# alanqrwang/keymorph

Hardware: AMD Instinct MI355X
Metric: volume-pairs/sec (fwd+bwd) at 256^3, 512 kp, TPS (higher is better)
Workload: dtype f32

## Files before the change

### include/keymorph_hip.h

```cpp
#ifndef KEYMORPH_HIP_H
#define KEYMORPH_HIP_H
#include <stddef.h>
#include <stdint.h>
#ifdef __cplusplus
extern "C" {
#endif

#define KMH_EINVAL (-22)
#define KMH_ABI_VERSION 1
int kmh_abi_version(void);

int kmh_grid_sample3d_fwd(const float* x, const float* grid, float* out, int N, int C, int D, int H,
                          int W, int Do, int Ho, int Wo, int mode, void* stream);
int kmh_grid_sample3d_bwd_grid(const float* x, const float* grid, const float* gout, float* dgrid,
                               int N, int C, int D, int H, int W, int Do, int Ho, int Wo, void* stream);
int kmh_grid_sample3d_bwd_input(const float* grid, const float* gout, float* dx, int N, int C, int D,
                                int H, int W, int Do, int Ho, int Wo, void* stream);

size_t kmh_reduce_ws_bytes(void);
int kmh_mse_fwd(const float* a, const float* b, long long n, float* out, void* ws, void* stream);
int kmh_mse_bwd(const float* a, const float* b, const float* gscale, long long n, float* da, void* stream);
int kmh_warp_mse_fwd(const float* x, const float* grid, const float* fixed, float* out, float* out_loss,
                     int N, int C, int D, int H, int W, int Do, int Ho, int Wo, void* ws, void* stream);
int kmh_warp_mse_fwd_grad(const float* x, const float* grid, const float* fixed, float* out, float* out_loss,
// ... 124 lines not shown
                               const float* wscale, void* stream);
size_t kmh_conv3d_up2_dgrad_pack_bytes(int Cout, int Cl, int terms);
int kmh_conv3d_up2_dgrad_pack_weight(const float* w, void* packed, int Cout, int Ctot, int cofs, int Cl, int terms,
                                     const float* wscale, void* stream);
size_t kmh_conv3d_up2_dgrad_stats_ws_bytes(int N, int Dl, int Hl, int Wl, int Cl);
int kmh_conv3d_up2_dgrad(const float* dz, const void* packed, float* ds, int N, int Dl, int Hl, int Wl, int Cl, int Cout,
                         int terms, const float* dscale, const float* wscale, void* stats_ws, double* stats_out,
                         int in_blocked ,
                         void* stream);
int kmh_up2_boxsum(const float* dz, float* G, int N, int Dl, int Hl, int Wl, int Cout, int in_blocked ,
                   void* stream);
size_t kmh_up2_wgrad_gemm_ws_bytes(int N, int V, int Cl, int J);
int kmh_up2_wgrad_gemm(const float* A, const float* B, float* C, int N, int V, int Cl, int J, int terms,
                       const float* ascale, const float* bscale, const float* a_scale, const float* a_shift, void* ws,
                       void* stream);
int kmh_up2_wgrad_fold_ok(int Cl, int Cout, int terms);
size_t kmh_up2_wgrad_fold_ws_bytes(int N, int Dl, int Hl, int Wl, int Cl, int Cout);
int kmh_up2_wgrad_fold(const float* xl, const float* dz, float* C, int N, int Dl, int Hl, int Wl, int Cl, int Cout, int terms,
                       const float* ascale, const float* dscale, const float* a_scale, const float* a_shift, int dz_blocked,
                       void* ws, void* stream);
int kmh_conv3d_up2_fwd(const float* xl, const float* scale, const float* shift, int Ctot, int cofs, const void* packed,
                       float* y, int N, int Dl, int Hl, int Wl, int Cl, int Cout, int terms, const float* ascale,
                       const float* wscale, void* stream);
size_t kmh_conv3d_wgrad_bf_ws_bytes(int N, int D, int H, int W, int Cin, int Cout, int terms);
int kmh_conv3d_wgrad_bf_blocked_ok(int N, int D, int H, int W, int Cin, int Cout, int terms);
int kmh_conv3d_wgrad_bf(const float* x, const float* scale, const float* shift, const float* dz,
                        const float* dzmask, float* dw, int N, int D, int H, int W, int Cin, int Cout, int relu_in,
                        int accumulate, int terms, int append_ones, const float* xscale, const float* dscale, int dz_blocked, const float* w_fold, double* bhat,
                        void* ws, void* stream);
int kmh_conv3d_wgrad_bf_sparse_ok(int N, int D, int H, int W, int Cin, int Cout, int terms);
int kmh_conv3d_wgrad_bf_sparse(const float* x, const float* scale, const float* shift, const float* dzp,
                               const unsigned char* winners, float* dw, int N, int D, int H, int W, int Cin, int Cout,
                               int relu_in, int accumulate, int terms, const float* xscale, const float* dscale,
                               const float* w_fold, double* bhat, void* ws, void* stream);
size_t kmh_conv3d_first_layer_fwd_ws_bytes(int N, int D, int H, int W, int Cout);
int kmh_conv3d_first_layer_fwd(const float* x, const float* scale, const float* shift, const float* w, float* y, int N,
                               int D, int H, int W, int Cout, void* ws, double* stats_out, void* stream);
size_t kmh_conv3d_first_layer_wgrad_ws_bytes(int N, int D, int H, int W, int Cout);
int kmh_conv3d_first_layer_wgrad(const float* x, const float* dz, const float* dzmask, const float* c123, double* rs, int N,
                                 int D, int H, int W, int Cout, void* ws, void* stream);
int kmh_conv3d_first_layer_fold(const void* rs, int rs_f64, const float* w, const float* scale_n, const float* shift_n, int Cout,
                                float* dw, double* ab_n, int accumulate, void* stream);
size_t kmh_conv3d_wgrad_ws_bytes(int N, int D, int H, int W, int Cin, int Cout);
int kmh_conv3d_wgrad(const float* x, const float* scale, const float* shift, const float* dz,
                     const float* dzmask, float* dw, int N, int D, int H, int W, int Cin, int Cout, int relu_in,
                     int accumulate, void* ws, void* stream);

size_t kmh_channel_stats_ws_bytes(int N, int C);
int kmh_channel_stats(const float* a, const float* b, int mode, int N, long long V, int C, double* out, void* ws,
                      const int* only_if, void* stream);
int kmh_gn_fwd_coeffs(const double* stats, const float* gamma, const float* beta, int N, int C, int G, double count,
                      float eps, float* scale, float* shift, float* mean_rstd, float* ascale, void* stream);
int kmh_absmax_scale(const float* x, long long n, float min_abs, float* out2, void* stream);
int kmh_gn_bwd_coeffs(const double* ab, const float* gamma, const float* mean_rstd, int N, int C, int G,
                      double count, float* c123, float* dgamma, float* dbeta, const int* only_if, void* stream);
int kmh_gn_bwd_coeffs_fold(const double* dstats, const double* bhat, const float* gamma, const float* beta,
                           const float* mean_rstd, int N, int C, int G, double count, float* c123, float* dgamma,
                           float* dbeta, int* fallback, void* stream);
int kmh_in_bwd_stats(const float* du, const float* z, const float* scale, const float* shift, int N, long long V, int C,
                     double* out, void* ws, void* stream);
int kmh_in_bwd_apply(const float* du, const float* z, const float* scale, const float* shift, const float* c123, int N,
                     long long V, int C, float* dz, float* dz_scale2, void* stream);
int kmh_in_bwd_apply_pool(const unsigned char* argmax, const float* du, const float* z, const float* scale,
                          const float* shift, const float* c123, int N, int D, int H, int W, int C, float* dz,
                          float* dz_scale2, void* stream);

int kmh_gn_bwd_apply(const float* dxn, const float* x, const float* c123, int N, long long V, int C,
                     int relu_mask, int accumulate, float* dx, float* dx_scale2, int out_blocked, void* stream);
int kmh_relu_mask(const float* dy, const float* y, long long n, float* dz, void* stream);
int kmh_norm_apply(const float* x, const float* scale, const float* shift, int N, long long V, int C, int relu,
                   float* y, void* stream);

int kmh_maxpool3d_fwd(const float* x, float* y, unsigned char* argmax, int N, int D, int H, int W, int C, void* stream);
int kmh_maxpool3d_bwd(const float* x, const unsigned char* argmax, const float* dy, const float* add, int add_cstride,
                      float* dx, int N, int D, int H, int W, int C, int out_blocked, void* stream);
size_t kmh_maxpool3d_bwd_split_bytes(int N, int D, int H, int W, int C);
int kmh_maxpool3d_bwd_split(const unsigned char* argmax, const float* dy, const float* dy_scale2, float* dxs, int N, int D,
                            int H, int W, int C, void* stream);
int kmh_maxpool3d_bwd_lazy(const unsigned char* argmax, const float* dy, const float* dxn, const float* x, const float* c123,
                           float* dx, int N, int D, int H, int W, int C, float* dx_scale2, void* stream);
int kmh_upcat_fwd(const float* skip, const float* low, float* out, int N, int D, int H, int W, int Cs, int Dl,
                  int Hl, int Wl, int Cl, void* stream);
int kmh_upcat_bwd(const float* dout, float* dskip, float* dlow, int N, int D, int H, int W, int Cs, int Dl, int Hl,
                  int Wl, int Cl, int accumulate_skip, void* stream);
int kmh_layout_convert(const float* in, float* out, int N, long long V, int C, int to_ncdhw, void* stream);

int kmh_pointwise_pack(const float* w, float* wt, int Cout, int Cin, void* stream);
int kmh_pointwise_fwd(const float* x, const float* wt, const float* bias, float* y, int N, long long V, int Cin,
                      int Cout, void* stream);
int kmh_pointwise_dgrad(const float* dy, const float* w, float* dx, int N, long long V, int Cin, int Cout,
                        void* stream);
size_t kmh_pointwise_wgrad_ws_bytes(int N, long long V, int Cin, int Cout);
int kmh_pointwise_wgrad(const float* dy, const float* x, float* dw, float* dbias, int N, long long V, int Cin,
                        int Cout, int accumulate, void* ws, void* stream);

size_t kmh_headcom_fwd_ws_bytes(int N, long long V, int Cout);
size_t kmh_headcom_bwd_ws_bytes(int N, long long V, int Cin, int Cout);
int kmh_headcom_fwd(const float* feat, const float* w, const float* bias, float* pts, float* sums, float* sq, int N, int D,
                    int H, int W, int Cin, int Cout, void* ws, void* stream);
int kmh_headcom_bwd(const float* dpts, const float* dpower, const float* feat, const float* w, const float* bias,
                    const float* sums, float* dfeat, float* dw, float* dbias, int N, int D, int H, int W, int Cin,
                    int Cout, int mask_dfeat, void* ws, void* stream);
size_t kmh_headcom_fwd_bf_ws_bytes(int N, long long V, int Cout, int terms);
size_t kmh_headcom_bwd_bf_ws_bytes(int N, long long V, int Cin, int Cout, int terms);
size_t kmh_headcom_mask_words(int N, int D, int H, int W, int Cout);
int kmh_headcom_fwd_bf(const float* feat, const float* w, const float* bias, float* pts, float* sums, float* sq,
// ... 60 lines not shown
```

### keymorph_amd/_handoff.py

```python
KEYS = ("stats", "grad_scale", "layout", "lazy_gn", "up_sources", "packed")
_ATTR = "_kmh_handoff"


def attach(t, key: str, payload) -> None:
    assert key in KEYS and payload is not None, key
    if not hasattr(t, _ATTR):
        setattr(t, _ATTR, {})
    getattr(t, _ATTR)[key] = (payload, t._version)


def peek(t, key: str):
    assert key in KEYS, key
    tag = getattr(t, _ATTR, {}).get(key)
    return tag[0] if (tag is not None and tag[1] == t._version) else None


def expect(t, key: str, present: bool, what: str, remedy: str) -> None:
    if (peek(t, key) is not None) != present:
        raise RuntimeError("keymorph_amd: %s: the tensor that arrived carries %s '%s' hand-off where %s was expected (a hook, "
                           "retain_grad, an in-place op or a second consumer replaced or changed it?) -- set %s=1"
                           % (what, "a" if not present else "no valid", key, "one" if present else "none", remedy))
```

### keymorph_amd/_lib.py

```python
from __future__ import annotations

import ctypes as C
import os

from .build import LIBPATH

_f = C.c_void_p
_i = C.c_int
_ll = C.c_longlong
_sz = C.c_size_t

PROTOS = {
    "kmh_abi_version": (_i, []),
    "kmh_grid_sample3d_fwd": (_i, [_f, _f, _f, _i, _i, _i, _i, _i, _i, _i, _i, _i, _f]),
    "kmh_grid_sample3d_bwd_grid": (_i, [_f, _f, _f, _f, _i, _i, _i, _i, _i, _i, _i, _i, _f]),
    "kmh_grid_sample3d_bwd_input": (_i, [_f, _f, _f, _i, _i, _i, _i, _i, _i, _i, _i, _f]),
    "kmh_reduce_ws_bytes": (_sz, []),
    "kmh_mse_fwd": (_i, [_f, _f, _ll, _f, _f, _f]),
    "kmh_mse_bwd": (_i, [_f, _f, _f, _ll, _f, _f]),
    "kmh_warp_mse_fwd": (_i, [_f, _f, _f, _f, _f, _i, _i, _i, _i, _i, _i, _i, _i, _f, _f]),
    "kmh_warp_mse_fwd_grad": (_i, [_f, _f, _f, _f, _f, _f, _i, _i, _i, _i, _i, _i, _i, _i, _f, _f]),
    "kmh_scale_unless_one": (_i, [_f, _ll, _f, _f]),
    "kmh_dice_sums": (_i, [_f, _f, _i, _ll, _f, _f, _f]),
    "kmh_rows_axpby": (_i, [_f, _f, _f, _f, _i, _ll, _f, _f]),
# ... 37 lines not shown
    "kmh_mi_final": (_i, [_f, _f, _i, _ll, _i, _f, _f, _f]),
    "kmh_mi_bwd": (_i, [_f, _f, _f, _f, _f, _i, _ll, _i, _f, _f, _f]),
    "kmh_mi_range": (_i, [_f, _f, _i, _ll, _i, _i, C.c_float, C.c_float, _i, C.c_float, C.c_float, _f, _f, _f]),
    "kmh_mi_hist_ranges": (_i, [_f, _f, _f, _i, _ll, _i, _f, _f]),
    "kmh_warp_mi_ws_bytes": (_sz, [_i, _i, _i, _i, _i]),
    "kmh_warp_mi_hist": (_i, [_f, _f, _f, _f, _i, _i, _i, _i, _i, _f, _f]),
    "kmh_warp_mi_bwd": (_i, [_f, _f, _f, _f, _f, _f, _i, _i, _i, _i, _i, _f, _f, _f]),
    "kmh_affine_build_matrix": (_i, [_f, _f, _f, _f, _f, _i, _f]),
    "kmh_affine_points_bwd": (_i, [_f, _f, _f, _f, _f, _i, _i, _f]),
    "kmh_com3d_fwd": (_i, [_f, _f, _f, _i, _i, _i, _i, _i, _f, _f]),
    "kmh_com3d_bwd": (_i, [_f, _f, _f, _f, _i, _i, _i, _i, _i, _f]),
    "kmh_conv3d_pack_weight": (_i, [_f, _f, _i, _i, _i, _f]),
    "kmh_conv3d_fwd": (_i, [_f, _f, _f, _f, _f, _f, _f, _i, _i, _i, _i, _i, _i, _i, _i, _f]),
    "kmh_conv3d_pack_bf_bytes": (_sz, [_i, _i, _i, _i]),
    "kmh_conv3d_pack_weight_bf": (_i, [_f, _f, _i, _i, _i, _i, _f, _f]),
    "kmh_conv3d_fwd_bf": (_i, [_f, _f, _f, _f, _f, _f, _f, _i, _i, _i, _i, _i, _i, _i, _i, _i, _i, _f, _f, _f, _f, _i, _f, _f]),
    "kmh_conv3d_fwd_bf_set_dispatch": (_i, [_i]),
    "kmh_conv3d_fwd_bf_variant": (_i, [_i, _i, _i, _i, _i, _i, _i, _i, _i]),
    "kmh_conv3d_fwd_bf_pool_ok": (_i, [_i, _i, _i, _i, _i, _i, _i]),
    "kmh_conv3d_fwd_bf_split_ok": (_i, [_i, _i, _i, _i, _i, _i, _i]),
    "kmh_conv3d_fwd_bf_sparse_ok": (_i, [_i, _i, _i, _i, _i, _i, _i]),
    "kmh_conv3d_fwd_bf_sparse": (_i, [_f, _f, _f, _f, _f, _i, _i, _i, _i, _i, _i, _i, _i, _f, _f, _f, _f, _f]),
    "kmh_conv3d_fwd_bf_pool": (_i, [_f, _f, _f, _f, _f, _f, _i, _i, _i, _i, _i, _i, _i, _i, _f, _f, _f, _f, _i, _f]),
    "kmh_conv3d_up2_dgrad_pack_bytes": (_sz, [_i, _i, _i]),
    "kmh_conv3d_up2_dgrad_pack_weight": (_i, [_f, _f, _i, _i, _i, _i, _i, _f, _f]),
    "kmh_conv3d_up2_dgrad_stats_ws_bytes": (_sz, [_i, _i, _i, _i, _i]),
    "kmh_conv3d_up2_dgrad": (_i, [_f, _f, _f, _i, _i, _i, _i, _i, _i, _i, _f, _f, _f, _f, _i, _f]),
    "kmh_up2_boxsum": (_i, [_f, _f, _i, _i, _i, _i, _i, _i, _f]),
    "kmh_up2_wgrad_gemm_ws_bytes": (_sz, [_i, _i, _i, _i]),
    "kmh_up2_wgrad_gemm": (_i, [_f, _f, _f, _i, _i, _i, _i, _i, _f, _f, _f, _f, _f, _f]),
    "kmh_up2_wgrad_fold_ok": (_i, [_i, _i, _i]),
    "kmh_up2_wgrad_fold_ws_bytes": (_sz, [_i, _i, _i, _i, _i, _i]),
    "kmh_up2_wgrad_fold": (_i, [_f, _f, _f, _i, _i, _i, _i, _i, _i, _i, _f, _f, _f, _f, _i, _f, _f]),
    "kmh_conv3d_up2_pack_bytes": (_sz, [_i, _i, _i]),
    "kmh_conv3d_up2_pack_weight": (_i, [_f, _f, _i, _i, _i, _i, _i, _f, _f]),
    "kmh_conv3d_up2_fwd": (_i, [_f, _f, _f, _i, _i, _f, _f, _i, _i, _i, _i, _i, _i, _i, _f, _f, _f]),
    "kmh_conv3d_fwd_bf_stats_ws_bytes": (_sz, [_i, _i, _i, _i, _i, _i]),
    "kmh_conv3d_first_layer_fwd_ws_bytes": (_sz, [_i, _i, _i, _i, _i]),
    "kmh_conv3d_first_layer_fwd": (_i, [_f, _f, _f, _f, _f, _i, _i, _i, _i, _i, _f, _f, _f]),
    "kmh_conv3d_wgrad_bf_ws_bytes": (_sz, [_i, _i, _i, _i, _i, _i, _i]),
    "kmh_conv3d_wgrad_bf": (_i, [_f, _f, _f, _f, _f, _f, _i, _i, _i, _i, _i, _i, _i, _i, _i, _i, _f, _f, _i, _f, _f, _f, _f]),
    "kmh_conv3d_wgrad_bf_blocked_ok": (_i, [_i, _i, _i, _i, _i, _i, _i]),
    "kmh_conv3d_wgrad_bf_sparse_ok": (_i, [_i, _i, _i, _i, _i, _i, _i]),
    "kmh_conv3d_wgrad_bf_sparse": (_i, [_f, _f, _f, _f, _f, _f, _i, _i, _i, _i, _i, _i, _i, _i, _i, _f, _f, _f, _f, _f, _f]),
    "kmh_conv3d_first_layer_wgrad_ws_bytes": (_sz, [_i, _i, _i, _i, _i]),
    "kmh_conv3d_first_layer_wgrad": (_i, [_f, _f, _f, _f, _f, _i, _i, _i, _i, _i, _f, _f]),
    "kmh_conv3d_first_layer_fold": (_i, [_f, _i, _f, _f, _f, _i, _f, _f, _i, _f]),
    "kmh_conv3d_wgrad_ws_bytes": (_sz, [_i, _i, _i, _i, _i, _i]),
    "kmh_conv3d_wgrad": (_i, [_f, _f, _f, _f, _f, _f, _i, _i, _i, _i, _i, _i, _i, _i, _f, _f]),
    "kmh_channel_stats_ws_bytes": (_sz, [_i, _i]),
    "kmh_channel_stats": (_i, [_f, _f, _i, _i, _ll, _i, _f, _f, _f, _f]),
    "kmh_gn_fwd_coeffs": (_i, [_f, _f, _f, _i, _i, _i, C.c_double, C.c_float, _f, _f, _f, _f, _f]),
    "kmh_absmax_scale": (_i, [_f, _ll, C.c_float, _f, _f]),
    "kmh_gn_bwd_coeffs": (_i, [_f, _f, _f, _i, _i, _i, C.c_double, _f, _f, _f, _f, _f]),
    "kmh_gn_bwd_coeffs_fold": (_i, [_f, _f, _f, _f, _f, _i, _i, _i, C.c_double, _f, _f, _f, _f, _f]),
    "kmh_gn_bwd_apply": (_i, [_f, _f, _f, _i, _ll, _i, _i, _i, _f, _f, _i, _f]),
    "kmh_in_bwd_stats": (_i, [_f, _f, _f, _f, _i, _ll, _i, _f, _f, _f]),
    "kmh_in_bwd_apply": (_i, [_f, _f, _f, _f, _f, _i, _ll, _i, _f, _f, _f]),
    "kmh_in_bwd_apply_pool": (_i, [_f, _f, _f, _f, _f, _f, _i, _i, _i, _i, _i, _f, _f, _f]),
    "kmh_relu_mask": (_i, [_f, _f, _ll, _f, _f]),
    "kmh_norm_apply": (_i, [_f, _f, _f, _i, _ll, _i, _i, _f, _f]),
    "kmh_maxpool3d_fwd": (_i, [_f, _f, _f, _i, _i, _i, _i, _i, _f]),
    "kmh_maxpool3d_bwd": (_i, [_f, _f, _f, _f, _i, _f, _i, _i, _i, _i, _i, _i, _f]),
    "kmh_maxpool3d_bwd_split_bytes": (_sz, [_i, _i, _i, _i, _i]),
    "kmh_maxpool3d_bwd_split": (_i, [_f, _f, _f, _f, _i, _i, _i, _i, _i, _f]),
    "kmh_maxpool3d_bwd_lazy": (_i, [_f, _f, _f, _f, _f, _f, _i, _i, _i, _i, _i, _f, _f]),
    "kmh_upcat_fwd": (_i, [_f, _f, _f, _i, _i, _i, _i, _i, _i, _i, _i, _i, _f]),
    "kmh_upcat_bwd": (_i, [_f, _f, _f, _i, _i, _i, _i, _i, _i, _i, _i, _i, _i, _f]),
    "kmh_layout_convert": (_i, [_f, _f, _i, _ll, _i, _i, _f]),
    "kmh_pointwise_pack": (_i, [_f, _f, _i, _i, _f]),
    "kmh_pointwise_fwd": (_i, [_f, _f, _f, _f, _i, _ll, _i, _i, _f]),
    "kmh_pointwise_dgrad": (_i, [_f, _f, _f, _i, _ll, _i, _i, _f]),
    "kmh_pointwise_wgrad_ws_bytes": (_sz, [_i, _ll, _i, _i]),
    "kmh_pointwise_wgrad": (_i, [_f, _f, _f, _f, _i, _ll, _i, _i, _i, _f, _f]),
    "kmh_headcom_fwd_ws_bytes": (_sz, [_i, _ll, _i]),
    "kmh_headcom_bwd_ws_bytes": (_sz, [_i, _ll, _i, _i]),
    "kmh_headcom_fwd_bf_ws_bytes": (_sz, [_i, _ll, _i, _i]),
    "kmh_headcom_bwd_bf_ws_bytes": (_sz, [_i, _ll, _i, _i, _i]),
    "kmh_headcom_mask_words": (_sz, [_i, _i, _i, _i, _i]),
    "kmh_headcom_fwd_bf": (_i, [_f, _f, _f, _f, _f, _f, _f, _i, _i, _i, _i, _i, _i, _i, _f, _f, _f]),
    "kmh_headcom_bwd_bf": (_i, [_f, _f, _f, _f, _f, _f, _f, _f, _f, _i, _i, _i, _i, _i, _i, _i, _i, _f, _f, _f, _f, _f]),
    "kmh_headcom_fwd": (_i, [_f, _f, _f, _f, _f, _f, _i, _i, _i, _i, _i, _i, _f, _f]),
    "kmh_headcom_bwd": (_i, [_f, _f, _f, _f, _f, _f, _f, _f, _f, _i, _i, _i, _i, _i, _i, _i, _f, _f]),
    "kmh_adam_step": (_i, [_f, _f, _f, _f, _ll, C.c_float, C.c_float, C.c_float, C.c_float, _i, C.c_float, _f]),
    "kmh_resize_trilinear3d_fwd": (_i, [_f, _f, _i, _i, _i, _i, _i, _i, _i, _i, _f, _f, _f, _i, _f]),
    "kmh_resize_trilinear3d_bwd": (_i, [_f, _f, _i, _i, _i, _i, _i, _i, _i, _i, _f, _f, _f, _f, _f, _f, _i, _f]),
    "kmh_components3d_ws_bytes": (_sz, [_i, _i, _i, _i]),
    "kmh_components3d": (_i, [_f, _f, _i, _i, _i, _i, _f, _f, _f]),
    "kmh_clean_mask3d": (_i, [_f, _f, _i, _i, _i, _i, C.c_double, _f, _f, _f]),
    "kmh_conv3d_thin_ok": (_i, [_i, _i]),
    "kmh_conv3d_thin_wgrad_ok": (_i, [_i, _i]),
    "kmh_conv3d_thin_fwd": (_i, [_f, _f, _f, _f, _i, _i, _i, _i, _i, _i, _i, _f]),
    "kmh_conv3d_thin_dgrad": (_i, [_f, _f, _f, _f, _i, _i, _i, _i, _i, _i, _f]),
    "kmh_conv3d_thin_wgrad_ws_bytes": (_sz, [_i, _i, _i, _i, _i, _i]),
    "kmh_conv3d_thin_wgrad": (_i, [_f, _f, _f, _f, _f, _i, _i, _i, _i, _i, _i, _f, _f]),
    "kmh_field_identity": (_i, [_f, _i, _i, _i, _i, _f]),
    "kmh_field_compose": (_i, [_f, _f, _f, _i, _i, _i, _i, _i, _i, _i, _f]),
    "kmh_field_invert_ws_bytes": (_sz, [_i, _i, _i, _i]),
    "kmh_field_invert": (_i, [_f, _f, _f, _f, _f, _f, _f, _i, _i, _i, _i, C.c_float, _i, _f, _f]),
    "kmh_field_to_displacement": (_i, [_f, _f, _i, _i, _i, _i, _f]),
    "kmh_field_from_displacement": (_i, [_f, _f, _i, _i, _i, _i, _f]),
    "kmh_bspline_grid_fwd": (_i, [_f, _f, _f, _i, _i, _i, _i, _i, _i, _i, _f]),
    "kmh_bspline_grid_ws_bytes": (_sz, [_i, _i, _i, _i, _i, _i, _i]),
    "kmh_bspline_grid_bwd": (_i, [_f, _f, _i, _i, _i, _i, _i, _i, _i, _f, _f]),
    "kmh_bspline_bending_ws_bytes": (_sz, [_i]),
    "kmh_bspline_bending_fwd": (_i, [_f, _f, _i, _i, _i, _i, _f, _f]),
# ... 105 lines not shown
```

### keymorph_amd/backbone_ops.py

```python
from __future__ import annotations

import os
from typing import Optional, Tuple

import torch

from . import _lib
from ._handoff import attach, expect, peek
from ._lib import check
from .ops import _p, _prep, _stream, workspace

Tensor = torch.Tensor
EPS = 1e-5

CONV_MODE = os.environ.get("KEYMORPH_HIP_CONV", "f16x3")
_TERMS = {"f16x3": 2, "bf16x6": 3}
_HEAD_TERMS = {"f16x3": 2, "bf16x6": 3}
BF_ROWS_PER_WAVE = int(os.environ.get("KEYMORPH_HIP_BF_ROWS", "4"))


def set_conv_mode(mode: str):
    global CONV_MODE
    assert mode in ("f32", "f16x3", "bf16x6"), mode
    CONV_MODE = mode


_SWITCHES = {
    "KEYMORPH_NO_EPILOGUE_STATS": "a separate statistics pass per layer instead of the convolution epilogue's",
    "KEYMORPH_NO_UPCONV": "materialise upsample+concat instead of the fused decoder operator, forward",
    "KEYMORPH_NO_UPCONV_BWD": "materialise upsample+concat instead of the fused decoder operator, backward",
    "KEYMORPH_NO_UPCONV_WGRAD": "the fused decoder operator rebuilds the upsampled half for the 27-tap weight gradient",
    "KEYMORPH_NO_UP2_FOLD": "the upsampled channels' weight gradient by the box-sum tensor + matrix product route",
    "KEYMORPH_NO_STATS_FOLD": "GroupNorm's backward statistics by a pass over the tensors",
    "KEYMORPH_NO_BLOCKED_GRADS": "every gradient in (N,D,H,W,C)",
    "KEYMORPH_NO_BLOCKED_UPCAT": "only the fused decoder operator's gradient in (N,D,H,W,C)",
    "KEYMORPH_NO_SPLIT_POOLGRAD": "the 256^3-level pooled gradient scattered as fp32 instead of pre-split records",
    "KEYMORPH_NO_SPARSE_POOLGRAD": "the 256^3-level pooled gradient scattered into pre-split records instead of handed over with its winners",
    "KEYMORPH_NO_CONV_POOL": "separate pooling pass instead of the conv epilogue's",
    "KEYMORPH_NO_LAZY_FIRST": "GroupNorm backward of the first block as its own pass",
    "KEYMORPH_NO_LAZY_SKIP": "GroupNorm's backward of a decoder skip applied in the decoder",
    "KEYMORPH_NO_LAZY_IN": "ConvNet block by block: separate norm / ReLU / pooling passes",
    "KEYMORPH_RANGE_AUDIT": "debug (ON = audit): per-sample dynamic range of every gradient operand, RANGE_AUDIT_LOG",
}


def _off(name: str) -> bool:
    if name not in _SWITCHES:
        raise KeyError(name)
    return bool(os.environ.get(name))


import contextlib
import functools
import threading

_AMP_DEFAULT = os.environ.get("KEYMORPH_AMP", "0") not in ("", "0")
_amp_tls = threading.local()


def amp_enabled() -> bool:
    return bool(getattr(_amp_tls, "on", _AMP_DEFAULT))


@contextlib.contextmanager
def amp_scope(on: bool):
    prev = amp_enabled()
    _amp_tls.on = bool(on)
    try:
        yield
    finally:
        _amp_tls.on = prev


def set_amp(on: bool) -> bool:
    prev = amp_enabled()
    _amp_tls.on = bool(on)
    return prev


def _t(terms: int) -> int:
    return 1 if (terms == 2 and amp_enabled()) else terms


def _binds_amp(cls):
    fwd, bwd = cls.forward, cls.backward

    @staticmethod
    @functools.wraps(fwd)
    def forward(ctx, *a, **k):
        ctx._kmh_amp = amp_enabled()
        return fwd(ctx, *a, **k)

    @staticmethod
    @functools.wraps(bwd)
    def backward(ctx, *g):
        with amp_scope(ctx._kmh_amp):
            return bwd(ctx, *g)

    cls.forward, cls.backward = forward, backward
    return cls


FIRST_BLOCK_DGRAD = os.environ.get("KEYMORPH_FIRST_BLOCK_DGRAD", "")


def set_first_block_dgrad(mode: str) -> str:
    global FIRST_BLOCK_DGRAD
    assert mode in ("", "bf16x6"), mode
    prev, FIRST_BLOCK_DGRAD = FIRST_BLOCK_DGRAD, mode
    return prev


def first_block_dgrad_terms() -> int:
    return 3 if (FIRST_BLOCK_DGRAD == "bf16x6" and CONV_MODE == "f16x3") else 0


def _f32(shape, dev):
    return torch.empty(shape, dtype=torch.float32, device=dev)


def channel_stats(a: Tensor, b: Optional[Tensor], N: int, V: int, C: int, only_if: Optional[Tensor] = None) -> Tensor:
    lib = _lib.load()
    out = torch.empty((N, C, 2), dtype=torch.float64, device=a.device)
    ws = workspace(int(lib.kmh_channel_stats_ws_bytes(N, C)), a.device, "stats")
    check(lib.kmh_channel_stats(_p(a), _p(b), 0 if b is None else 1, N, V, C, _p(out), _p(ws), _p(only_if), _stream()),
          "kmh_channel_stats")
    return out


def _needs_range_scales() -> bool:
    return _TERMS.get(CONV_MODE, 0) == 2


_CONSTS = {}


def _const(device, *values) -> Tensor:
    key = (str(device), values)
    t = _CONSTS.get(key)
    if t is None:
        t = _CONSTS[key] = torch.tensor(values, dtype=torch.float32, device=device)
    return t


def absmax_scale(x: Tensor, min_abs: float = 0.0) -> Tensor:
    lib = _lib.load()
    out = _f32((2,), x.device)
    check(lib.kmh_absmax_scale(_p(x), x.numel(), float(min_abs), _p(out), _stream()), "kmh_absmax_scale")
    return out


def conv_emits_stats() -> bool:
    return CONV_MODE != "f32" and not _off("KEYMORPH_NO_EPILOGUE_STATS")


def _tag_stats(t: Tensor, stats: Optional[Tensor]) -> None:
    if stats is not None:
        attach(t, "stats", stats)


def _peek_stats(t: Tensor) -> Optional[Tensor]:
    return peek(t, "stats")


STATS_STATS = {"carried": 0, "measured": 0}


def input_stats(x: Tensor, N: int, V: int, C: int) -> Tensor:
    s = _peek_stats(x)
    if s is not None and tuple(s.shape) == (N, C, 2):
        STATS_STATS["carried"] += 1
        return s
    STATS_STATS["measured"] += 1
    return channel_stats(x, None, N, V, C)


def _tag_grad_scale(t: Optional[Tensor], scale2: Optional[Tensor], loosen: float = 1.0) -> None:
    if t is None or scale2 is None:
        return
    if loosen != 1.0:
        scale2 = torch.stack([scale2[0] * (1.0 / loosen), scale2[1] * loosen])
    attach(t, "grad_scale", scale2)


def _sum_bound(a: Optional[Tensor], b: Optional[Tensor]) -> Optional[Tensor]:
    if a is None or b is None:
        return None
    return torch.stack([torch.minimum(a[0], b[0]) * 0.5, torch.maximum(a[1], b[1]) * 2.0])


GRAD_SCALE_STATS = {"carried": 0, "measured": 0}
RANGE_AUDIT_LOG = []


def range_audit(t: Tensor) -> dict:
    with torch.no_grad():
        a = t.detach().abs().reshape(t.shape[0], -1).float()
        m_n = a.amax(dim=1).double()
        M = float(m_n.max())
        if M == 0.0:
            return {"max": 0.0, "per_sample_log2_below_max": [0.0] * t.shape[0], "worst_relative_precision": 2.0 ** -22,
                    "flushed_fraction": 0.0}
        S = 2.0 ** (14 - int(torch.floor(torch.log2(torch.tensor(M))).item()))
        nz = a > 0
        flushed = float(((a * S < 2.0 ** -25) & nz).sum()) / max(1.0, float(nz.sum()))
        below = [float(torch.log2(torch.tensor(M) / m)) if float(m) > 0 else float("inf") for m in m_n]
        prec = max(max(2.0 ** -22, 2.0 ** (b - 39)) for b in below if b != float("inf"))
        return {"max": M, "per_sample_log2_below_max": below, "worst_relative_precision": prec,
                "flushed_fraction": flushed}


def grad_scale(dy: Tensor) -> Tensor:
    if _off("KEYMORPH_RANGE_AUDIT") and not _blocked_kind(dy):
        RANGE_AUDIT_LOG.append(dict(range_audit(dy), shape=tuple(dy.shape)))
    s = peek(dy, "grad_scale")
    if s is not None:
        GRAD_SCALE_STATS["carried"] += 1
        return s
    GRAD_SCALE_STATS["measured"] += 1
    return absmax_scale(dy)


def norm_coeffs(stats: Tensor, gamma: Optional[Tensor], beta: Optional[Tensor], N: int, C: int, G: int, V: int,
                want_ascale: bool = False):
    lib = _lib.load()
    dev = stats.device
    scale, shift, mr = _f32((N, C), dev), _f32((N, C), dev), _f32((N, G, 2), dev)
    ascale = _f32((2,), dev) if (want_ascale and _needs_range_scales()) else None
    check(lib.kmh_gn_fwd_coeffs(_p(stats), _p(gamma), _p(beta), N, C, G, float(V), EPS, _p(scale), _p(shift),
                                _p(mr), _p(ascale), _stream()), "kmh_gn_fwd_coeffs")
    return (scale, shift, mr, ascale) if want_ascale else (scale, shift, mr)


def pack_weight(w: Tensor, transposed: bool, wscale: Optional[Tensor] = None, terms: int = 0) -> Tensor:
    lib = _lib.load()
    Cout, Cin = w.shape[:2]
    if CONV_MODE != "f32":
        terms = terms or _TERMS[CONV_MODE]
        out = torch.empty(int(lib.kmh_conv3d_pack_bf_bytes(Cout, Cin, int(transposed), terms)), dtype=torch.uint8,
                          device=w.device)
        wscale = (wscale if wscale is not None else absmax_scale(w)) if terms == 2 else None
        attach(out, "packed", (terms, wscale))
        check(lib.kmh_conv3d_pack_weight_bf(_p(w), _p(out), Cout, Cin, int(transposed), terms, _p(wscale), _stream()),
              "kmh_conv3d_pack_weight_bf")
        return out
    out = _f32((27, Cout, Cin) if transposed else (27, Cin, Cout), w.device)
    check(lib.kmh_conv3d_pack_weight(_p(w), _p(out), Cout, Cin, int(transposed), _stream()), "kmh_conv3d_pack_weight")
    return out


def _packed(pk: Tensor):
    return peek(pk, "packed") or (0, None)


def _conv_meta(N, D, H, W, Cin, Cout, taps=27) -> None:
    if _lib.profiler.enabled:
        _lib.profiler.meta = {"flops": 2.0 * taps * Cin * Cout * N * D * H * W, "shape": (N, D, H, W, Cin, Cout)}


def conv3_raw(x, scale, shift, packed, bias, N, D, H, W, Cin, Cout, relu_in, relu_out, mask=None,
              ascale=None, stats_out: Optional[Tensor] = None, in_blocked: bool = False,
              addend: Optional[Tensor] = None, winners: Optional[Tensor] = None) -> Tensor:
    lib = _lib.load()
    y = _f32((N, D, H, W, Cout), x.device)
    _conv_meta(N, D, H, W, Cin, Cout)
    terms, wscale = _packed(packed)
    if int(in_blocked) == 3:
        assert terms == 2 and winners is not None and scale is None and shift is None and mask is None and addend is None \
            and not relu_in and ascale is not None and not amp_enabled(), "pooled + winners: a gradient operand of the f16x3 mode"
        assert x.shape == winners.shape == (N, D // 2, H // 2, W // 2, Cin) and winners.dtype == torch.uint8
        sws = None
        if stats_out is not None:
            sws = workspace(int(lib.kmh_conv3d_fwd_bf_stats_ws_bytes(N, D, H, W, Cout, BF_ROWS_PER_WAVE)), x.device, "convstats")
        check(lib.kmh_conv3d_fwd_bf_sparse(_p(x), _p(winners), _p(packed), _p(bias), _p(y), N, D, H, W, Cin, Cout, int(relu_out), 2,
                                           _p(ascale), _p(wscale), _p(sws), _p(stats_out), _stream()), "kmh_conv3d_fwd_bf_sparse")
        return y
    assert winners is None
    if terms:
        if terms == 2 and ascale is None:
            assert scale is None, "a normalised input needs the range scale of the NORMALISED tensor (norm_coeffs)"
            ascale = absmax_scale(x)
        sws = None
        if stats_out is not None:
            sws = workspace(int(lib.kmh_conv3d_fwd_bf_stats_ws_bytes(N, D, H, W, Cout, BF_ROWS_PER_WAVE)), x.device,
                            "convstats")
        check(lib.kmh_conv3d_fwd_bf(_p(x), _p(scale), _p(shift), _p(mask), _p(packed), _p(bias), _p(y), N, D, H, W,
                                    Cin, Cout, int(relu_in), int(relu_out), _t(terms), BF_ROWS_PER_WAVE,
                                    _p(ascale if terms == 2 else None), _p(wscale), _p(sws), _p(stats_out),
                                    int(in_blocked), _p(addend), _stream()), "kmh_conv3d_fwd_bf")
        return y
    assert stats_out is None and addend is None, "only the split-operand kernels emit output statistics / take an addend"
    assert not in_blocked, "the channel-blocked input layout belongs to the split-operand kernels"
    check(lib.kmh_conv3d_fwd(_p(x), _p(scale), _p(shift), _p(mask), _p(packed), _p(bias), _p(y), N, D, H, W, Cin,
                             Cout, int(relu_in), int(relu_out), _stream()), "kmh_conv3d_fwd")
# ... 262 lines not shown
            if dy_sparse:
                sd_in = sd_in if sd_in is not None else absmax_scale(dy)
                full = dy.detach()
                SPLIT_STATS["handoffs"] += 1
                SPARSE_STATS["handoffs"] += 1
            elif dy_split:
                sd_in = sd_in if sd_in is not None else absmax_scale(dy)
                full = torch.empty((N, Cout // 8, D * H * W + 1, 8), dtype=torch.float32, device=dy.device)
                check(lib.kmh_maxpool3d_bwd_split(_p(ctx.pool_arg), _p(dy), _p(sd_in), _p(full), N, D, H, W, Cout, _stream()),
                      "kmh_maxpool3d_bwd_split")
                SPLIT_STATS["handoffs"] += 1
            else:
                full = torch.empty((N, D, H, W, Cout), dtype=torch.float32, device=dy.device)
                if odd:
                    full.zero_()
                check(lib.kmh_maxpool3d_bwd(None, _p(ctx.pool_arg), _p(dy), None, 0, _p(full), N, D, H, W, Cout,
                                            int(dy_blocked), _stream()), "kmh_maxpool3d_bwd")
            _tag_grad_scale(full, sd_in)
            dy = full
            if dy_blocked:
                attach(dy, "layout", 3 if dy_sparse else (2 if dy_split else 1))
                BLOCKED_STATS["handoffs"] += 1
        kind = 3 if dy_sparse else (2 if dy_split else int(dy_blocked))
        if _blocked_kind(dy) != kind:
            raise RuntimeError("keymorph_amd: gradient layout kind %d where %d was expected (1 = fp32 channel-blocked, 2 = pre-split"
                               " records, 3 = pooled + winners); a hook or an in-place op between two operators changed the tensor" % (_blocked_kind(dy), kind))
        ymask = None if dy_premasked else y
        first = Cin == 1 and not ctx.needs_input_grad[0] and (Cout <= 16 or CONV_MODE != "f32")
        dscale = (grad_scale(dy) if (_needs_range_scales() and not (first and Cout <= 16)) else None)
        if first:
            lazy_c123, ymask = lazy_tag if dy_lazy else (None, ymask)
            dw, dgamma, dbeta = first_layer_grads(x, scale, shift, mr, gamma, weight, dy, ymask, N, D, H, W, Cout, G,
                                                  dscale=dscale, lazy_c123=lazy_c123)
            return (None, dgamma, dbeta, dw) + (None,) * 9
        assert not dy_lazy, "only the first layer's correlation kernel applies a pending GroupNorm backward"
        need_affine = ctx.needs_input_grad[1] or ctx.needs_input_grad[2]
        need_dxn = ctx.needs_input_grad[0] or need_affine
        fold = need_dxn and ctx.needs_input_grad[3] and conv_emits_stats() and not _off("KEYMORPH_NO_STATS_FOLD")
        bhat = torch.zeros((N, Cin), dtype=torch.float64, device=x.device) if fold else None
        dw = (conv3_wgrad(x, scale, shift, dy, N, D, H, W, Cin, Cout, False, dzmask=ymask, xscale=ctx.ascale,
                          dscale=dscale, dz_blocked=kind, fold=(weight, bhat) if fold else None,
                          winners=ctx.pool_arg if dy_sparse else None)
              if ctx.needs_input_grad[3] else None)
        dx = dgamma = dbeta = None
        if need_dxn:
            dstats = torch.empty((N, Cin, 2), dtype=torch.float64, device=x.device) if fold else None
            if ctx.dgrad_terms:
                FIRST_BLOCK_STATS["exact_dgrads"] += 1
            dxn = conv3_raw(dy, None, None,
                            pack_weight(weight, True, None if ctx.dgrad_terms else getattr(ctx, "wscale", None), terms=ctx.dgrad_terms),
                            None, N, D, H, W, Cout, Cin, False, False,
                            mask=ymask, ascale=dscale, in_blocked=kind, stats_out=dstats,
                            winners=ctx.pool_arg if dy_sparse else None)
            sc2 = torch.zeros(2, dtype=torch.float32, device=x.device) if (_needs_range_scales() and ctx.needs_input_grad[0]) else None
            c123, dgamma, dbeta = _gn_bwd_coeffs(lambda flag: channel_stats(dxn, x, N, V, Cin, only_if=flag), gamma, mr,
                                                 N, Cin, G, V, fold=(dstats, bhat, beta) if fold else None)
            if ctx.needs_input_grad[0] and dx_lazy:
                assert x_from_relu and not dx_blocked
                dx = dxn
                attach(dx, "lazy_gn", (c123, x))
                LAZY_STATS["handoffs"] += 1
            elif ctx.needs_input_grad[0]:
                dx = _gn_bwd_apply(dxn, x, c123, N, V, Cin, sc2, from_relu=x_from_relu,
                                   out=torch.empty_like(dxn) if dx_blocked else None, blocked=dx_blocked)
        return (dx, dgamma, dbeta, dw) + (None,) * 9


def _up2_forward(skip, low, scale, shift, ascale, weight, N, D, H, W, Cs, Cl, Cout, ystats):
    lib = _lib.load()
    terms = _TERMS[CONV_MODE]
    dev = skip.device
    pk_s = pack_weight(weight[:, :Cs].contiguous(), False)
    wsu = None
    if terms == 2:
        wsu = absmax_scale(weight[:, Cs:].contiguous()) * _const(dev, 0.125, 8.0)
    pku = torch.empty(int(lib.kmh_conv3d_up2_pack_bytes(Cout, Cl, terms)), dtype=torch.uint8, device=dev)
    check(lib.kmh_conv3d_up2_pack_weight(_p(weight), _p(pku), Cout, Cs + Cl, Cs, Cl, terms, _p(wsu), _stream()),
          "kmh_conv3d_up2_pack_weight")
    part = _f32((N, D, H, W, Cout), dev)
    _conv_meta(N, D, H, W, Cl, Cout, taps=8)
    check(lib.kmh_conv3d_up2_fwd(_p(low), _p(scale), _p(shift), Cs + Cl, Cs, _p(pku), _p(part), N, D // 2, H // 2,
                                 W // 2, Cl, Cout, _t(terms), _p(ascale if terms == 2 else None), _p(wsu), _stream()),
          "kmh_conv3d_up2_fwd")
    y = conv3_raw(skip, scale[:, :Cs].contiguous(), shift[:, :Cs].contiguous(), pk_s, None, N, D, H, W, Cs, Cout,
                  False, True, ascale=ascale, stats_out=ystats, addend=part)
    UPCONV_STATS["calls"] += 1
    return y


def upcat_conv_ok(skip, low, Cout) -> bool:
    return (CONV_MODE in _TERMS and conv_emits_stats() and Cout > 16 and Cout % 4 == 0 and skip.shape[-1] % 8 == 0
            and low.shape[-1] % 8 == 0 and all(a == 2 * b for a, b in zip(skip.shape[1:4], low.shape[1:4]))
            and not _off("KEYMORPH_NO_UPCONV") and not _off("KEYMORPH_NO_UPCONV_BWD"))


@_binds_amp
class _UpCatConvGCR(torch.autograd.Function):

    @staticmethod
    def forward(ctx, skip, low, gamma, beta, weight, num_groups, dy_premasked, dskip_lazy=False, dy_blocked=False):
        ctx.dskip_lazy = bool(dskip_lazy)
        ctx.dy_blocked = bool(dy_blocked)
        assert not dy_blocked or dy_premasked, "a channel-blocked gradient comes from a SingleConv, i.e. already masked"
        skip, low, gamma, beta, weight = _prep(skip), _prep(low), _prep(gamma), _prep(beta), _prep(weight)
        N, D, H, W, Cs = skip.shape
        Cl, Cout = low.shape[-1], weight.shape[0]
        V = D * H * W
# ... 23 lines not shown
            check(lib.kmh_relu_mask(_p(dy), _p(y), dy.numel(), _p(dzm), _stream()), "kmh_relu_mask")
            dy = dzm
        dscale = grad_scale(dy) if _needs_range_scales() else None
        bhat_s = torch.zeros((N, Cs), dtype=torch.float64, device=dy.device)
        dw_s = conv3_wgrad(skip, scale[:, :Cs].contiguous(), shift[:, :Cs].contiguous(), dy, N, D, H, W, Cs, Cout, False,
                           xscale=ctx.ascale, dscale=dscale, dz_blocked=blk, fold=(weight[:, :Cs].contiguous(), bhat_s))
        if Cout % 4 == 0 and not _off("KEYMORPH_NO_UPCONV_WGRAD"):
            Vl = V // 8
            sc_l, sh_l = scale[:, Cs:].contiguous(), shift[:, Cs:].contiguous()
            terms = _TERMS[CONV_MODE]
            dwn = _f32((N, Cl, 27, Cout), dy.device)
            if _lib.profiler.enabled:
                _lib.profiler.meta = {"flops": 2.0 * 27 * Cl * Cout * N * Vl, "shape": (N, Vl, Cl, 27 * Cout)}
            if up2_wgrad_fold_ok(Cl, Cout, terms):
                UP2_STATS["fold"] += 1
                gws = workspace(int(lib.kmh_up2_wgrad_fold_ws_bytes(N, D // 2, H // 2, W // 2, Cl, Cout)), dy.device, "wgrad")
                check(lib.kmh_up2_wgrad_fold(_p(low), _p(dy), _p(dwn), N, D // 2, H // 2, W // 2, Cl, Cout, _t(terms), _p(ctx.ascale),
                                             _p(dscale), _p(sc_l), _p(sh_l), int(blk), _p(gws), _stream()), "kmh_up2_wgrad_fold")
            else:
                UP2_STATS["boxsum"] += 1
                boxes = _f32((N, Vl, 27 * Cout), dy.device)
                check(lib.kmh_up2_boxsum(_p(dy), _p(boxes), N, D // 2, H // 2, W // 2, Cout, int(blk), _stream()), "kmh_up2_boxsum")
                gws = workspace(int(lib.kmh_up2_wgrad_gemm_ws_bytes(N, Vl, Cl, 27 * Cout)), dy.device, "wgrad")
                bsc = (dscale * _const(dy.device, 0.125, 8.0)) if terms == 2 else None
                check(lib.kmh_up2_wgrad_gemm(_p(low), _p(boxes), _p(dwn), N, Vl, Cl, 27 * Cout, _t(terms),
                                             _p(ctx.ascale if terms == 2 else None), _p(bsc), _p(sc_l), _p(sh_l), _p(gws),
                                             _stream()), "kmh_up2_wgrad_gemm")
                del boxes
            dw_l = dwn.sum(0).permute(2, 0, 1).reshape(Cout, Cl, 3, 3, 3)
            wl = weight[:, Cs:].reshape(Cout, Cl, 27).permute(1, 2, 0)
            bhat_l = (dwn.double() * wl.double().unsqueeze(0)).sum(dim=(2, 3))
        else:
            xu = _f32((N, D, H, W, Cl), dy.device)
            check(lib.kmh_upcat_fwd(_p(skip), _p(low), _p(xu), N, D, H, W, 0, D // 2, H // 2, W // 2, Cl, _stream()),
                  "kmh_upcat_fwd")
            bhat_l = torch.zeros((N, Cl), dtype=torch.float64, device=dy.device)
            dw_l = conv3_wgrad(xu, scale[:, Cs:].contiguous(), shift[:, Cs:].contiguous(), dy, N, D, H, W, Cl, Cout,
                               False, xscale=ctx.ascale, dscale=dscale, dz_blocked=blk,
                               fold=(weight[:, Cs:].contiguous(), bhat_l))
            del xu
        dw = torch.cat([dw_s, dw_l], dim=1)
        bhat = torch.cat([bhat_s, bhat_l], dim=1)
        dst_s = torch.empty((N, Cs, 2), dtype=torch.float64, device=dy.device)
        dxn_s = conv3_raw(dy, None, None, pack_weight(weight[:, :Cs].contiguous(), True), None, N, D, H, W, Cout, Cs,
                          False, False, ascale=dscale, stats_out=dst_s, in_blocked=blk)
        dst_l = torch.empty((N, Cl, 2), dtype=torch.float64, device=dy.device)
        dsum_l = conv3_up2_dgrad(dy, weight, Cs, Cl, dscale, stats_out=dst_l, dz_blocked=blk)
        dstats = torch.cat([dst_s, dst_l], dim=1)
        ab = lambda flag: torch.cat([channel_stats(dxn_s, skip, N, V, Cs, only_if=flag),
                                     channel_stats(dsum_l, low, N, V // 8, Cl, only_if=flag)], dim=1)
        c123, dgamma, dbeta = _gn_bwd_coeffs(ab, gamma, mr, N, C, G, V, fold=(dstats, bhat, beta))
        c_s = c123[:, :Cs].contiguous()
        c_l = (c123[:, Cs:] * _const(dy.device, 1.0, 8.0, 8.0)).contiguous()
        sc_s = torch.zeros(2, dtype=torch.float32, device=dy.device) if _needs_range_scales() else None
        sc_l = torch.zeros(2, dtype=torch.float32, device=dy.device) if _needs_range_scales() else None
        dskip = dlow = None
        if ctx.needs_input_grad[0] and ctx.dskip_lazy:
            dskip = dxn_s
            attach(dskip, "lazy_gn", (c_s, skip))
            LAZY_STATS["handoffs"] += 1
        elif ctx.needs_input_grad[0]:
            dskip = _gn_bwd_apply(dxn_s, skip, c_s, N, V, Cs, sc_s)
        if ctx.needs_input_grad[1]:
            dlow = _gn_bwd_apply(dsum_l, low, c_l, N, V // 8, Cl, sc_l)
        return (dskip, dlow, dgamma, dbeta, dw) + (None,) * 4


def upcat_blocked_ok(skip, low, Cout) -> bool:
    N, D, H, W, Cs = skip.shape
    return (torch.is_grad_enabled() and Cout % 8 == 0 and not _off("KEYMORPH_NO_UPCONV_WGRAD")
            and not _off("KEYMORPH_NO_BLOCKED_UPCAT") and grad_blocked_ok(N, D, H, W, Cs, Cout))


def upcat_conv_gcr(skip, low, gamma, beta, weight, num_groups: int, dy_premasked: bool = False,
                   dskip_lazy: bool = False, dy_blocked: bool = False) -> Tensor:
    if dskip_lazy:
        node = skip.grad_fn
        if node is not None and type(node).__name__ == "_PoolForkBackward":
            node._kmh_expect_lazy = True
        else:
            dskip_lazy = False
    y, ystats = _UpCatConvGCR.apply(skip, low, gamma, beta, weight, num_groups, dy_premasked, dskip_lazy, dy_blocked)
    _tag_stats(y, ystats)
    return y


def single_conv_gcr(x, gamma, beta, weight, num_groups: int, x_from_relu: bool = True,
                    dy_premasked: bool = False, dy_blocked: bool = False, dx_blocked: bool = False,
                    pool: bool = False, dy_lazy: bool = False, dx_lazy: bool = False, dgrad_terms: int = 0) -> Tensor:
    y, ystats = _SingleConvGCR.apply(x, gamma, beta, weight, num_groups, x_from_relu, dy_premasked, dy_blocked,
                                     dx_blocked, pool, dy_lazy, dx_lazy, dgrad_terms)
    _tag_stats(y, ystats)
    return y


POOL_STATS = {"fused": 0}
FIRST_BLOCK_STATS = {"exact_dgrads": 0}
LAZY_STATS = {"handoffs": 0}


def lazy_skip_ok(skip) -> bool:
    return (torch.is_grad_enabled() and skip.shape[1] % 2 == 0 and skip.shape[2] % 2 == 0 and skip.shape[3] % 2 == 0
            and skip.shape[4] % 4 == 0 and not _off("KEYMORPH_NO_LAZY_SKIP"))


def lazy_first_layer_ok(x, cout1: int) -> bool:
    return (x.shape[-1] == 1 and cout1 <= 16 and not x.requires_grad and torch.is_grad_enabled()
            and not _off("KEYMORPH_NO_LAZY_FIRST"))
# ... 31 lines not shown
    if add is not None:
        acs = add.stride(3)
        dense_voxels = add.stride() == (D * H * W * acs, H * W * acs, W * acs, acs, 1)
        if odd or add.dtype != torch.float32 or not dense_voxels:
            add, acs = add.contiguous().float().clone(), C
    if add is not None and acs == C and odd:
        dx = add
    else:
        dx = (torch.zeros if odd else torch.empty)((N, D, H, W, C), dtype=torch.float32, device=arg.device)
    dy_c = _prep(dy)
    check(lib.kmh_maxpool3d_bwd(None, _p(arg), _p(dy_c), _p(add), acs, _p(dx), N, D, H, W, C, int(out_blocked),
                                _stream()), "kmh_maxpool3d_bwd")
    if out_blocked:
        attach(dx, "layout", 1)
        BLOCKED_STATS["handoffs"] += 1
    sd = peek(dy, "grad_scale")
    _tag_grad_scale(dx, sd if add_tag is _NO_ADD else _sum_bound(sd, add_tag))
    return dx


class _MaxPool2(torch.autograd.Function):
    @staticmethod
    def forward(ctx, x, blocked_grad):
        ctx.blocked_grad = bool(blocked_grad)
        return _maxpool_fwd(ctx, x)[1]

    @staticmethod
    def backward(ctx, dy):
        return _maxpool_bwd(ctx, dy, None, ctx.blocked_grad), None


def maxpool2(x: Tensor, blocked_grad: bool = False) -> Tensor:
    return _MaxPool2.apply(x, blocked_grad)


class _PoolFork(torch.autograd.Function):

    @staticmethod
    def forward(ctx, x):
        x, y = _maxpool_fwd(ctx, x)
        ctx.set_materialize_grads(False)
        return y, x.view_as(x)

    @staticmethod
    def backward(ctx, dy, dskip):
        if dskip is not None and getattr(ctx, "_kmh_expect_lazy", False):
            expect(dskip, "lazy_gn", True, "pool_fork's skip gradient with its GroupNorm backward pending", "KEYMORPH_NO_LAZY_SKIP")
        lazy = peek(dskip, "lazy_gn") if dskip is not None else None
        if lazy is not None:
            lib = _lib.load()
            c123, x = lazy
            N, D, H, W, C = ctx.xshape
            dxn = _prep(dskip)
            sc2 = torch.zeros(2, dtype=torch.float32, device=dxn.device) if _needs_range_scales() else None
            if dy is None:
                return _gn_bwd_apply(dxn, x, c123, N, D * H * W, C, sc2)
            (arg,) = ctx.saved_tensors
            dx = torch.empty((N, D, H, W, C), dtype=torch.float32, device=dxn.device)
            check(lib.kmh_maxpool3d_bwd_lazy(_p(arg), _p(_prep(dy)), _p(dxn), _p(x), _p(c123), _p(dx), N, D, H, W, C, _p(sc2),
                                             _stream()), "kmh_maxpool3d_bwd_lazy")
            _tag_grad_scale(dx, sc2)
            return dx
        if dy is None:
            return dskip
        return _maxpool_bwd(ctx, dy, dskip)


def pool_fork(x: Tensor):
    y, skip = _PoolFork.apply(x)
    _tag_stats(skip, _peek_stats(x))
    return y, skip


class _UpCat(torch.autograd.Function):
    @staticmethod
    def forward(ctx, skip, low, lazy_skip_grad):
        lib = _lib.load()
        skip, low = _prep(skip), _prep(low)
        N, D, H, W, Cs = skip.shape
        _, Dl, Hl, Wl, Cl = low.shape
        out = _f32((N, D, H, W, Cs + Cl), skip.device)
        check(lib.kmh_upcat_fwd(_p(skip), _p(low), _p(out), N, D, H, W, Cs, Dl, Hl, Wl, Cl, _stream()), "kmh_upcat_fwd")
        ctx.dims = (N, D, H, W, Cs, Dl, Hl, Wl, Cl)
        ctx.lazy = bool(lazy_skip_grad)
        return out

    @staticmethod
    def backward(ctx, dout):
        lib = _lib.load()
        N, D, H, W, Cs, Dl, Hl, Wl, Cl = ctx.dims
        dout = _prep(dout)
        dskip = None if ctx.lazy else _f32((N, D, H, W, Cs), dout.device)
        dlow = _f32((N, Dl, Hl, Wl, Cl), dout.device)
        check(lib.kmh_upcat_bwd(_p(dout), _p(dskip), _p(dlow), N, D, H, W, Cs, Dl, Hl, Wl, Cl, 0, _stream()),
              "kmh_upcat_bwd")
        if ctx.lazy:
            dskip = dout[..., :Cs]
        sd = peek(dout, "grad_scale")
        _tag_grad_scale(dskip, sd)
        if (D, H, W) == (2 * Dl, 2 * Hl, 2 * Wl):
            _tag_grad_scale(dlow, sd, loosen=8.0)
        return dskip, dlow, None


def upcat(skip: Tensor, low: Tensor, lazy_skip_grad: bool = False) -> Tensor:
    out = _UpCat.apply(skip, low, lazy_skip_grad)
    ss, sl = _peek_stats(skip), _peek_stats(low)
# ... 156 lines not shown
        dw = conv3_wgrad(x, None, None, dz, N, D, H, W, Cin, Cout, False, dzmask=dzmask)
        dzm = dz
        if dzmask is not None:
            dzm = torch.empty_like(dz)
            check(lib.kmh_relu_mask(_p(dz), _p(dzmask), dz.numel(), _p(dzm), _stream()), "kmh_relu_mask")
        db = channel_stats(dzm, None, N, V, Cout)[:, :, 0].sum(0).float()
        dx = None
        if ctx.needs_input_grad[0]:
            dx = conv3_raw(dz, None, None, pack_weight(weight, True), None, N, D, H, W, Cout, Cin, False, False,
                           mask=dzmask)
        return (dx, dw, db, dgamma, dbeta) + (None,) * 5


def conv_block(x, weight, bias, gamma=None, beta=None, groups: int = 0) -> Tensor:
    return _ConvBlock.apply(x, weight, bias, gamma, beta, groups)


def conv_block_batchnorm(x, weight, bias, bn: "torch.nn.modules.batchnorm._BatchNorm", training: bool) -> Tensor:
    assert abs(bn.eps - EPS) < 1e-12, "the norm kernels use eps = 1e-5 (what every norm layer of the reference uses)"
    use_batch = training or not bn.track_running_stats or bn.running_mean is None
    if not use_batch:
        return _ConvBlock.apply(x, weight, bias, bn.weight, bn.bias, 0, 2, bn.running_mean, bn.running_var, bn.eps)
    y, stats = _ConvBlock.apply(x, weight, bias, bn.weight, bn.bias, 0, 1, None, None, bn.eps)
    if training and bn.track_running_stats and bn.running_mean is not None:
        with torch.no_grad():
            n = float(x.shape[0] * x.shape[1] * x.shape[2] * x.shape[3])
            mean = stats[0, :, 0] / n
            var = (stats[0, :, 1] / n - mean * mean).clamp_min(0.0)
            bn.num_batches_tracked += 1
            mom = bn.momentum if bn.momentum is not None else 1.0 / float(bn.num_batches_tracked)
            bn.running_mean.mul_(1 - mom).add_(mean.to(bn.running_mean.dtype), alpha=mom)
            bn.running_var.mul_(1 - mom).add_((var * (n / max(n - 1.0, 1.0))).to(bn.running_var.dtype), alpha=mom)
    return y


LAZY_IN_STATS = {"units": 0}


def convnet_lazy_ok(x: Tensor, norm_type: str) -> bool:
    return (norm_type == "instance" and conv_emits_stats() and not _off("KEYMORPH_NO_LAZY_IN")
            and not (x.requires_grad and torch.is_grad_enabled())
            and all(int(d) % 16 == 0 for d in x.shape[1:4]))


def _in_bwd(g, u, zprev, scale, shift, mr, arg=None, in_place=False):
    lib = _lib.load()
    N, Dp, Hp, Wp, C = zprev.shape
    ab = torch.empty((N, C, 2), dtype=torch.float64, device=g.device)
    ws = workspace(int(lib.kmh_channel_stats_ws_bytes(N, C)), g.device, "stats")
    check(lib.kmh_in_bwd_stats(_p(g), _p(u), _p(scale), _p(shift), N, u.shape[1] * u.shape[2] * u.shape[3], C, _p(ab), _p(ws),
                               _stream()), "kmh_in_bwd_stats")
    c123, _, _ = _gn_bwd_coeffs(ab, None, mr, N, C, C, Dp * Hp * Wp)
    out = g if in_place else torch.empty_like(zprev)
    sc2 = torch.zeros(2, dtype=torch.float32, device=g.device) if _needs_range_scales() else None
    if arg is not None:
        check(lib.kmh_in_bwd_apply_pool(_p(arg), _p(g), _p(zprev), _p(scale), _p(shift), _p(c123), N, Dp, Hp, Wp, C, _p(out),
                                        _p(sc2), _stream()), "kmh_in_bwd_apply_pool")
    else:
        check(lib.kmh_in_bwd_apply(_p(g), _p(zprev), _p(scale), _p(shift), _p(c123), N, Dp * Hp * Wp, C, _p(out), _p(sc2),
                                   _stream()), "kmh_in_bwd_apply")
    _tag_grad_scale(out, sc2)
    return out


@_binds_amp
class _ConvINUnit(torch.autograd.Function):

    @staticmethod
    def forward(ctx, zprev, st, weight, bias, pool, first):
        lib = _lib.load()
        zprev, weight, bias = _prep(zprev), _prep(weight), _prep(bias)
        N, Dp, Hp, Wp, Cin = zprev.shape
        Cout = weight.shape[0]
        ctx.first, ctx.pool = bool(first), bool(pool)
        scale = shift = mr = ascale = arg = None
        u = zprev
        if not first:
            scale, shift, mr, ascale = norm_coeffs(st, None, None, N, Cin, Cin, Dp * Hp * Wp, want_ascale=True)
            if pool:
                u = _f32((N, Dp // 2, Hp // 2, Wp // 2, Cin), zprev.device)
                arg = torch.empty(u.shape, dtype=torch.uint8, device=zprev.device)
                check(lib.kmh_maxpool3d_fwd(_p(zprev), _p(u), _p(arg), N, Dp, Hp, Wp, Cin, _stream()), "kmh_maxpool3d_fwd")
        D, H, W = u.shape[1:4]
        pk = pack_weight(weight, False)
        ctx.wscale = _packed(pk)[1]
        zst = torch.empty((N, Cout, 2), dtype=torch.float64, device=zprev.device)
        z = conv3_raw(u, scale, shift, pk, bias, N, D, H, W, Cin, Cout, not first, False, ascale=ascale, stats_out=zst)
        ctx.ascale = ascale
        ctx.dims = (N, Dp, Hp, Wp, D, H, W, Cin, Cout)
        saved = [zprev, weight] + ([] if first else [scale, shift, mr]) + ([u, arg] if (pool and not first) else [])
        ctx.save_for_backward(*saved)
        ctx.mark_non_differentiable(zst)
        LAZY_IN_STATS["units"] += 1
        return z, zst

    @staticmethod
    def backward(ctx, dz, _dst):
        N, Dp, Hp, Wp, D, H, W, Cin, Cout = ctx.dims
        saved = ctx.saved_tensors
        zprev, weight = saved[0], saved[1]
        dscale = peek(dz, "grad_scale")
        dz = _prep(dz)
        if _needs_range_scales() and dscale is None:
            dscale = absmax_scale(dz)
        db = torch.zeros(Cout, dtype=torch.float32, device=dz.device)
        if ctx.first:
            xs = absmax_scale(zprev) if _needs_range_scales() else None
# ... 50 lines not shown
    N, D, H, W, Cin = feat.shape
    Cout = w.shape[0]
    pts, sums = _f32((N, Cout, 3), feat.device), _f32((N, Cout, 4), feat.device)
    hsc = hmask = None
    if CONV_MODE != "f32" and Cin % 4 == 0:
        terms = _HEAD_TERMS[CONV_MODE]
        ws = workspace(int(lib.kmh_headcom_fwd_bf_ws_bytes(N, D * H * W, Cout, terms)), feat.device, "head")
        if scales and terms == 2:
            hsc = _f32((4,), feat.device)
        nmask = int(lib.kmh_headcom_mask_words(N, D, H, W, Cout)) if mask else 0
        if nmask:
            hmask = torch.empty(nmask, dtype=torch.int32, device=feat.device)
        check(lib.kmh_headcom_fwd_bf(_p(feat), _p(w), _p(b), _p(pts), _p(sums), _p(sq), _p(hsc), N, D, H, W, Cin, Cout,
                                     _t(terms), _p(hmask), _p(ws), _stream()), "kmh_headcom_fwd_bf")
    else:
        ws = workspace(int(lib.kmh_headcom_fwd_ws_bytes(N, D * H * W, Cout)), feat.device, "head")
        check(lib.kmh_headcom_fwd(_p(feat), _p(w), _p(b), _p(pts), _p(sums), _p(sq), N, D, H, W, Cin, Cout, _p(ws),
                                  _stream()), "kmh_headcom_fwd")
    return pts, sums, hsc, hmask


@_binds_amp
class _HeadCoM(torch.autograd.Function):

    @staticmethod
    def forward(ctx, feat, w, b, feat_from_relu=False):
        ctx.set_materialize_grads(False)
        ctx.mask_dfeat = int(bool(feat_from_relu))
        feat, w = _prep(feat), _prep(w)
        b = None if b is None else _prep(b)
        pts, sums, ctx.hsc, ctx.hmask = _headcom_fwd(feat, w, b, scales=True, mask=HEAD_MASK and any(ctx.needs_input_grad[:3]))
        if CONV_MODE != "f32" and feat.shape[-1] % 4 == 0:
            HEAD_STATS["mask" if ctx.hmask is not None else "recompute"] += 1
        ctx.save_for_backward(feat, w, sums) if b is None else ctx.save_for_backward(feat, w, sums, b)
        return pts, sums[:, :, 0].contiguous()

    @staticmethod
    def backward(ctx, dpts, dpower):
        lib = _lib.load()
        saved = ctx.saved_tensors
        feat, w, sums = saved[:3]
        b = saved[3] if len(saved) > 3 else None
        N, D, H, W, Cin = feat.shape
        Cout = w.shape[0]
        dpts = torch.zeros((N, Cout, 3), dtype=torch.float32, device=feat.device) if dpts is None else _prep(dpts)
        dpower = None if dpower is None else _prep(dpower)
        dfeat = torch.empty_like(feat) if ctx.needs_input_grad[0] else None
        need_w = ctx.needs_input_grad[1] or (b is not None and ctx.needs_input_grad[2])
        dw = torch.empty_like(w) if need_w else None
        db = _f32((Cout,), feat.device) if (need_w and b is not None) else None
        if CONV_MODE != "f32" and Cin % 4 == 0:
            terms = _HEAD_TERMS[CONV_MODE]
            ws = workspace(int(lib.kmh_headcom_bwd_bf_ws_bytes(N, D * H * W, Cin, Cout, terms)), feat.device, "head")
            dsc = (torch.zeros(2, dtype=torch.float32, device=feat.device)
                   if (terms == 2 and dfeat is not None) else None)
            check(lib.kmh_headcom_bwd_bf(_p(dpts), _p(dpower), _p(feat), _p(w), _p(b), _p(sums), _p(dfeat), _p(dw), _p(db), N, D, H,
                                         W, Cin, Cout, _t(terms), ctx.mask_dfeat, _p(ctx.hsc), _p(dsc), _p(ctx.hmask), _p(ws), _stream()),
                  "kmh_headcom_bwd_bf")
            _tag_grad_scale(dfeat, dsc)
        else:
            ws = workspace(int(lib.kmh_headcom_bwd_ws_bytes(N, D * H * W, Cin, Cout)), feat.device, "head")
            check(lib.kmh_headcom_bwd(_p(dpts), _p(dpower), _p(feat), _p(w), _p(b), _p(sums), _p(dfeat), _p(dw), _p(db), N, D, H,
                                      W, Cin, Cout, ctx.mask_dfeat, _p(ws), _stream()), "kmh_headcom_bwd")
        return dfeat, dw, db, None


HEAD_FUSED_MAX_CIN = 64


def head_moments(feat: Tensor, w: Tensor, b: Optional[Tensor]):
    with torch.no_grad():
        feat, w = _prep(feat), _prep(w)
        b = None if b is None else _prep(b)
        sq = _f32((feat.shape[0], w.shape[0]), feat.device)
        pts, sums, _, _ = _headcom_fwd(feat, w, b, sq=sq)
        return pts, sums[:, :, 0].contiguous(), sq


def head_com(feat: Tensor, w: Tensor, b: Optional[Tensor], feat_from_relu: bool = False) -> Tensor:
    return _HeadCoM.apply(feat, w, b, feat_from_relu)[0]


def head_com_power(feat: Tensor, w: Tensor, b: Optional[Tensor], feat_from_relu: bool = False):
    return _HeadCoM.apply(feat, w, b, feat_from_relu)
```

### keymorph_amd/csrc/absmax.h

```cpp
#pragma once
#include "common.h"

namespace kmh_absmax {
__device__ __forceinline__ void publish(float m, unsigned* acc) {
  m = wave_max(m);
  if ((threadIdx.x & 63) == 0) {
    const unsigned bits = __float_as_uint(m);
    if (bits > __hip_atomic_load(acc, __ATOMIC_RELAXED, __HIP_MEMORY_SCOPE_AGENT)) atomicMax(acc, bits);
  }
}
__global__ __launch_bounds__(256) static void partial_kernel(const float* __restrict__ x, long long n,
                                                             unsigned* __restrict__ acc) {
  float m = 0.f;
  long long head = (long long)(((16 - (reinterpret_cast<unsigned long long>(x) & 15)) & 15) >> 2);
  if (head > n) head = n;
  const float* xb = x + head;
  const long long nb = n - head, n4 = nb >> 2;
  for (long long i = (long long)blockIdx.x * 256 + threadIdx.x; i < n4; i += (long long)gridDim.x * 256) {
    const float4 v = reinterpret_cast<const float4*>(xb)[i];
    m = fmaxf(fmaxf(m, fmaxf(fabsf(v.x), fabsf(v.y))), fmaxf(fabsf(v.z), fabsf(v.w)));
  }
  if (blockIdx.x == 0) {
    for (long long i = threadIdx.x; i < head; i += 256) m = fmaxf(m, fabsf(x[i]));
    for (long long i = (n4 << 2) + threadIdx.x; i < nb; i += 256) m = fmaxf(m, fabsf(xb[i]));
  }
  publish(m, acc);
}
__global__ static void final_kernel(float* __restrict__ out2, float min_abs) {
  const float m = fmaxf(__uint_as_float(reinterpret_cast<unsigned*>(out2)[0]), min_abs);
  range_scale(m, out2);
}
static inline int launch(const float* x, long long n, float min_abs, float* out2, hipStream_t s) {
  hipError_t e = hipMemsetAsync(out2, 0, 2 * sizeof(float), s);
  if (e != hipSuccess) return (int)e;
  long long nb = (n / 4 + 256) / 256;
  if (nb > 2048) nb = 2048;
  partial_kernel<<<(int)nb, 256, 0, s>>>(x, n, reinterpret_cast<unsigned*>(out2));
  final_kernel<<<1, 1, 0, s>>>(out2, min_abs);
  return (int)hipGetLastError();
}
}
```

### keymorph_amd/csrc/headcom.hip

```cpp
#include <type_traits>
#include "common.h"
#include "absmax.h"

namespace {

typedef float f32x16 __attribute__((ext_vector_type(16)));
constexpr int HTPB = 256;
constexpr int VT = 128;
constexpr int LD = 65;
constexpr int GC = 128;

struct Dims { int D, H, W; };

__device__ __forceinline__ void stage_feat(const float* __restrict__ feat, long long v0, long long V, int Cin,
                                           Dims d, float* sX, float4* sC, int tid) {
  for (int e = tid; e < VT * 64; e += HTPB) {
    const int c = e & 63, v = e >> 6;
    float val = 0.f;
    if (c < Cin && v0 + v < V) val = feat[(v0 + v) * Cin + c];
    sX[v * LD + c] = val;
  }
  if (tid < VT) {
    const long long v = v0 + tid;
    float4 c = make_float4(0.f, 0.f, 0.f, 0.f);
// ... 689 lines not shown
      }
#pragma unroll
      for (int s2 = 0; s2 < 2; ++s2) {
        bf16x8 a[TERMS];
        split8<TERMS>(dh + 8 * s2, a);
#pragma unroll
        for (int ct = 0; ct < 2; ++ct) {
          if (32 * ct < Cin) {
            bf16x8 b[TERMS];
#pragma unroll
            for (int t = 0; t < TERMS; ++t)
              b[t] = *reinterpret_cast<const bf16x8*>(sFT + t * (64 * 128) + swz(32 * ct + li, 4 * vb + 2 * s2 + lh));
            dw[ct] = mfma_split<TERMS>(a, b, dw[ct]);
          }
        }
      }
    }
    n = n_next;
    v0 = v_next;
    step(n_next, v_next);
    if (tile + 1 < t_end) {
      commit(tile + 1, v0);
      if (tile + 2 < t_end) feat_fetch<WVT, NT_>(pre, feat + (long long)n_next * V * Cin, v_next, V, Cin, tid);
    }
    __syncthreads();
  }
  float* ow = pw + (long long)slab * Cout * Cin;
#pragma unroll
  for (int ct = 0; ct < 2; ++ct) {
    const int c = 32 * ct + li;
#pragma unroll
    for (int r = 0; r < 16; ++r) {
      const int k = grp * (32 * NWV) + 32 * wv + (r & 3) + 8 * (r >> 2) + 4 * lh;
      if (k < Cout && c < Cin) ow[(long long)k * Cin + c] = dw[ct][r] * desc_w;
    }
  }
  db += __shfl_xor(db, 32, 64);
  if (ROWS) db /= sDh;
  if (lh == 0 && co < Cout) pb[(long long)slab * Cout + co] = db;
}

constexpr int BF_TPB = 512;
constexpr int WBLK = 64;
template <int TERMS>
__global__ __launch_bounds__(BF_TPB, 2) void headcom_bwd_feat_bf_kernel(const float* __restrict__ feat,
                                                                        const __bf16* __restrict__ wkp,
                                                                        const __bf16* __restrict__ wt,
                                                                        const float* __restrict__ bias,
                                                                        const float* __restrict__ g,
                                                                        float* __restrict__ dfeat, long long V,
                                                                        int Cin, int Cout, int CoutP, Dims d,
                                                                        const float* __restrict__ hs, int mask_dfeat,
                                                                        unsigned* __restrict__ amax ,
                                                                        const int* __restrict__ gate, int want) {
  if (gate && *gate != want) return;
  extern __shared__ __attribute__((aligned(16))) unsigned char hsm[];
  constexpr int IMG = TERMS * 64 * 128;
  constexpr int BUF = 2 * IMG + WBLK * 32;
  constexpr int NLD = (2 * IMG / 16 + BF_TPB - 1) / BF_TPB;
  const int tid = threadIdx.x, lane = tid & 63, wv = tid >> 6, li = lane & 31, lh = lane >> 5;
  const int n = blockIdx.y;
  const long long v = (long long)blockIdx.x * 256 + 32 * wv + li;
  const bool vok = v < V;
  const int nks = (Cin + 15) >> 4;
  const float* fn = feat + (long long)n * V * Cin;
  const float sFs = hs[0], desc = hs[1] * hs[3], sDh = hs[4], desc_f = hs[5] * hs[3];
  float cz = 0.f, cy = 0.f, cx = 0.f;
  if (vok) {
    const int x = (int)(v % d.W), y = (int)((v / d.W) % d.H), z = (int)(v / ((long long)d.W * d.H));
    cz = d.D > 1 ? (float)z / (float)(d.D - 1) : 0.f;
    cy = d.H > 1 ? (float)y / (float)(d.H - 1) : 0.f;
    cx = d.W > 1 ? (float)x / (float)(d.W - 1) : 0.f;
  }
  bf16x8 fb[4][TERMS];
#pragma unroll
  for (int s = 0; s < 4; ++s) {
    float x8[8] = {0.f, 0.f, 0.f, 0.f, 0.f, 0.f, 0.f, 0.f};
    const int c0 = 16 * s + 4 * lh;
    if (vok && c0 < Cin) {
      const float4 p = *reinterpret_cast<const float4*>(fn + v * Cin + c0);
      x8[0] = p.x; x8[1] = p.y; x8[2] = p.z; x8[3] = p.w;
    }
    if (vok && c0 + 8 < Cin) {
      const float4 p = *reinterpret_cast<const float4*>(fn + v * Cin + c0 + 8);
      x8[4] = p.x; x8[5] = p.y; x8[6] = p.z; x8[7] = p.w;
    }
#pragma unroll
    for (int j = 0; j < 8; ++j) x8[j] *= sFs;
    split8<TERMS>(x8, fb[s]);
  }
  f32x16 acc2[2];
#pragma unroll
  for (int mt = 0; mt < 2; ++mt)
#pragma unroll
    for (int r = 0; r < 16; ++r) acc2[mt][r] = 0.f;

  const int nblk = CoutP / WBLK;
  uint4 pre[NLD];
  auto fetch = [&](int blk) {
#pragma unroll
    for (int k = 0; k < NLD; ++k) {
      const int i = tid + k * BF_TPB;
      pre[k] = make_uint4(0u, 0u, 0u, 0u);
      if (i < 2 * IMG / 16) {
        const int chunk = i & 7, row = (i >> 3) & 63, t = (i >> 9) % TERMS, img = i / (TERMS * 512);
        const __bf16* src = img == 0 ? wkp + ((long long)t * CoutP + blk * WBLK + row) * 64 + chunk * 8
// ... 43 lines not shown
          bf16x8 a[TERMS];
#pragma unroll
          for (int t = 0; t < TERMS; ++t)
            a[t] = *reinterpret_cast<const bf16x8*>(sWk + t * (64 * 128) + swz(32 * m + li, 2 * s + lh));
          acc = mfma_split<TERMS>(a, fb[s], acc);
        }
      }
      float dh[16];
#pragma unroll
      for (int r = 0; r < 16; ++r) {
        const float4 gq = *reinterpret_cast<const float4*>(sG + (32 * m + (r & 3) + 8 * (r >> 2) + 4 * lh) * 8);
        const float gd = fmaf(gq.w, cx, fmaf(gq.z, cy, fmaf(gq.y, cz, gq.x)));
        dh[r] = acc[r] > 0.f ? gd : 0.f;
      }
#pragma unroll
      for (int s2 = 0; s2 < 2; ++s2) {
        bf16x8 b[TERMS];
        split8<TERMS>(dh + 8 * s2, b);
#pragma unroll
        for (int mt = 0; mt < 2; ++mt) {
          if (32 * mt < Cin) {
            bf16x8 a[TERMS];
#pragma unroll
            for (int t = 0; t < TERMS; ++t)
              a[t] = *reinterpret_cast<const bf16x8*>(sWt + t * (64 * 128) + swz(32 * mt + li, 4 * m + 2 * s2 + lh));
            acc2[mt] = mfma_split<TERMS>(a, b, acc2[mt]);
          }
        }
      }
    }
    if (blk + 1 < nblk) commit(blk + 1, hsm + ((blk + 1) & 1) * BUF);
    __syncthreads();
  }
  float mxo = 0.f;
  if (vok) {
    float* o = dfeat + ((long long)n * V + v) * Cin;
#pragma unroll
    for (int mt = 0; mt < 2; ++mt)
#pragma unroll
      for (int q = 0; q < 4; ++q) {
        const int c = 32 * mt + 8 * q + 4 * lh;
        if (c < Cin) {
          float4 r = make_float4(acc2[mt][4 * q] * desc_f, acc2[mt][4 * q + 1] * desc_f, acc2[mt][4 * q + 2] * desc_f,
                                 acc2[mt][4 * q + 3] * desc_f);
          if (mask_dfeat) {
            const float4 f = *reinterpret_cast<const float4*>(fn + v * Cin + c);
            r.x = f.x > 0.f ? r.x : 0.f; r.y = f.y > 0.f ? r.y : 0.f; r.z = f.z > 0.f ? r.z : 0.f; r.w = f.w > 0.f ? r.w : 0.f;
          }
          *reinterpret_cast<float4*>(o + c) = r;
          mxo = fmaxf(fmaxf(mxo, fmaxf(fabsf(r.x), fabsf(r.y))), fmaxf(fabsf(r.z), fabsf(r.w)));
        }
      }
  }
  if (amax) kmh_absmax::publish(mxo, amax);
}

template <int TERMS, int NWV, bool WIDE, bool AMP = false>
__global__ __launch_bounds__(64 * NWV, 2) void headcom_bwd_w_mask_kernel(
    const float* __restrict__ feat, const unsigned* __restrict__ mask, const float* __restrict__ g,
    float* __restrict__ pw , float* __restrict__ pb , int N, long long V,
    int Cin, int Cout, int CoutP, Dims d, int tiles_per_slab, int ngroups, const float* __restrict__ hs,
    const int* __restrict__ gate, int want) {
  if (gate && *gate != want) return;
  extern __shared__ __attribute__((aligned(16))) unsigned char hsm[];
  constexpr int WBUF = TERMS * 64 * 128;
  const int tid = threadIdx.x, lane = tid & 63, wv = tid >> 6, li = lane & 31, lh = lane >> 5;
  const int item = xcd_remap(blockIdx.x, gridDim.x);
  const int grp = item % ngroups, slab = item / ngroups;
  constexpr int NT_ = 64 * NWV;
  const int co = grp * (32 * NWV) + 32 * wv + li;
  const float sFs = hs[0], sDh = hs[4], desc_w = hs[5] * hs[1];
  f32x16 dw[2];
#pragma unroll
  for (int ct = 0; ct < 2; ++ct)
#pragma unroll
    for (int r = 0; r < 16; ++r) dw[ct][r] = 0.f;
  kmh_f2 db2 = {0.f, 0.f};
  const long long tiles_per_n = V / WVT, ntiles = tiles_per_n * N;
  long long t_beg = (long long)slab * tiles_per_slab, t_end = t_beg + tiles_per_slab;
  if (t_end > ntiles) t_end = ntiles;
  FeatRegs<WVT, NT_> pre;
  int n = t_beg < t_end ? (int)(t_beg / tiles_per_n) : 0;
  long long v0 = (t_beg - (long long)n * tiles_per_n) * WVT;
  const unsigned* mrow = mask + co;
  auto commit = [&](long long tile, long long vfirst) {
    unsigned char* b = hsm + (int)((tile - t_beg) & 1) * WBUF;
    feat_commit<TERMS, WVT, NT_, true, false>(pre, vfirst, V, d, nullptr, b, nullptr, tid, sFs, false);
  };
  auto mfetch = [&](int nn, long long vv, unsigned out[2]) {
    const long long nb = ((long long)nn * V + vv) >> 5;
    out[0] = mrow[nb * CoutP];
    out[1] = mrow[(nb + 1) * CoutP];
  };
  auto step = [&](int& nn, long long& vv) { vv += WVT; if (vv >= V) { vv = 0; ++nn; } };
  int n_next = n;
  long long v_next = v0;
  step(n_next, v_next);
  unsigned mcur[2] = {0u, 0u}, mnext[2] = {0u, 0u};
  if (t_beg < t_end) {
    feat_fetch<WVT, NT_>(pre, feat + (long long)n * V * Cin, v0, V, Cin, tid);
    mfetch(n, v0, mcur);
    commit(t_beg, v0);
    if (t_beg + 1 < t_end) {
      feat_fetch<WVT, NT_>(pre, feat + (long long)n_next * V * Cin, v_next, V, Cin, tid);
      mfetch(n_next, v_next, mnext);
    }
  }
// ... 20 lines not shown
        unsigned m;
        asm("v_bfe_i32 %0, %1, %2, 1" : "=v"(m) : "v"(w), "n"(pos));
        dh[r] = __uint_as_float(__float_as_uint(fmaf(gxs, (float)pos, G)) & m);
      }
#pragma unroll
      for (int j = 0; j < 8; ++j) db2 += kmh_f2{dh[2 * j], dh[2 * j + 1]};
#pragma unroll
      for (int s2 = 0; s2 < 2; ++s2) {
        bf16x8 a[TERMS];
        split8<TERMS>(dh + 8 * s2, a);
#pragma unroll
        for (int ct = 0; ct < (WIDE ? 2 : 1); ++ct) {
          bf16x8 b[TERMS];
#pragma unroll
          for (int t = 0; t < TERMS; ++t)
            b[t] = *reinterpret_cast<const bf16x8*>(sFT + t * (64 * 128) + swz(32 * ct + li, 4 * vb + 2 * s2 + lh));
          dw[ct] = mfma_split<TERMS, AMP>(a, b, dw[ct]);
        }
      }
    }
    n = n_next;
    v0 = v_next;
    step(n_next, v_next);
    mcur[0] = mnext[0]; mcur[1] = mnext[1];
    if (tile + 1 < t_end) {
      commit(tile + 1, v0);
      if (tile + 2 < t_end) {
        feat_fetch<WVT, NT_>(pre, feat + (long long)n_next * V * Cin, v_next, V, Cin, tid);
        mfetch(n_next, v_next, mnext);
      }
    }
    __syncthreads();
  }
  float* ow = pw + (long long)slab * Cout * Cin;
#pragma unroll
  for (int ct = 0; ct < 2; ++ct) {
    const int c = 32 * ct + li;
#pragma unroll
    for (int r = 0; r < 16; ++r) {
      const int k = grp * (32 * NWV) + 32 * wv + (r & 3) + 8 * (r >> 2) + 4 * lh;
      if (k < Cout && c < Cin) ow[(long long)k * Cin + c] = dw[ct][r] * desc_w;
    }
  }
  float db = db2.x + db2.y;
  db += __shfl_xor(db, 32, 64);
  db /= sDh;
  if (lh == 0 && co < Cout) pb[(long long)slab * Cout + co] = db;
}

template <int TERMS, bool WIDE, bool AMP = false>
__global__ __launch_bounds__(BF_TPB, 2) void headcom_bwd_feat_mask_kernel(
    const float* __restrict__ feat, const __bf16* __restrict__ wt, const unsigned* __restrict__ mask,
    const float* __restrict__ g, float* __restrict__ dfeat, long long V, int Cin, int Cout, int CoutP, Dims d,
    const float* __restrict__ hs, int mask_dfeat, unsigned* __restrict__ amax, const int* __restrict__ gate, int want) {
  if (gate && *gate != want) return;
  extern __shared__ __attribute__((aligned(16))) unsigned char hsm[];
  constexpr int IMG = TERMS * 64 * 128;
  constexpr int BUF = IMG + 8 * WBLK * 16;
  constexpr int NLD = (IMG / 16 + BF_TPB - 1) / BF_TPB;
  const int tid = threadIdx.x, lane = tid & 63, li = lane & 31, lh = lane >> 5;
  const int wv = __builtin_amdgcn_readfirstlane(tid >> 6);
  const int n = blockIdx.y;
  const long long vw = (long long)blockIdx.x * 256 + 32 * wv;
  const bool wok = vw < V;
  const long long v = vw + li;
  const float* fn = feat + (long long)n * V * Cin;
  const float sDh = hs[4], desc_f = hs[5] * hs[3];
  float cz = 0.f, cy = 0.f, cx = 0.f;
  if (wok) {
    const unsigned u = (unsigned)vw, row = u / (unsigned)d.W, x0 = u - row * (unsigned)d.W;
    const unsigned z = row / (unsigned)d.H, y = row - z * (unsigned)d.H;
    cz = d.D > 1 ? (float)z / (float)(d.D - 1) : 0.f;
    cy = d.H > 1 ? (float)y / (float)(d.H - 1) : 0.f;
    cx = d.W > 1 ? (float)(x0 + li) / (float)(d.W - 1) : 0.f;
  }
  const unsigned* mrow = mask + ((((long long)n * V + (wok ? vw : 0)) >> 5) * CoutP) + lane;
  f32x16 acc2[2];
#pragma unroll
  for (int mt = 0; mt < 2; ++mt)
#pragma unroll
    for (int r = 0; r < 16; ++r) acc2[mt][r] = 0.f;
  const int nblk = CoutP / WBLK;
  uint4 pre[NLD];
  unsigned mpre;
  auto fetch = [&](int blk) {
#pragma unroll
    for (int k = 0; k < NLD; ++k) {
      const int i = tid + k * BF_TPB;
      pre[k] = make_uint4(0u, 0u, 0u, 0u);
      if (i < IMG / 16) {
        const int chunk = i & 7, row = (i >> 3) & 63, t = i >> 9;
        pre[k] = *reinterpret_cast<const uint4*>(wt + ((long long)t * 64 + row) * CoutP + blk * WBLK + chunk * 8);
      }
    }
    mpre = mrow[blk * WBLK];
  };
  auto commit = [&](int blk, unsigned char* buf) {
#pragma unroll
    for (int k = 0; k < NLD; ++k) {
      const int i = tid + k * BF_TPB;
      if (i < IMG / 16) {
        const int chunk = i & 7, row = (i >> 3) & 63, t = i >> 9;
        *reinterpret_cast<uint4*>(buf + t * (64 * 128) + swz(row, chunk)) = pre[k];
      }
    }
    const int k = blk * WBLK + lane;
    float4 gq = make_float4(0.f, 0.f, 0.f, 0.f);
// ... 17 lines not shown
#pragma unroll
      for (int hb = 0; hb < 2; ++hb) {
        kmh_f4 ab[8];
#pragma unroll
        for (int r = 0; r < 8; ++r) ab[r] = sAB4[32 * m + (r & 3) + 8 * ((8 * hb + r) >> 2) + 4 * lh];
        __builtin_amdgcn_sched_barrier(0);
#pragma unroll
        for (int r = 0; r < 8; ++r) {
          asm volatile("" : "+v"(ab[r]));
          unsigned mk;
          float gd;
          asm("v_bfe_i32 %0, %1, %2, 1" : "=v"(mk) : "v"(ab[r].z), "v"(li));
          asm("v_fma_f32 %0, %1, %2, %3" : "=v"(gd) : "v"(ab[r].y), "v"(cx), "v"(ab[r].x));
          dh[8 * hb + r] = __uint_as_float(__float_as_uint(gd) & mk);
        }
      }
#pragma unroll
      for (int s2 = 0; s2 < 2; ++s2) {
        bf16x8 b[TERMS];
        split8<TERMS>(dh + 8 * s2, b);
#pragma unroll
        for (int mt = 0; mt < (WIDE ? 2 : 1); ++mt) {
          bf16x8 a[TERMS];
#pragma unroll
          for (int t = 0; t < TERMS; ++t)
            a[t] = *reinterpret_cast<const bf16x8*>(sWt + t * (64 * 128) + swz(32 * mt + li, 4 * m + 2 * s2 + lh));
          acc2[mt] = mfma_split<TERMS, AMP>(a, b, acc2[mt]);
        }
      }
    }
    if (blk + 1 < nblk) commit(blk + 1, hsm + ((blk + 1) & 1) * BUF);
    __syncthreads();
  }
  float mxo = 0.f;
  if (wok) {
    float* o = dfeat + ((long long)n * V + v) * Cin;
#pragma unroll
    for (int mt = 0; mt < 2; ++mt)
#pragma unroll
      for (int q = 0; q < 4; ++q) {
        const int c = 32 * mt + 8 * q + 4 * lh;
        if (c < Cin) {
          float4 r = make_float4(acc2[mt][4 * q] * desc_f, acc2[mt][4 * q + 1] * desc_f, acc2[mt][4 * q + 2] * desc_f,
                                 acc2[mt][4 * q + 3] * desc_f);
          if (mask_dfeat) {
            const float4 f = *reinterpret_cast<const float4*>(fn + v * Cin + c);
            r.x = f.x > 0.f ? r.x : 0.f; r.y = f.y > 0.f ? r.y : 0.f; r.z = f.z > 0.f ? r.z : 0.f; r.w = f.w > 0.f ? r.w : 0.f;
          }
          *reinterpret_cast<float4*>(o + c) = r;
          mxo = fmaxf(fmaxf(mxo, fmaxf(fabsf(r.x), fabsf(r.y))), fmaxf(fabsf(r.z), fabsf(r.w)));
        }
      }
  }
  if (amax) kmh_absmax::publish(mxo, amax);
}


static int fwd_slabs(long long V, int* tps) {
  const long long ntiles = (V + VT - 1) / VT;
  long long t = (ntiles + 255) / 256;
  if (t < 1) t = 1;
  *tps = (int)t;
  return (int)((ntiles + t - 1) / t);
}
static int bwdw_slabs(int N, long long V, int* tps) {
  const long long ntiles = ((V + VT - 1) / VT) * N;
  long long t = (ntiles + 255) / 256;
  if (t < 1) t = 1;
  *tps = (int)t;
  return (int)((ntiles + t - 1) / t);
}

}

KMH_API size_t kmh_headcom_fwd_ws_bytes(int N, long long V, int Cout) {
  int tps;
  return (size_t)N * Cout * fwd_slabs(V, &tps) * 5 * sizeof(double);
}
KMH_API size_t kmh_headcom_bwd_ws_bytes(int N, long long V, int Cin, int Cout) {
  int tps;
  const int ns = bwdw_slabs(N, V, &tps);
  return (size_t)N * Cout * 4 * sizeof(float) + (size_t)ns * 4 * ((size_t)Cout * Cin + Cout) * sizeof(float) + 256;
}

KMH_API int kmh_headcom_fwd(const float* feat, const float* w, const float* bias, float* pts, float* sums, float* sq,
                            int N, int D, int H, int W, int Cin, int Cout, void* ws, void* stream) {
  if (Cin > 64) return -22;
  hipStream_t s = (hipStream_t)stream;
  const long long V = (long long)D * H * W;
  int tps;
  const int ns = fwd_slabs(V, &tps);
  Dims d{D, H, W};
  headcom_fwd_kernel<<<dim3(ns, ceil_div(Cout, GC), N), HTPB, 0, s>>>(feat, w, bias, (double*)ws, V, Cin, Cout, d, tps,
                                                                     ns);
  headcom_final_kernel<<<ceil_div(N * Cout, 64), 64, 0, s>>>((const double*)ws, ns, N * Cout, pts, sums, sq);
  return KMH_LAUNCH_CHECK();
}

KMH_API int kmh_headcom_bwd(const float* dpts, const float* dpower, const float* feat, const float* w, const float* bias,
                            const float* sums, float* dfeat, float* dw, float* dbias, int N, int D, int H, int W,
                            int Cin, int Cout, int mask_dfeat, void* ws, void* stream) {
  if (Cin > 64) return -22;
  hipStream_t s = (hipStream_t)stream;
  const long long V = (long long)D * H * W;
  Dims d{D, H, W};
  float* g = (float*)ws;
  int tps;
// ... 115 lines not shown
  const HeadBfPlan p = head_bf_plan(N, V, Cout, TERMS);
  double* partial = (double*)ws;
  void* img = (char*)ws + align256((size_t)N * Cout * p.nslab_f * 5 * sizeof(double));
  float* hs = (float*)((char*)img + align256(p.img_bytes));
  int rc = head_scales<TERMS>(feat, (long long)N * V * Cin, w, (long long)Cout * Cin, hs, s);
  if (rc) return rc;
  rc = head_pack<TERMS>(w, Cout, Cin, p, img, hs, s);
  if (rc) return rc;
  Dims d{D, H, W};
  const size_t lds = 2 * ((size_t)TERMS * FVT * 128 + FVT * sizeof(float4));
  const bool rows = head_rows_ok(D, H, W);
  if (mask && !rows) return -22;
  auto kern = p.nwv == 16 ? (rows ? (amp ? headcom_fwd_bf_kernel<TERMS, true, 16, true> : headcom_fwd_bf_kernel<TERMS, true, 16>)
                                  : headcom_fwd_bf_kernel<TERMS, false, 16>)
                          : (rows ? (amp ? headcom_fwd_bf_kernel<TERMS, true, 4, true> : headcom_fwd_bf_kernel<TERMS, true, 4>)
                                  : headcom_fwd_bf_kernel<TERMS, false, 4>);
  hipError_t e = hipFuncSetAttribute((const void*)kern, hipFuncAttributeMaxDynamicSharedMemorySize, (int)lds);
  if (e != hipSuccess) return (int)e;
  kern<<<dim3(p.nslab_f * p.ngroups, N), 64 * p.nwv, lds, s>>>(feat, (const __bf16*)img, bias, partial, V, Cin, Cout, p.CoutP, d,
                                                         p.tps_f, p.nslab_f, p.ngroups, hs, sq != nullptr, mask);
  headcom_final_kernel<<<ceil_div(N * Cout, 64), 64, 0, s>>>(partial, p.nslab_f, N * Cout, pts, sums, sq);
  if (scales_out) head_scales_copy_kernel<<<1, 64, 0, s>>>(hs, scales_out);
  return KMH_LAUNCH_CHECK();
}

template <int TERMS>
static int head_bwd_bf(const float* dpts, const float* dpower, const float* feat, const float* w, const float* bias, const float* sums,
                       float* dfeat, float* dw, float* dbias, int N, int D, int H, int W, int Cin, int Cout,
                       int mask_dfeat, const float* scales_in, float* dfeat_scale2, const unsigned* mask, void* ws,
                       hipStream_t s, bool amp) {
  const long long V = (long long)D * H * W;
  if (mask && !head_rows_ok(D, H, W)) return -22;
  const HeadBfPlan p = head_bf_plan(N, V, Cout, TERMS);
  char* base = (char*)ws;
  float* g = (float*)base;
  base += align256((size_t)N * Cout * 4 * sizeof(float));
  void* img = base;
  base += align256(p.img_bytes);
  float* pw = (float*)base;
  float* pb = pw + (size_t)p.nslab_w * Cout * Cin;
  float* hs = (float*)((char*)pb + align256((size_t)p.nslab_w * Cout * sizeof(float)));
  const HeadBfPlan p3 = head_bf_plan(N, V, Cout, 3);
  void* img3 = (char*)hs + 256;
  float* hs3 = (float*)((char*)img3 + align256(p3.img_bytes));
  int* gate = TERMS == 2 ? (int*)((char*)hs3 + 128) : nullptr;
  int rc = head_scales<TERMS>(feat, (long long)N * V * Cin, w, (long long)Cout * Cin, hs, s, scales_in);
  if (rc) return rc;
  rc = head_pack<TERMS>(w, Cout, Cin, p, img, hs, s);
  if (rc) return rc;
  Dims d{D, H, W};
  headcom_coef_kernel<<<ceil_div(N * Cout, 64), 64, 0, s>>>(dpts, dpower, sums, N * Cout, g);
  if (TERMS == 2) head_dh_scale_kernel<<<1, 256, 0, s>>>(g, N * Cout, hs + 4, gate);

  auto launch = [&](auto tag, const HeadBfPlan& pl, const void* img_, const float* hs_, int want, bool amp) -> int {
    constexpr int T = decltype(tag)::value;
    const __bf16* wk = (const __bf16*)img_;
    const __bf16* wkp = wk + (size_t)T * pl.CoutP * 64;
    const __bf16* wt = wkp + (size_t)T * pl.CoutP * 64;
    if (dfeat && mask) {
      const size_t lds = 2 * ((size_t)T * 64 * 128 + 8 * WBLK * 16);
      auto kern = Cin > 32 ? (amp ? headcom_bwd_feat_mask_kernel<T, true, true> : headcom_bwd_feat_mask_kernel<T, true>)
                           : (amp ? headcom_bwd_feat_mask_kernel<T, false, true> : headcom_bwd_feat_mask_kernel<T, false>);
      hipError_t e = hipFuncSetAttribute((const void*)kern, hipFuncAttributeMaxDynamicSharedMemorySize, (int)lds);
      if (e != hipSuccess) return (int)e;
      kern<<<dim3(ceil_div(V, 256), N), BF_TPB, lds, s>>>(
          feat, wt, mask, g, dfeat, V, Cin, Cout, pl.CoutP, d, hs_, mask_dfeat, reinterpret_cast<unsigned*>(dfeat_scale2),
          gate, want);
    } else if (dfeat) {
      const size_t lds = 2 * ((size_t)2 * T * 64 * 128 + WBLK * 32);
      hipError_t e = hipFuncSetAttribute((const void*)headcom_bwd_feat_bf_kernel<T>,
                                         hipFuncAttributeMaxDynamicSharedMemorySize, (int)lds);
      if (e != hipSuccess) return (int)e;
      headcom_bwd_feat_bf_kernel<T><<<dim3(ceil_div(V, 256), N), BF_TPB, lds, s>>>(
          feat, wkp, wt, bias, g, dfeat, V, Cin, Cout, pl.CoutP, d, hs_, mask_dfeat,
          reinterpret_cast<unsigned*>(dfeat_scale2), gate, want);
    }
    if (dw && mask) {
      const size_t lds = 2 * ((size_t)T * 64 * 128);
      auto kern = pl.nwv_w == 8 ? (Cin > 32 ? (amp ? headcom_bwd_w_mask_kernel<T, 8, true, true> : headcom_bwd_w_mask_kernel<T, 8, true>)
                                            : (amp ? headcom_bwd_w_mask_kernel<T, 8, false, true> : headcom_bwd_w_mask_kernel<T, 8, false>))
                                : (Cin > 32 ? (amp ? headcom_bwd_w_mask_kernel<T, 4, true, true> : headcom_bwd_w_mask_kernel<T, 4, true>)
                                            : (amp ? headcom_bwd_w_mask_kernel<T, 4, false, true> : headcom_bwd_w_mask_kernel<T, 4, false>));
      hipError_t e = hipFuncSetAttribute((const void*)kern, hipFuncAttributeMaxDynamicSharedMemorySize, (int)lds);
      if (e != hipSuccess) return (int)e;
      kern<<<dim3(pl.nslab_w * pl.ngroups_w), 64 * pl.nwv_w, lds, s>>>(feat, mask, g, pw, pb, N, V, Cin, Cout, pl.CoutP, d,
                                                                      pl.tps_w, pl.ngroups_w, hs_, gate, want);
    } else if (dw) {
      const size_t lds = 2 * ((size_t)2 * T * WVT * 128 + WVT * sizeof(float4));
      const bool rows = W % 32 == 0 && V % WVT == 0 && V < (1ll << 31);
      auto kern = pl.nwv_w == 8 ? (rows ? headcom_bwd_w_bf_kernel<T, true, 8> : headcom_bwd_w_bf_kernel<T, false, 8>)
                                : (rows ? headcom_bwd_w_bf_kernel<T, true, 4> : headcom_bwd_w_bf_kernel<T, false, 4>);
      hipError_t e = hipFuncSetAttribute((const void*)kern, hipFuncAttributeMaxDynamicSharedMemorySize, (int)lds);
      if (e != hipSuccess) return (int)e;
      kern<<<dim3(pl.nslab_w * pl.ngroups_w), 64 * pl.nwv_w, lds, s>>>(feat, wk, bias, g, pw, pb, N, V, Cin, Cout, pl.CoutP,
                                                                      d, pl.tps_w, pl.ngroups_w, hs_, gate, want);
    }
    return KMH_LAUNCH_CHECK();
  };
  rc = launch(std::integral_constant<int, TERMS>{}, p, img, hs, 0, amp);
  if (rc) return rc;
  if (TERMS == 2) {
    head_scales_one_kernel<<<1, 64, 0, s>>>(hs3);
    rc = head_pack<3>(w, Cout, Cin, p3, img3, hs3, s);
    if (rc) return rc;
    rc = launch(std::integral_constant<int, 3>{}, p3, img3, hs3, 1, false);
    if (rc) return rc;
  }
  if (dfeat && dfeat_scale2) kmh_absmax::final_kernel<<<1, 1, 0, s>>>(dfeat_scale2, 0.f);
  if (dw) {
    int nb = ceil_div((long long)Cout * Cin, 64);
    if (nb > 2048) nb = 2048;
    headcom_reduce_kernel<<<nb, 256, 0, s>>>(pw, p.nslab_w, (long long)Cout * Cin, dw);
    if (dbias) headcom_reduce_kernel<<<ceil_div(Cout, 64), 256, 0, s>>>(pb, p.nslab_w, Cout, dbias);
  }
  return KMH_LAUNCH_CHECK();
}
}

KMH_API size_t kmh_headcom_fwd_bf_ws_bytes(int N, long long V, int Cout, int terms) {
  const HeadBfPlan p = head_bf_plan(N, V, Cout, terms);
  return align256((size_t)N * Cout * p.nslab_f * 5 * sizeof(double)) + align256(p.img_bytes) + 256;
}
KMH_API size_t kmh_headcom_bwd_bf_ws_bytes(int N, long long V, int Cin, int Cout, int terms) {
  const HeadBfPlan p = head_bf_plan(N, V, Cout, terms);
  const HeadBfPlan p3 = head_bf_plan(N, V, Cout, 3);
  return align256((size_t)N * Cout * 4 * sizeof(float)) + align256(p.img_bytes) +
         (size_t)p.nslab_w * (size_t)Cout * Cin * sizeof(float) + align256((size_t)p.nslab_w * Cout * sizeof(float)) + 512 +
         align256(p3.img_bytes) + 512;
}

KMH_API size_t kmh_headcom_mask_words(int N, int D, int H, int W, int Cout) {
  if (!head_rows_ok(D, H, W)) return 0;
  return (size_t)N * ((size_t)D * H * W / 32) * (size_t)(ceil_div(Cout, GC) * GC);
}
KMH_API int kmh_headcom_fwd_bf(const float* feat, const float* w, const float* bias, float* pts, float* sums, float* sq,
                               float* scales_out, int N, int D, int H, int W, int Cin, int Cout, int terms, unsigned* mask,
                               void* ws, void* stream) {
  const bool amp = kmh_take_amp(terms);
  if (Cin > 64 || (Cin & 3) || (terms != 2 && terms != 3)) return -22;
  return terms == 3
             ? head_fwd_bf<3>(feat, w, bias, pts, sums, sq, scales_out, N, D, H, W, Cin, Cout, mask, ws, (hipStream_t)stream, amp)
             : head_fwd_bf<2>(feat, w, bias, pts, sums, sq, scales_out, N, D, H, W, Cin, Cout, mask, ws, (hipStream_t)stream, amp);
}
KMH_API int kmh_headcom_bwd_bf(const float* dpts, const float* dpower, const float* feat, const float* w, const float* bias,
                               const float* sums, float* dfeat, float* dw, float* dbias, int N, int D, int H, int W,
                               int Cin, int Cout, int terms, int mask_dfeat, const float* scales_in,
                               float* dfeat_scale2, const unsigned* mask, void* ws, void* stream) {
  const bool amp = kmh_take_amp(terms);
  if (Cin > 64 || (Cin & 3) || (terms != 2 && terms != 3)) return -22;
  return terms == 3 ? head_bwd_bf<3>(dpts, dpower, feat, w, bias, sums, dfeat, dw, dbias, N, D, H, W, Cin, Cout,
                                     mask_dfeat, scales_in, dfeat_scale2, mask, ws, (hipStream_t)stream, amp)
                    : head_bwd_bf<2>(dpts, dpower, feat, w, bias, sums, dfeat, dw, dbias, N, D, H, W, Cin, Cout,
                                     mask_dfeat, scales_in, dfeat_scale2, mask, ws, (hipStream_t)stream, amp);
}
```

### keymorph_amd/csrc/norm.hip

```cpp
#include "common.h"
#include "absmax.h"
#include "stats_final.h"

namespace {

constexpr int TPB = 256;
constexpr int STAT_BLOCKS = 512;

template <int MODE, int VEC>
__global__ __launch_bounds__(TPB) void channel_stats_kernel(const float* __restrict__ a,
                                                            const float* __restrict__ b, long long V, int C,
                                                            double* __restrict__ partial,
                                                            const int* __restrict__ only_if) {
  if (only_if && *only_if == 0) return;
  extern __shared__ __attribute__((aligned(16))) double sred[];
  const int n = blockIdx.y;
  const int CQ = C / VEC;
  const int rows = TPB / CQ;
  const int q = threadIdx.x % CQ, vl = threadIdx.x / CQ;
  const bool active = vl < rows;
  const long long per = (V + gridDim.x - 1) / gridDim.x;
  const long long vbeg = per * blockIdx.x;
  long long vend = vbeg + per;
  if (vend > V) vend = V;
  double d0[VEC], d1[VEC];
  float f0[VEC], f1[VEC];
#pragma unroll
  for (int j = 0; j < VEC; ++j) { d0[j] = d1[j] = 0.0; f0[j] = f1[j] = 0.f; }
  if (active) {
    const float* ap = a + (long long)n * V * C + (long long)q * VEC;
    const float* bp = MODE ? b + (long long)n * V * C + (long long)q * VEC : nullptr;
    int cnt = 0;
    for (long long v = vbeg + vl; v < vend; v += rows) {
      float av[VEC], bv[VEC];
      if (VEC == 4) {
        const float4 t = *reinterpret_cast<const float4*>(ap + v * C);
        av[0] = t.x; av[1] = t.y; av[2] = t.z; av[3] = t.w;
        if (MODE) {
          const float4 u = *reinterpret_cast<const float4*>(bp + v * C);
          bv[0] = u.x; bv[1] = u.y; bv[2] = u.z; bv[3] = u.w;
        }
      } else {
        av[0] = ap[v * C];
        if (MODE) bv[0] = bp[v * C];
      }
#pragma unroll
      for (int j = 0; j < VEC; ++j) {
        f0[j] += av[j];
        f1[j] += MODE ? av[j] * bv[j] : av[j] * av[j];
      }
      if (++cnt == 64) {
#pragma unroll
// ... 96 lines not shown

__global__ void gn_bwd_coeffs_fold_kernel(const double* __restrict__ dstats, const double* __restrict__ bhat,
                                          const float* __restrict__ gamma, const float* __restrict__ beta,
                                          const float* __restrict__ mean_rstd, int N, int C, int G, double count,
                                          float* __restrict__ c123, float* __restrict__ dgamma,
                                          float* __restrict__ dbeta, int* __restrict__ fallback) {
  __shared__ int zero_gamma;
  if (threadIdx.x == 0) zero_gamma = 0;
  __syncthreads();
  for (int c = threadIdx.x; c < C; c += blockDim.x)
    if (gamma && gamma[c] == 0.f) zero_gamma = 1;
  __syncthreads();
  if (threadIdx.x == 0) *fallback = zero_gamma;
  if (zero_gamma) return;
  const int cpg = C / G;
  for (int ng = threadIdx.x; ng < N * G; ng += blockDim.x) {
    const int n = ng / G, g = ng % G;
    const double mean = mean_rstd[ng * 2], rstd = mean_rstd[ng * 2 + 1];
    double S1 = 0, S2 = 0;
    for (int c = g * cpg; c < (g + 1) * cpg; ++c) {
      const double ga = gamma ? (double)gamma[c] : 1.0, be = beta ? (double)beta[c] : 0.0;
      const double A = dstats[((long long)n * C + c) * 2], Bh = bhat[(long long)n * C + c];
      S1 += ga * A;
      S2 += Bh - be * A;
    }
    const double m = count * cpg;
    for (int c = g * cpg; c < (g + 1) * cpg; ++c) {
      const double ga = gamma ? (double)gamma[c] : 1.0;
      float* o = c123 + ((long long)n * C + c) * 3;
      o[0] = (float)(rstd * ga);
      o[1] = (float)(-rstd * rstd * S2 / m);
      o[2] = (float)(-rstd * S1 / m + rstd * rstd * S2 * mean / m);
    }
  }
  if (dgamma) {
    for (int c = threadIdx.x; c < C; c += blockDim.x) {
      const double ga = gamma ? (double)gamma[c] : 1.0, be = beta ? (double)beta[c] : 0.0;
      double dg = 0, db = 0;
      for (int n = 0; n < N; ++n) {
        const double A = dstats[((long long)n * C + c) * 2], Bh = bhat[(long long)n * C + c];
        dg += (Bh - be * A) / ga;
        db += A;
      }
      dgamma[c] += (float)dg;
      dbeta[c] += (float)db;
    }
  }
}

__global__ __launch_bounds__(TPB) void gn_bwd_apply_kernel(const float* dxn, const float* __restrict__ x,
                                                           const float* __restrict__ c123, long long V, int C,
                                                           int relu_mask, int accumulate, float* dx,
                                                           unsigned* __restrict__ amax ,
                                                           int out_blocked ) {
  const int n = blockIdx.y;
  const long long total = V * C;
  float mx = 0.f;
  const float* cc = c123 + (long long)n * C * 3;
  const long long base = (long long)n * total;
  if ((C & 3) == 0) {
    const long long t4 = total >> 2;
    for (long long e = (long long)blockIdx.x * TPB + threadIdx.x; e < t4; e += (long long)gridDim.x * TPB) {
      const int c = (int)((e * 4) % C);
      const float4 g = *reinterpret_cast<const float4*>(dxn + base + e * 4);
      const float4 xv = *reinterpret_cast<const float4*>(x + base + e * 4);
      float r[4];
      const float gg[4] = {g.x, g.y, g.z, g.w}, xx[4] = {xv.x, xv.y, xv.z, xv.w};
#pragma unroll
      for (int j = 0; j < 4; ++j) {
        float v = cc[(c + j) * 3] * gg[j] + cc[(c + j) * 3 + 1] * xx[j] + cc[(c + j) * 3 + 2];
        if (relu_mask && !(xx[j] > 0.f)) v = 0.f;
        r[j] = v;
      }
      float4* o = reinterpret_cast<float4*>(
          dx + base + (out_blocked ? ((long long)(c >> 3) * V + (e * 4) / C) * 8 + (c & 7) : e * 4));
      if (accumulate) { const float4 p = *o; r[0] += p.x; r[1] += p.y; r[2] += p.z; r[3] += p.w; }
      *o = make_float4(r[0], r[1], r[2], r[3]);
      mx = fmaxf(fmaxf(mx, fmaxf(fabsf(r[0]), fabsf(r[1]))), fmaxf(fabsf(r[2]), fabsf(r[3])));
    }
  } else {
    for (long long e = (long long)blockIdx.x * TPB + threadIdx.x; e < total; e += (long long)gridDim.x * TPB) {
      const int c = (int)(e % C);
      float v = cc[c * 3] * dxn[base + e] + cc[c * 3 + 1] * x[base + e] + cc[c * 3 + 2];
      if (relu_mask && !(x[base + e] > 0.f)) v = 0.f;
      v = accumulate ? dx[base + e] + v : v;
      dx[base + e] = v;
      mx = fmaxf(mx, fabsf(v));
    }
  }
  if (amax) {
    kmh_absmax::publish(mx, amax);
  }
}

__global__ __launch_bounds__(TPB) void norm_apply_kernel(const float* x, const float* __restrict__ scale,
                                                         const float* __restrict__ shift, long long V, int C,
                                                         int relu, float* y) {
  const int n = blockIdx.y;
  const long long total = V * C, base = (long long)n * total;
  const float* sc = scale + (long long)n * C;
  const float* sh = shift + (long long)n * C;
  if ((C & 3) == 0) {
    for (long long e = (long long)blockIdx.x * TPB + threadIdx.x; e < (total >> 2); e += (long long)gridDim.x * TPB) {
      const int c = (int)((e * 4) % C);
      float4 v = *reinterpret_cast<const float4*>(x + base + e * 4);
      v.x = v.x * sc[c] + sh[c]; v.y = v.y * sc[c + 1] + sh[c + 1];
      v.z = v.z * sc[c + 2] + sh[c + 2]; v.w = v.w * sc[c + 3] + sh[c + 3];
      if (relu) { v.x = fmaxf(v.x, 0.f); v.y = fmaxf(v.y, 0.f); v.z = fmaxf(v.z, 0.f); v.w = fmaxf(v.w, 0.f); }
      *reinterpret_cast<float4*>(y + base + e * 4) = v;
    }
  } else {
    for (long long e = (long long)blockIdx.x * TPB + threadIdx.x; e < total; e += (long long)gridDim.x * TPB) {
      const int c = (int)(e % C);
      float v = x[base + e] * sc[c] + sh[c];
      y[base + e] = relu ? fmaxf(v, 0.f) : v;
    }
  }
}

__global__ __launch_bounds__(TPB) void relu_mask_kernel(const float* __restrict__ dy, const float* __restrict__ y,
                                                        long long n, float* __restrict__ dz) {
  for (long long e = (long long)blockIdx.x * TPB + threadIdx.x; e < n; e += (long long)gridDim.x * TPB)
    dz[e] = y[e] > 0.f ? dy[e] : 0.f;
}


template <int VEC>
__global__ __launch_bounds__(TPB) void in_bwd_stats_kernel(const float* __restrict__ du, const float* __restrict__ z,
                                                           const float* __restrict__ scale, const float* __restrict__ shift,
                                                           long long V, int C, double* __restrict__ partial) {
  extern __shared__ __attribute__((aligned(16))) double sred[];
  const int n = blockIdx.y;
  const int CQ = C / VEC;
  const int rows = TPB / CQ;
  const int q = threadIdx.x % CQ, vl = threadIdx.x / CQ;
  const bool active = vl < rows;
  const long long per = (V + gridDim.x - 1) / gridDim.x;
  const long long vbeg = per * blockIdx.x;
  long long vend = vbeg + per;
  if (vend > V) vend = V;
  double d0[VEC], d1[VEC];
  float f0[VEC], f1[VEC], sc[VEC], sh[VEC];
#pragma unroll
  for (int j = 0; j < VEC; ++j) {
    d0[j] = d1[j] = 0.0; f0[j] = f1[j] = 0.f;
    sc[j] = active ? scale[(long long)n * C + q * VEC + j] : 0.f;
    sh[j] = active ? shift[(long long)n * C + q * VEC + j] : 0.f;
  }
  if (active) {
    const float* ap = du + (long long)n * V * C + (long long)q * VEC;
    const float* bp = z + (long long)n * V * C + (long long)q * VEC;
    int cnt = 0;
    for (long long v = vbeg + vl; v < vend; v += rows) {
      float av[VEC], bv[VEC];
      if (VEC == 4) {
        const float4 t = *reinterpret_cast<const float4*>(ap + v * C);
        const float4 u = *reinterpret_cast<const float4*>(bp + v * C);
        av[0] = t.x; av[1] = t.y; av[2] = t.z; av[3] = t.w;
        bv[0] = u.x; bv[1] = u.y; bv[2] = u.z; bv[3] = u.w;
      } else {
        av[0] = ap[v * C];
        bv[0] = bp[v * C];
      }
#pragma unroll
      for (int j = 0; j < VEC; ++j) {
        const float g = fmaf(bv[j], sc[j], sh[j]) > 0.f ? av[j] : 0.f;
        f0[j] += g;
        f1[j] += g * bv[j];
      }
      if (++cnt == 64) {
#pragma unroll
        for (int j = 0; j < VEC; ++j) { d0[j] += f0[j]; d1[j] += f1[j]; f0[j] = f1[j] = 0.f; }
        cnt = 0;
      }
    }
#pragma unroll
    for (int j = 0; j < VEC; ++j) { d0[j] += f0[j]; d1[j] += f1[j]; }
#pragma unroll
    for (int j = 0; j < VEC; ++j) {
      sred[((long long)vl * C + q * VEC + j) * 2] = d0[j];
      sred[((long long)vl * C + q * VEC + j) * 2 + 1] = d1[j];
    }
  }
  __syncthreads();
  for (int e = threadIdx.x; e < C * 2; e += TPB) {
    double s = 0;
    for (int r = 0; r < rows; ++r) s += sred[(long long)r * C * 2 + e];
    partial[((long long)n * gridDim.x + blockIdx.x) * C * 2 + e] = s;
  }
}

__global__ __launch_bounds__(TPB) void in_bwd_apply_kernel(const float* du, const float* __restrict__ z,
                                                           const float* __restrict__ scale, const float* __restrict__ shift,
                                                           const float* __restrict__ c123, long long V, int C, float* dz,
                                                           unsigned* __restrict__ amax) {
  const int n = blockIdx.y;
  const long long total = V * C, base = (long long)n * total;
  const float* cc = c123 + (long long)n * C * 3;
  const float* sc = scale + (long long)n * C;
  const float* sh = shift + (long long)n * C;
  float mx = 0.f;
  if ((C & 3) == 0) {
    const long long t4 = total >> 2;
    for (long long e = (long long)blockIdx.x * TPB + threadIdx.x; e < t4; e += (long long)gridDim.x * TPB) {
      const int c = (int)((e * 4) % C);
      const float4 g4 = *reinterpret_cast<const float4*>(du + base + e * 4);
      const float4 z4 = *reinterpret_cast<const float4*>(z + base + e * 4);
      const float gg[4] = {g4.x, g4.y, g4.z, g4.w}, zz[4] = {z4.x, z4.y, z4.z, z4.w};
      float r[4];
#pragma unroll
      for (int j = 0; j < 4; ++j) {
        const float g = fmaf(zz[j], sc[c + j], sh[c + j]) > 0.f ? gg[j] : 0.f;
        r[j] = cc[(c + j) * 3] * g + cc[(c + j) * 3 + 1] * zz[j] + cc[(c + j) * 3 + 2];
      }
      *reinterpret_cast<float4*>(dz + base + e * 4) = make_float4(r[0], r[1], r[2], r[3]);
      mx = fmaxf(fmaxf(mx, fmaxf(fabsf(r[0]), fabsf(r[1]))), fmaxf(fabsf(r[2]), fabsf(r[3])));
    }
  } else {
    for (long long e = (long long)blockIdx.x * TPB + threadIdx.x; e < total; e += (long long)gridDim.x * TPB) {
      const int c = (int)(e % C);
      const float zv = z[base + e];
      const float g = fmaf(zv, sc[c], sh[c]) > 0.f ? du[base + e] : 0.f;
      const float v = cc[c * 3] * g + cc[c * 3 + 1] * zv + cc[c * 3 + 2];
      dz[base + e] = v;
      mx = fmaxf(mx, fabsf(v));
    }
  }
  if (amax) kmh_absmax::publish(mx, amax);
}

__global__ __launch_bounds__(TPB) void in_bwd_apply_pool_kernel(const unsigned* __restrict__ argm, const float4* __restrict__ du,
                                                                const float4* __restrict__ z, const float* __restrict__ scale,
                                                                const float* __restrict__ shift, const float* __restrict__ c123,
                                                                float4* __restrict__ dz, int D, int H, int W, int C4, int Do,
                                                                int Ho, int Wo, unsigned* __restrict__ amax) {
  const int n = blockIdx.y;
  const int total = Do * Ho * Wo * C4;
  const long long V = (long long)D * H * W;
  const float4* zn = z + (long long)n * V * C4;
  float4* dzo = dz + (long long)n * V * C4;
  const float* cc = c123 + (long long)n * C4 * 12;
  const float* sc = scale + (long long)n * C4 * 4;
  const float* sh = shift + (long long)n * C4 * 4;
  float mx = 0.f;
  for (int e = blockIdx.x * TPB + threadIdx.x; e < total; e += gridDim.x * TPB) {
    const int c = e % C4, v = e / C4;
    const int xo = v % Wo, r = v / Wo, yo = r % Ho, zo = r / Ho;
    const unsigned a = argm[(long long)n * total + e];
    const float4 g = du[(long long)n * total + e];
    const int aw[4] = {(int)(a & 255), (int)((a >> 8) & 255), (int)((a >> 16) & 255), (int)(a >> 24)};
    const float gg[4] = {g.x, g.y, g.z, g.w};
    float k1[4], k2[4], k3[4], s1[4], s0[4];
#pragma unroll
    for (int j = 0; j < 4; ++j) {
      k1[j] = cc[(4 * c + j) * 3]; k2[j] = cc[(4 * c + j) * 3 + 1]; k3[j] = cc[(4 * c + j) * 3 + 2];
      s1[j] = sc[4 * c + j]; s0[j] = sh[4 * c + j];
    }
#pragma unroll
    for (int k = 0; k < 8; ++k) {
      const int zz = 2 * zo + (k >> 2), yy = 2 * yo + ((k >> 1) & 1), xx = 2 * xo + (k & 1);
      const long long o = ((long long)(zz * H + yy) * W + xx) * C4 + c;
      const float4 z4 = zn[o];
      const float zv[4] = {z4.x, z4.y, z4.z, z4.w};
      float t[4];
#pragma unroll
      for (int j = 0; j < 4; ++j) {
        const float gj = (k == aw[j] && fmaf(zv[j], s1[j], s0[j]) > 0.f) ? gg[j] : 0.f;
        t[j] = k1[j] * gj + k2[j] * zv[j] + k3[j];
      }
      dzo[o] = make_float4(t[0], t[1], t[2], t[3]);
      mx = fmaxf(fmaxf(mx, fmaxf(fabsf(t[0]), fabsf(t[1]))), fmaxf(fabsf(t[2]), fabsf(t[3])));
    }
  }
  if (amax) kmh_absmax::publish(mx, amax);
}

__global__ __launch_bounds__(TPB) void maxpool_fwd_kernel(const float* __restrict__ x, float* __restrict__ y,
                                                          unsigned char* __restrict__ arg , int D,
                                                          int H, int W, int C, int Do, int Ho, int Wo) {
  const int n = blockIdx.y;
  const long long total = (long long)Do * Ho * Wo * C;
  const float* xn = x + (long long)n * D * H * W * C;
  float* yn = y + (long long)n * total;
  for (long long e = (long long)blockIdx.x * TPB + threadIdx.x; e < total; e += (long long)gridDim.x * TPB) {
    const int c = (int)(e % C);
    long long v = e / C;
    const int xo = (int)(v % Wo), yo = (int)((v / Wo) % Ho), zo = (int)(v / ((long long)Wo * Ho));
    float m = -INFINITY;
    int am = 0;
#pragma unroll
    for (int k = 0; k < 8; ++k) {
      const int zz = 2 * zo + (k >> 2), yy = 2 * yo + ((k >> 1) & 1), xx = 2 * xo + (k & 1);
      const float val = xn[(((long long)zz * H + yy) * W + xx) * C + c];
      if (val > m || val != val) { m = val; am = k; }
    }
    yn[e] = m;
    if (arg) arg[(long long)n * total + e] = (unsigned char)am;
  }
}

__global__ __launch_bounds__(TPB) void maxpool_bwd_kernel(const float* __restrict__ x,
                                                          const unsigned char* __restrict__ argm ,
                                                          const float* __restrict__ dy, const float* add, int acs,
                                                          float* dx, int D, int H, int W, int C, int Do, int Ho, int Wo,
                                                          int out_blocked ) {
  const int n = blockIdx.y;
  const long long total = (long long)Do * Ho * Wo * C;
  const float* xn = x ? x + (long long)n * D * H * W * C : nullptr;
  float* dxn = dx + (long long)n * D * H * W * C;
  const float* an = add ? add + (long long)n * D * H * W * acs : nullptr;
  const float* dyn = dy + (long long)n * total;
  for (long long e = (long long)blockIdx.x * TPB + threadIdx.x; e < total; e += (long long)gridDim.x * TPB) {
    const int c = (int)(e % C);
    long long v = e / C;
    const int xo = (int)(v % Wo), yo = (int)((v / Wo) % Ho), zo = (int)(v / ((long long)Wo * Ho));
    int arg = 0;
    if (argm) {
      arg = argm[(long long)n * total + e];
    } else {
      float m = -INFINITY;
#pragma unroll
      for (int k = 0; k < 8; ++k) {
        const int zz = 2 * zo + (k >> 2), yy = 2 * yo + ((k >> 1) & 1), xx = 2 * xo + (k & 1);
        const float val = xn[(((long long)zz * H + yy) * W + xx) * C + c];
        if (val > m || val != val) { m = val; arg = k; }
      }
    }
// ... 87 lines not shown
      const int k = 2 * kk + dxx;
      const long long vox = ((long long)(2 * zo + (kk >> 1)) * H + 2 * yo + (kk & 1)) * W + 2 * xo + dxx;
      const float4 val = make_float4(k == a0 ? g.x : 0.f, k == a1 ? g.y : 0.f, k == a2 ? g.z : 0.f, k == a3 ? g.w : 0.f);
      *reinterpret_cast<float4*>(dxn + ((long long)chunk * V + vox) * 8 + 4 * qh) = val;
    }
  }
}

__global__ __launch_bounds__(TPB) void maxpool_bwd4_split_kernel(const unsigned* __restrict__ argm, const float4* __restrict__ dy,
                                                                 const float* __restrict__ scale2, float* __restrict__ dx, int D,
                                                                 int H, int W, int C4, int Do, int Ho, int Wo) {
  const int n = blockIdx.y;
  const long long V = (long long)D * H * W;
  const long long pooled = (long long)Do * Ho * Wo * C4;
  const int nchunk = C4 >> 1;
  float* dxn = dx + (long long)n * nchunk * (V + 1) * 8;
  const float S = scale2[0];
  if (blockIdx.x == 0) {
    for (int e = threadIdx.x; e < nchunk * 2; e += TPB)
      *reinterpret_cast<float4*>(dxn + ((long long)(e >> 1) * (V + 1) + V) * 8 + 4 * (e & 1)) = make_float4(0.f, 0.f, 0.f, 0.f);
  }
  const int ppr = Wo * 4;
  const long long total = (long long)nchunk * Do * Ho * ppr;
  for (long long e = (long long)blockIdx.x * TPB + threadIdx.x; e < total; e += (long long)gridDim.x * TPB) {
    const int p = (int)(e % ppr);
    const long long r = e / ppr;
    const int yo = (int)(r % Ho), zo = (int)((r / Ho) % Do), chunk = (int)(r / ((long long)Ho * Do));
    const int xo = p >> 2, dxx = (p >> 1) & 1, half = p & 1;
    const long long idx = (((long long)zo * Ho + yo) * Wo + xo) * C4 + 2 * chunk;
    const uint2 a2 = *reinterpret_cast<const uint2*>(argm + (long long)n * pooled + idx);
    const float4 g0 = dy[(long long)n * pooled + idx], g1 = dy[(long long)n * pooled + idx + 1];
    const float g[8] = {g0.x, g0.y, g0.z, g0.w, g1.x, g1.y, g1.z, g1.w};
    int a[8];
#pragma unroll
    for (int j = 0; j < 4; ++j) { a[j] = (a2.x >> (8 * j)) & 255; a[4 + j] = (a2.y >> (8 * j)) & 255; }
#pragma unroll
    for (int kk = 0; kk < 4; ++kk) {
      const int k = 2 * kk + dxx;
      const long long vox = ((long long)(2 * zo + (kk >> 1)) * H + 2 * yo + (kk & 1)) * W + 2 * xo + dxx;
      float val[8];
#pragma unroll
      for (int j = 0; j < 8; ++j) val[j] = fmaf(k == a[j] ? g[j] : 0.f, S, 0.f);
      kmh_bf16x8 parts[2];
      split8<2>(val, parts);
      *reinterpret_cast<kmh_bf16x8*>(dxn + ((long long)chunk * (V + 1) + vox) * 8 + 4 * half) = half ? parts[1] : parts[0];
    }
  }
}

__global__ __launch_bounds__(TPB) void maxpool_bwd4_lazy_kernel(const unsigned* __restrict__ argm, const float4* __restrict__ dy,
                                                                const float4* __restrict__ dxn, const float4* __restrict__ x,
                                                                const float* __restrict__ c123, float4* __restrict__ dx,
                                                                int D, int H, int W, int C4, int Do, int Ho, int Wo,
                                                                unsigned* __restrict__ amax) {
  const int n = blockIdx.y;
  const int total = Do * Ho * Wo * C4;
  const long long V = (long long)D * H * W;
  const float4* gn = dxn + (long long)n * V * C4;
  const float4* xn = x + (long long)n * V * C4;
  float4* dxo = dx + (long long)n * V * C4;
  const float* cc = c123 + (long long)n * C4 * 12;
  float mx = 0.f;
  for (int e = blockIdx.x * TPB + threadIdx.x; e < total; e += gridDim.x * TPB) {
    const int c = e % C4, v = e / C4;
    const int xo = v % Wo, r = v / Wo, yo = r % Ho, zo = r / Ho;
    const unsigned a = argm[(long long)n * total + e];
    const float4 g = dy[(long long)n * total + e];
    const int a0 = a & 255, a1 = (a >> 8) & 255, a2 = (a >> 16) & 255, a3 = a >> 24;
    float k1[4], k2[4], k3[4];
#pragma unroll
    for (int j = 0; j < 4; ++j) { k1[j] = cc[(4 * c + j) * 3]; k2[j] = cc[(4 * c + j) * 3 + 1]; k3[j] = cc[(4 * c + j) * 3 + 2]; }
#pragma unroll
    for (int k = 0; k < 8; ++k) {
      const int zz = 2 * zo + (k >> 2), yy = 2 * yo + ((k >> 1) & 1), xx = 2 * xo + (k & 1);
      const long long o = ((long long)(zz * H + yy) * W + xx) * C4 + c;
      const float4 d4 = gn[o], x4 = xn[o];
      const float dd[4] = {d4.x, d4.y, d4.z, d4.w}, xv[4] = {x4.x, x4.y, x4.z, x4.w};
      float s4[4];
#pragma unroll
      for (int j = 0; j < 4; ++j) {
        float t = k1[j] * dd[j] + k2[j] * xv[j] + k3[j];
        if (!(xv[j] > 0.f)) t = 0.f;
        s4[j] = t;
      }
      float4 val = make_float4(k == a0 ? g.x : 0.f, k == a1 ? g.y : 0.f, k == a2 ? g.z : 0.f, k == a3 ? g.w : 0.f);
      val.x += s4[0]; val.y += s4[1]; val.z += s4[2]; val.w += s4[3];
      dxo[o] = val;
      mx = fmaxf(fmaxf(mx, fmaxf(fabsf(val.x), fabsf(val.y))), fmaxf(fabsf(val.z), fabsf(val.w)));
    }
  }
  if (amax) kmh_absmax::publish(mx, amax);
}

__device__ __forceinline__ int nearest_src(int dst, int in_size, int out_size) {
  const float scale = (float)in_size / (float)out_size;
  int s = (int)floorf((float)dst * scale);
  return s < in_size - 1 ? s : in_size - 1;
}

__global__ __launch_bounds__(TPB) void upcat_fwd_kernel(const float* __restrict__ skip, const float* __restrict__ low,
                                                        float* __restrict__ out, int D, int H, int W, int Cs, int Dl,
                                                        int Hl, int Wl, int Cl) {
  const int n = blockIdx.y;
  const int C = Cs + Cl;
  const long long total = (long long)D * H * W * C;
  for (long long e = (long long)blockIdx.x * TPB + threadIdx.x; e < total; e += (long long)gridDim.x * TPB) {
    const int c = (int)(e % C);
    const long long v = e / C;
    float val;
    if (c < Cs) {
      val = skip[((long long)n * D * H * W + v) * Cs + c];
    } else {
      const int xx = (int)(v % W), yy = (int)((v / W) % H), zz = (int)(v / ((long long)W * H));
      const int xs = nearest_src(xx, Wl, W), ys = nearest_src(yy, Hl, H), zs = nearest_src(zz, Dl, D);
      val = low[((((long long)n * Dl + zs) * Hl + ys) * Wl + xs) * Cl + (c - Cs)];
    }
    out[(long long)n * total + e] = val;
  }
}

__global__ __launch_bounds__(TPB) void upcat_fwd4_kernel(const float4* __restrict__ skip, const float4* __restrict__ low,
                                                         float4* __restrict__ out, int D, int H, int W, int Cs4, int Dl,
                                                         int Hl, int Wl, int Cl4) {
  const int n = blockIdx.y;
  const unsigned C4 = Cs4 + Cl4;
  const unsigned V = (unsigned)D * H * W;
  const unsigned long long total = (unsigned long long)V * C4;
  for (unsigned long long e = (unsigned long long)blockIdx.x * TPB + threadIdx.x; e < total;
       e += (unsigned long long)gridDim.x * TPB) {
    const unsigned v = (unsigned)(e / C4), c = (unsigned)(e - (unsigned long long)v * C4);
    float4 val;
    if (c < (unsigned)Cs4) {
      val = skip[((unsigned long long)n * V + v) * Cs4 + c];
    } else {
      const unsigned xx = v % W, t = v / W, yy = t % H, zz = t / H;
      const int xs = nearest_src(xx, Wl, W), ys = nearest_src(yy, Hl, H), zs = nearest_src(zz, Dl, D);
      val = low[((((unsigned long long)n * Dl + zs) * Hl + ys) * Wl + xs) * Cl4 + (c - Cs4)];
    }
    out[(unsigned long long)n * total + e] = val;
  }
}

__global__ __launch_bounds__(TPB) void upcat_bwd_low2x4_kernel(const float4* __restrict__ dout, float4* __restrict__ dlow,
                                                               int H, int W, int Cs4, int Dl, int Hl, int Wl, int Cl4) {
// ... 94 lines not shown
  }
}

static inline int stream_blocks(long long elems) {
  int nb = ceil_div(elems, (long long)TPB * 8);
  if (nb > 4096) nb = 4096;
  return nb < 1 ? 1 : nb;
}

}

KMH_API size_t kmh_channel_stats_ws_bytes(int N, int C) {
  return (size_t)N * STAT_BLOCKS * C * 2 * sizeof(double);
}

KMH_API int kmh_channel_stats(const float* a, const float* b, int mode, int N, long long V, int C, double* out,
                              void* ws, const int* only_if, void* stream) {
  hipStream_t s = (hipStream_t)stream;
  if (C > TPB * 4) return -22;
  int nblk = ceil_div(V, 2048);
  if (nblk > STAT_BLOCKS) nblk = STAT_BLOCKS;
  if (nblk < 1) nblk = 1;
  const bool v4 = (C % 4 == 0) && (C / 4 <= TPB);
  const int CQ = v4 ? C / 4 : C;
  if (CQ > TPB) return -22;
  const int rows = TPB / CQ;
  const size_t lds = (size_t)rows * C * 2 * sizeof(double);
  if (lds > 64 * 1024) return -22;
  dim3 g(nblk, N);
  if (v4) {
    if (mode == 0) channel_stats_kernel<0, 4><<<g, TPB, lds, s>>>(a, b, V, C, (double*)ws, only_if);
    else channel_stats_kernel<1, 4><<<g, TPB, lds, s>>>(a, b, V, C, (double*)ws, only_if);
  } else {
    if (mode == 0) channel_stats_kernel<0, 1><<<g, TPB, lds, s>>>(a, b, V, C, (double*)ws, only_if);
    else channel_stats_kernel<1, 1><<<g, TPB, lds, s>>>(a, b, V, C, (double*)ws, only_if);
  }
  kmh_stats::final_kernel<<<dim3(ceil_div(C * 2, 256 / kWave), N), 256, 0, s>>>((const double*)ws, nblk, C, out, only_if);
  return KMH_LAUNCH_CHECK();
}

KMH_API int kmh_gn_fwd_coeffs(const double* stats, const float* gamma, const float* beta, int N, int C, int G,
                              double count, float eps, float* scale, float* shift, float* mean_rstd,
                              float* ascale, void* stream) {
  if (G <= 0 || C % G) return -22;
  gn_fwd_coeffs_kernel<<<N, 64, 0, (hipStream_t)stream>>>(stats, gamma, beta, C, G, count, eps, scale, shift,
                                                         mean_rstd, ascale);
  return KMH_LAUNCH_CHECK();
}

KMH_API int kmh_absmax_scale(const float* x, long long n, float min_abs, float* out2, void* stream) {
  return kmh_absmax::launch(x, n, min_abs, out2, (hipStream_t)stream);
}

KMH_API int kmh_gn_bwd_coeffs(const double* ab, const float* gamma, const float* mean_rstd, int N, int C, int G,
                              double count, float* c123, float* dgamma, float* dbeta, const int* only_if, void* stream) {
  if (G <= 0 || C % G) return -22;
  gn_bwd_coeffs_kernel<<<1, 256, 0, (hipStream_t)stream>>>(ab, gamma, mean_rstd, N, C, G, count, c123, dgamma,
                                                          dbeta, only_if);
  return KMH_LAUNCH_CHECK();
}

KMH_API int kmh_gn_bwd_coeffs_fold(const double* dstats, const double* bhat, const float* gamma, const float* beta,
                                   const float* mean_rstd, int N, int C, int G, double count, float* c123,
                                   float* dgamma, float* dbeta, int* fallback, void* stream) {
  if (G <= 0 || C % G || !fallback) return -22;
  gn_bwd_coeffs_fold_kernel<<<1, 256, 0, (hipStream_t)stream>>>(dstats, bhat, gamma, beta, mean_rstd, N, C, G, count,
                                                               c123, dgamma, dbeta, fallback);
  return KMH_LAUNCH_CHECK();
}

KMH_API int kmh_gn_bwd_apply(const float* dxn, const float* x, const float* c123, int N, long long V, int C,
                             int relu_mask, int accumulate, float* dx, float* dx_scale2, int out_blocked, void* stream) {
  hipStream_t s = (hipStream_t)stream;
  if (out_blocked && ((C & 7) || dx == dxn || dx == x)) return -22;
  gn_bwd_apply_kernel<<<dim3(stream_blocks(V * C / 4), N), TPB, 0, s>>>(dxn, x, c123, V, C, relu_mask, accumulate, dx,
                                                                      reinterpret_cast<unsigned*>(dx_scale2), out_blocked);
  if (dx_scale2) kmh_absmax::final_kernel<<<1, 1, 0, s>>>(dx_scale2, 0.f);
  return KMH_LAUNCH_CHECK();
}

__device__ __forceinline__ const float* dz_quad(const float* dn, long long vox, int c, int Cout, long long V, int in_blocked) {
  return in_blocked ? dn + ((long long)(c >> 3) * V + vox) * 8 + (c & 7) : dn + vox * Cout + c;
}

__global__ __launch_bounds__(256, 3) void up2_boxsum_kernel(const float* __restrict__ dz, float* __restrict__ G, int Dl,
                                                            int Hl, int Wl, int Cout, int in_blocked) {
  const int n = blockIdx.y;
  const int cq = Cout >> 2;
  const long long total = (long long)Dl * Hl * Wl * 3 * cq;
  const int D = 2 * Dl, H = 2 * Hl, W = 2 * Wl;
  const float* dn = dz + (long long)n * D * H * W * Cout;
  float* gn = G + (long long)n * Dl * Hl * Wl * 27 * Cout;
  for (long long e = (long long)blockIdx.x * 256 + threadIdx.x; e < total; e += (long long)gridDim.x * 256) {
    const int q = (int)(e % cq);
    const int kz = (int)((e / cq) % 3);
    const long long m = e / (3 * cq);
    const int mx = (int)(m % Wl), my = (int)((m / Wl) % Hl), mz = (int)(m / ((long long)Wl * Hl));
    float4 Y[3][3];
#pragma unroll
    for (int a = 0; a < 9; ++a) (&Y[0][0])[a] = make_float4(0.f, 0.f, 0.f, 0.f);
#pragma unroll
    for (int dzp = 0; dzp < 2; ++dzp) {
      const int uz = 2 * mz - 1 + (2 - kz) + dzp;
#pragma unroll
      for (int iy = 0; iy < 4; ++iy) {
        const int uy = 2 * my - 1 + iy;
        float4 a4[4];
#pragma unroll
        for (int ix = 0; ix < 4; ++ix) {
          const int ux = 2 * mx - 1 + ix;
          a4[ix] = make_float4(0.f, 0.f, 0.f, 0.f);
          if ((unsigned)ux < (unsigned)W && (unsigned)uy < (unsigned)H && (unsigned)uz < (unsigned)D)
            a4[ix] = *reinterpret_cast<const float4*>(dz_quad(dn, ((long long)uz * H + uy) * W + ux, 4 * q, Cout,
                                                              (long long)D * H * W, in_blocked));
        }
#pragma unroll
        for (int kx = 0; kx < 3; ++kx) {
          const float4 u = a4[2 - kx], v = a4[3 - kx];
          const float4 xs = make_float4(u.x + v.x, u.y + v.y, u.z + v.z, u.w + v.w);
#pragma unroll
          for (int ky = 0; ky < 3; ++ky)
            if (iy == 2 - ky || iy == 3 - ky) {
              Y[ky][kx].x += xs.x; Y[ky][kx].y += xs.y; Y[ky][kx].z += xs.z; Y[ky][kx].w += xs.w;
            }
        }
      }
    }
    float* o = gn + (m * 27 + kz * 9) * Cout + 4 * q;
#pragma unroll
    for (int a = 0; a < 9; ++a) *reinterpret_cast<float4*>(o + (long long)a * Cout) = (&Y[0][0])[a];
// ... 50 lines not shown
          }
      }
    }
  }
  const long long mg = ((long long)mz * Hl + my) * Wl + mx;
  float* o = G + ((long long)n * Dl * Hl * Wl * 27 + mg * 27 + kz * 9) * Cout + c;
#pragma unroll
  for (int a = 0; a < 9; ++a) *reinterpret_cast<float4*>(o + (long long)a * Cout) = (&Y[0][0])[a];
}

KMH_API int kmh_up2_boxsum(const float* dz, float* G, int N, int Dl, int Hl, int Wl, int Cout, int in_blocked, void* stream) {
  if ((Cout & 3) || (in_blocked && (Cout & 7))) return -22;
  const int tx = (Wl + BT_X - 1) / BT_X, ty = (Hl + BT_Y - 1) / BT_Y, tz = (Dl + BT_Z - 1) / BT_Z;
  const int chunks = (Cout + 4 * BT_CQ - 1) / (4 * BT_CQ);
  if ((long long)tx * ty * tz < (1ll << 31) && chunks < 65536 && N < 65536) {
    up2_boxsum_tiled_kernel<<<dim3(tx * ty * tz, chunks, N), BT_TPB, 0, (hipStream_t)stream>>>(dz, G, Dl, Hl, Wl, Cout, tx, ty, in_blocked);
    return KMH_LAUNCH_CHECK();
  }
  const long long total = (long long)Dl * Hl * Wl * 3 * (Cout / 4);
  up2_boxsum_kernel<<<dim3(stream_blocks(total), N), 256, 0, (hipStream_t)stream>>>(dz, G, Dl, Hl, Wl, Cout, in_blocked);
  return KMH_LAUNCH_CHECK();
}

KMH_API int kmh_norm_apply(const float* x, const float* scale, const float* shift, int N, long long V, int C,
                           int relu, float* y, void* stream) {
  norm_apply_kernel<<<dim3(stream_blocks(V * C / 4), N), TPB, 0, (hipStream_t)stream>>>(x, scale, shift, V, C, relu,
                                                                                       y);
  return KMH_LAUNCH_CHECK();
}

KMH_API int kmh_in_bwd_stats(const float* du, const float* z, const float* scale, const float* shift, int N, long long V,
                             int C, double* out, void* ws, void* stream) {
  hipStream_t s = (hipStream_t)stream;
  if (C > TPB * 4) return -22;
  int nblk = ceil_div(V, 2048);
  if (nblk > STAT_BLOCKS) nblk = STAT_BLOCKS;
  if (nblk < 1) nblk = 1;
  const bool v4 = (C % 4 == 0) && (C / 4 <= TPB);
  const int CQ = v4 ? C / 4 : C;
  if (CQ > TPB) return -22;
  const int rows = TPB / CQ;
  const size_t lds = (size_t)rows * C * 2 * sizeof(double);
  if (lds > 64 * 1024) return -22;
  dim3 g(nblk, N);
  if (v4) in_bwd_stats_kernel<4><<<g, TPB, lds, s>>>(du, z, scale, shift, V, C, (double*)ws);
  else in_bwd_stats_kernel<1><<<g, TPB, lds, s>>>(du, z, scale, shift, V, C, (double*)ws);
  kmh_stats::final_kernel<<<dim3(ceil_div(C * 2, 256 / kWave), N), 256, 0, s>>>((const double*)ws, nblk, C, out, nullptr);
  return KMH_LAUNCH_CHECK();
}

KMH_API int kmh_in_bwd_apply(const float* du, const float* z, const float* scale, const float* shift, const float* c123,
                             int N, long long V, int C, float* dz, float* dz_scale2, void* stream) {
  hipStream_t s = (hipStream_t)stream;
  if (dz_scale2) {
    hipError_t e = hipMemsetAsync(dz_scale2, 0, 2 * sizeof(float), s);
    if (e != hipSuccess) return (int)e;
  }
  in_bwd_apply_kernel<<<dim3(stream_blocks(V * C / 4), N), TPB, 0, s>>>(du, z, scale, shift, c123, V, C, dz,
                                                                       reinterpret_cast<unsigned*>(dz_scale2));
  if (dz_scale2) kmh_absmax::final_kernel<<<1, 1, 0, s>>>(dz_scale2, 0.f);
  return KMH_LAUNCH_CHECK();
}

KMH_API int kmh_in_bwd_apply_pool(const unsigned char* argmax, const float* du, const float* z, const float* scale,
                                  const float* shift, const float* c123, int N, int D, int H, int W, int C, float* dz,
                                  float* dz_scale2, void* stream) {
  const int Do = D / 2, Ho = H / 2, Wo = W / 2;
  const long long pooled = (long long)Do * Ho * Wo * C;
  if (!argmax || !du || !z || !c123 || !dz || (C & 3) || (D & 1) || (H & 1) || (W & 1)) return -22;
  if (pooled / 4 >= (1ll << 31) || (long long)D * H * W >= (1ll << 31)) return -22;
  if ((((uintptr_t)du | (uintptr_t)z | (uintptr_t)dz) & 15) || ((uintptr_t)argmax & 3)) return -22;
  hipStream_t s = (hipStream_t)stream;
  if (dz_scale2) {
    hipError_t e = hipMemsetAsync(dz_scale2, 0, 2 * sizeof(float), s);
    if (e != hipSuccess) return (int)e;
  }
  in_bwd_apply_pool_kernel<<<dim3(stream_blocks(pooled), N), TPB, 0, s>>>(
      (const unsigned*)argmax, (const float4*)du, (const float4*)z, scale, shift, c123, (float4*)dz, D, H, W, C / 4, Do, Ho, Wo,
      reinterpret_cast<unsigned*>(dz_scale2));
  if (dz_scale2) kmh_absmax::final_kernel<<<1, 1, 0, s>>>(dz_scale2, 0.f);
  return KMH_LAUNCH_CHECK();
}

KMH_API int kmh_relu_mask(const float* dy, const float* y, long long n, float* dz, void* stream) {
  relu_mask_kernel<<<stream_blocks(n), TPB, 0, (hipStream_t)stream>>>(dy, y, n, dz);
  return KMH_LAUNCH_CHECK();
}

KMH_API int kmh_maxpool3d_fwd(const float* x, float* y, unsigned char* argmax, int N, int D, int H, int W, int C,
                              void* stream) {
  const int Do = D / 2, Ho = H / 2, Wo = W / 2;
  const long long pooled = (long long)Do * Ho * Wo * C;
  if ((C & 3) == 0 && pooled / 4 < (1ll << 31) && (long long)D * H * W < (1ll << 31))
    maxpool_fwd4_kernel<<<dim3(stream_blocks(pooled), N), TPB, 0, (hipStream_t)stream>>>(
        (const float4*)x, (float4*)y, (unsigned*)argmax, D, H, W, C / 4, Do, Ho, Wo);
  else
    maxpool_fwd_kernel<<<dim3(stream_blocks(pooled), N), TPB, 0, (hipStream_t)stream>>>(x, y, argmax, D, H, W, C, Do, Ho, Wo);
  return KMH_LAUNCH_CHECK();
}

KMH_API int kmh_maxpool3d_bwd(const float* x, const unsigned char* argmax, const float* dy, const float* add,
                              int add_cstride, float* dx, int N, int D, int H, int W, int C, int out_blocked, void* stream) {
  const int Do = D / 2, Ho = H / 2, Wo = W / 2;
  if ((add && add_cstride < C) || (!x && !argmax)) return -22;
  if (out_blocked && ((C & 7) || (D & 1) || (H & 1) || (W & 1) || add == dx)) return -22;
  const long long pooled = (long long)Do * Ho * Wo * C;
  const bool aligned = (((uintptr_t)add | (uintptr_t)dx | (uintptr_t)dy) & 15) == 0 && ((uintptr_t)argmax & 3) == 0;
  if (argmax && aligned && (C & 3) == 0 && (add_cstride & 3) == 0 && pooled / 4 < (1ll << 31) &&
      (long long)D * H * W < (1ll << 31)) {
    if (out_blocked && !add) {
      maxpool_bwd4_rows_kernel<<<dim3(stream_blocks(pooled), N), TPB, 0, (hipStream_t)stream>>>(
          (const unsigned*)argmax, (const float4*)dy, dx, D, H, W, C / 4, Do, Ho, Wo);
      return KMH_LAUNCH_CHECK();
    }
    auto kern = out_blocked ? maxpool_bwd4_kernel<true> : maxpool_bwd4_kernel<false>;
    kern<<<dim3(stream_blocks(pooled), N), TPB, 0, (hipStream_t)stream>>>((const unsigned*)argmax, (const float4*)dy, add,
                                                                         add_cstride, dx, D, H, W, C / 4, Do, Ho, Wo);
  } else {
    maxpool_bwd_kernel<<<dim3(stream_blocks(pooled), N), TPB, 0, (hipStream_t)stream>>>(
        x, argmax, dy, add, add_cstride, dx, D, H, W, C, Do, Ho, Wo, out_blocked);
  }
  return KMH_LAUNCH_CHECK();
}

KMH_API size_t kmh_maxpool3d_bwd_split_bytes(int N, int D, int H, int W, int C) {
  return (size_t)N * (C / 8) * ((size_t)D * H * W + 1) * 32;
}
KMH_API int kmh_maxpool3d_bwd_split(const unsigned char* argmax, const float* dy, const float* dy_scale2, float* dxs, int N,
                                    int D, int H, int W, int C, void* stream) {
  const int Do = D / 2, Ho = H / 2, Wo = W / 2;
  const long long pooled = (long long)Do * Ho * Wo * C;
  if (!argmax || !dy || !dy_scale2 || !dxs || (C & 7) || (D & 1) || (H & 1) || (W & 1) || N <= 0 || D <= 0 || H <= 0 || W <= 0)
    return -22;
  if (pooled / 4 >= (1ll << 31) || (long long)D * H * W >= (1ll << 31)) return -22;
  if ((((uintptr_t)dxs | (uintptr_t)dy) & 15) || ((uintptr_t)argmax & 7)) return -22;
  maxpool_bwd4_split_kernel<<<dim3(stream_blocks(pooled), N), TPB, 0, (hipStream_t)stream>>>(
      (const unsigned*)argmax, (const float4*)dy, dy_scale2, dxs, D, H, W, C / 4, Do, Ho, Wo);
  return KMH_LAUNCH_CHECK();
}

KMH_API int kmh_maxpool3d_bwd_lazy(const unsigned char* argmax, const float* dy, const float* dxn, const float* x,
                                   const float* c123, float* dx, int N, int D, int H, int W, int C, float* dx_scale2,
                                   void* stream) {
  const int Do = D / 2, Ho = H / 2, Wo = W / 2;
  const long long pooled = (long long)Do * Ho * Wo * C;
  if (!argmax || !dy || !dxn || !x || !c123 || !dx || (C & 3) || (D & 1) || (H & 1) || (W & 1)) return -22;
  if (pooled / 4 >= (1ll << 31) || (long long)D * H * W >= (1ll << 31)) return -22;
  if ((((uintptr_t)dxn | (uintptr_t)x | (uintptr_t)dx | (uintptr_t)dy) & 15) || ((uintptr_t)argmax & 3)) return -22;
  hipStream_t s = (hipStream_t)stream;
  if (dx_scale2) {
    hipError_t e = hipMemsetAsync(dx_scale2, 0, 2 * sizeof(float), s);
    if (e != hipSuccess) return (int)e;
  }
  maxpool_bwd4_lazy_kernel<<<dim3(stream_blocks(pooled), N), TPB, 0, s>>>(
      (const unsigned*)argmax, (const float4*)dy, (const float4*)dxn, (const float4*)x, c123, (float4*)dx, D, H, W, C / 4, Do,
      Ho, Wo, reinterpret_cast<unsigned*>(dx_scale2));
  if (dx_scale2) kmh_absmax::final_kernel<<<1, 1, 0, s>>>(dx_scale2, 0.f);
  return KMH_LAUNCH_CHECK();
}

KMH_API int kmh_upcat_fwd(const float* skip, const float* low, float* out, int N, int D, int H, int W, int Cs,
                          int Dl, int Hl, int Wl, int Cl, void* stream) {
  if (((Cs | Cl) & 3) == 0 && (long long)D * H * W < (1ll << 32))
    upcat_fwd4_kernel<<<dim3(stream_blocks((long long)D * H * W * (Cs + Cl) / 4), N), TPB, 0, (hipStream_t)stream>>>(
        (const float4*)skip, (const float4*)low, (float4*)out, D, H, W, Cs / 4, Dl, Hl, Wl, Cl / 4);
  else
    upcat_fwd_kernel<<<dim3(stream_blocks((long long)D * H * W * (Cs + Cl)), N), TPB, 0, (hipStream_t)stream>>>(
        skip, low, out, D, H, W, Cs, Dl, Hl, Wl, Cl);
  return KMH_LAUNCH_CHECK();
}

KMH_API int kmh_upcat_bwd(const float* dout, float* dskip, float* dlow, int N, int D, int H, int W, int Cs, int Dl,
                          int Hl, int Wl, int Cl, int accumulate_skip, void* stream) {
  hipStream_t s = (hipStream_t)stream;
  const long long V = (long long)D * H * W;
  if (dskip)
    upcat_bwd_skip_kernel<<<dim3(stream_blocks(V * Cs), N), TPB, 0, s>>>(dout, dskip, V, Cs, Cs + Cl,
                                                                       accumulate_skip);
  if (((Cs | Cl) & 3) == 0 && D == 2 * Dl && H == 2 * Hl && W == 2 * Wl && V < (1ll << 32))
    upcat_bwd_low2x4_kernel<<<dim3(stream_blocks((long long)Dl * Hl * Wl * Cl / 4), N), TPB, 0, s>>>(
        (const float4*)dout, (float4*)dlow, H, W, Cs / 4, Dl, Hl, Wl, Cl / 4);
  else
    upcat_bwd_low_kernel<<<dim3(stream_blocks((long long)Dl * Hl * Wl * Cl), N), TPB, 0, s>>>(dout, dlow, D, H, W,
                                                                                             Cs, Dl, Hl, Wl, Cl);
  return KMH_LAUNCH_CHECK();
}

KMH_API int kmh_layout_convert(const float* in, float* out, int N, long long V, int C, int to_ncdhw,
                               void* stream) {
  dim3 g(ceil_div(V, 32), ceil_div(C, 32), N);
  nchw_to_nhwc_kernel<<<g, 256, 0, (hipStream_t)stream>>>(in, out, V, C, to_ncdhw);
  return KMH_LAUNCH_CHECK();
}
```

### keymorph_amd/parallel.py

```python
from __future__ import annotations

import os
from typing import Iterable, List

import torch
import torch.distributed as dist

from . import _lib
from ._lib import check
from .ops import _p, _stream


def init_distributed():
    world = int(os.environ.get("WORLD_SIZE", "1"))
    rank = int(os.environ.get("RANK", "0"))
    local = int(os.environ.get("LOCAL_RANK", "0"))
    if os.environ.get("KEYMORPH_SHARE_GPU") == "1":
        local = 0
    if world > 1 and not dist.is_initialized():
        os.environ.setdefault("MASTER_ADDR", "127.0.0.1")
        os.environ.setdefault("MASTER_PORT", "29500")
        backend = os.environ.get("KEYMORPH_DIST_BACKEND") or ("nccl" if torch.cuda.is_available() else "gloo")
        if torch.cuda.is_available():
            torch.cuda.set_device(local)
        dist.init_process_group(backend=backend, rank=rank, world_size=world)
    return rank, local, world


def shard_indices(num_items: int, rank: int, world: int) -> List[int]:
    base, rem = divmod(num_items, world)
    start = rank * base + min(rank, rem)
    return list(range(start, start + base + (1 if rank < rem else 0)))


class FlatParams:

    def __init__(self, params: Iterable[torch.nn.Parameter]):
        self.params = [p for p in params if p.requires_grad]
        n = sum(p.numel() for p in self.params)
        dev = self.params[0].device
        self.flat = torch.empty(n, dtype=torch.float32, device=dev)
        self._grad = torch.zeros(n, dtype=torch.float32, device=dev)
        self._views = []
        o = 0
        for p in self.params:
            k = p.numel()
            self.flat[o:o + k].copy_(p.data.reshape(-1))
            p.data = self.flat[o:o + k].view_as(p.data)
            v = self._grad[o:o + k].view_as(p.data)
            p.grad = v
            self._views.append(v)
            o += k
        self.numel = n

    def zero_grad(self):
        for p in self.params:
            p.grad = None

    def gather(self) -> torch.Tensor:
        src, dst, zero = [], [], []
        for p, v in zip(self.params, self._views):
            g = p.grad
            if g is None:
                zero.append(v)
            elif g.data_ptr() != v.data_ptr():
                src.append(g.detach().reshape(v.shape).to(v.dtype))
                dst.append(v)
            p.grad = v
        with torch.no_grad():
            if zero:
                torch._foreach_zero_(zero)
            if dst:
                torch._foreach_copy_(dst, src)
        return self._grad

    @property
    def grad(self) -> torch.Tensor:
        return self.gather()

    def broadcast(self, src: int = 0):
        if dist.is_initialized() and dist.get_world_size() > 1:
            dist.broadcast(self.flat, src)

    def allreduce_grads(self) -> float:
        g = self.gather()
        if dist.is_initialized() and dist.get_world_size() > 1:
            dist.all_reduce(g, op=dist.ReduceOp.SUM)
            return 1.0 / dist.get_world_size()
        return 1.0


class FusedAdam:

    def __init__(self, flat: FlatParams, lr=1e-3, betas=(0.9, 0.999), eps=1e-8):
        self.flat, self.lr, self.betas, self.eps = flat, lr, betas, eps
        self.m = torch.zeros_like(flat.flat)
        self.v = torch.zeros_like(flat.flat)
        self.t = 0

    def state_dict(self):
        state, o = {}, 0
        for i, p in enumerate(self.flat.params):
            k = p.numel()
            state[i] = {"step": torch.tensor(float(self.t)), "exp_avg": self.m[o:o + k].view_as(p).clone(),
                        "exp_avg_sq": self.v[o:o + k].view_as(p).clone()}
            o += k
        group = {"lr": self.lr, "betas": tuple(self.betas), "eps": self.eps, "weight_decay": 0, "amsgrad": False,
                 "maximize": False, "foreach": None, "capturable": False, "differentiable": False, "fused": None,
                 "params": list(range(len(self.flat.params)))}
        return {"state": state, "param_groups": [group]}

    def load_state_dict(self, sd):
        groups = sd["param_groups"]
        assert len(groups) == 1 and len(groups[0]["params"]) == len(self.flat.params), "parameter list mismatch"
        g = groups[0]
        assert not g.get("amsgrad", False) and not g.get("weight_decay", 0), "plain Adam only"
        self.lr, self.betas, self.eps = g["lr"], tuple(g["betas"]), g["eps"]
        o, steps = 0, set()
        for i, p in zip(g["params"], self.flat.params):
            k = p.numel()
            st = sd["state"].get(i)
            if st is None:
                self.m[o:o + k].zero_(); self.v[o:o + k].zero_()
            else:
                self.m[o:o + k].copy_(st["exp_avg"].reshape(-1))
                self.v[o:o + k].copy_(st["exp_avg_sq"].reshape(-1))
                steps.add(int(st["step"]))
            o += k
        assert len(steps) <= 1, "per-parameter step counts differ"
        self.t = steps.pop() if steps else 0

    def step(self, grad_scale: float = 1.0):
        self.t += 1
        lib = _lib.load()
        check(lib.kmh_adam_step(_p(self.flat.flat), _p(self.flat.gather()), _p(self.m), _p(self.v), self.flat.numel,
                                self.lr, self.betas[0], self.betas[1], self.eps, self.t, grad_scale, _stream()),
              "kmh_adam_step")


def gather_group_points(local_points: torch.Tensor, num_subjects: int) -> torch.Tensor:
    if not (dist.is_initialized() and dist.get_world_size() > 1):
        assert local_points.shape[0] == num_subjects
        return local_points
    world, rank = dist.get_world_size(), dist.get_rank()
    counts = [len(shard_indices(num_subjects, r, world)) for r in range(world)]
    assert local_points.shape[0] == counts[rank], "this rank's block does not match shard_indices()"
    m = max(counts)
    pad = local_points.new_zeros((m,) + tuple(local_points.shape[1:]))
    pad[: counts[rank]] = local_points
    outs = [torch.empty_like(pad) for _ in range(world)]
    dist.all_gather(outs, pad.contiguous())
    return torch.cat([o[:c] for o, c in zip(outs, counts)], dim=0)


def allgather_points(points: torch.Tensor) -> torch.Tensor:
    if not (dist.is_initialized() and dist.get_world_size() > 1):
        return points
    outs = [torch.empty_like(points) for _ in range(dist.get_world_size())]
    dist.all_gather(outs, points.contiguous())
    return torch.cat(outs, dim=0)
```

Measured before the change: 15.99.

## Fold range-scale finish into last workgroup and batch weight absmax per step

```diff
diff --git a/include/keymorph_hip.h b/include/keymorph_hip.h
--- a/include/keymorph_hip.h
+++ b/include/keymorph_hip.h
@@ -200,6 +200,7 @@
 int kmh_gn_fwd_coeffs(const double* stats, const float* gamma, const float* beta, int N, int C, int G, double count,
                       float eps, float* scale, float* shift, float* mean_rstd, float* ascale, void* stream);
 int kmh_absmax_scale(const float* x, long long n, float min_abs, float* out2, void* stream);
+int kmh_absmax_segments(const float* flat, const long long* table, int nseg, long long max_len, float* out, void* stream);
 int kmh_gn_bwd_coeffs(const double* ab, const float* gamma, const float* mean_rstd, int N, int C, int G,
                       double count, float* c123, float* dgamma, float* dbeta, const int* only_if, void* stream);
 int kmh_gn_bwd_coeffs_fold(const double* dstats, const double* bhat, const float* gamma, const float* beta,
diff --git a/keymorph_amd/_handoff.py b/keymorph_amd/_handoff.py
--- a/keymorph_amd/_handoff.py
+++ b/keymorph_amd/_handoff.py
@@ -1,4 +1,4 @@
-KEYS = ("stats", "grad_scale", "layout", "lazy_gn", "up_sources", "packed")
+KEYS = ("stats", "grad_scale", "layout", "lazy_gn", "up_sources", "packed", "wscale")
 _ATTR = "_kmh_handoff"
 
 
diff --git a/keymorph_amd/_lib.py b/keymorph_amd/_lib.py
--- a/keymorph_amd/_lib.py
+++ b/keymorph_amd/_lib.py
@@ -113,6 +113,7 @@
     "kmh_channel_stats": (_i, [_f, _f, _i, _i, _ll, _i, _f, _f, _f, _f]),
     "kmh_gn_fwd_coeffs": (_i, [_f, _f, _f, _i, _i, _i, C.c_double, C.c_float, _f, _f, _f, _f, _f]),
     "kmh_absmax_scale": (_i, [_f, _ll, C.c_float, _f, _f]),
+    "kmh_absmax_segments": (_i, [_f, _f, _i, _ll, _f, _f]),
     "kmh_gn_bwd_coeffs": (_i, [_f, _f, _f, _i, _i, _i, C.c_double, _f, _f, _f, _f, _f]),
     "kmh_gn_bwd_coeffs_fold": (_i, [_f, _f, _f, _f, _f, _i, _i, _i, C.c_double, _f, _f, _f, _f, _f]),
     "kmh_gn_bwd_apply": (_i, [_f, _f, _f, _i, _ll, _i, _i, _i, _f, _f, _i, _f]),
diff --git a/keymorph_amd/backbone_ops.py b/keymorph_amd/backbone_ops.py
--- a/keymorph_amd/backbone_ops.py
+++ b/keymorph_amd/backbone_ops.py
@@ -40,6 +40,7 @@
     "KEYMORPH_NO_LAZY_FIRST": "GroupNorm backward of the first block as its own pass",
     "KEYMORPH_NO_LAZY_SKIP": "GroupNorm's backward of a decoder skip applied in the decoder",
     "KEYMORPH_NO_LAZY_IN": "ConvNet block by block: separate norm / ReLU / pooling passes",
+    "KEYMORPH_NO_FINAL_FOLD": "range scales finished by launches of their own (zero-fill, measure, finish) instead of the measuring kernel's last workgroup",
     "KEYMORPH_RANGE_AUDIT": "debug (ON = audit): per-sample dynamic range of every gradient operand, RANGE_AUDIT_LOG",
 }
 
@@ -141,6 +142,12 @@
     if t is None:
         t = _CONSTS[key] = torch.tensor(values, dtype=torch.float32, device=device)
     return t
+
+
+def _scale_slot(dev) -> Tensor:
+    if _off("KEYMORPH_NO_FINAL_FOLD"):
+        return torch.zeros(2, dtype=torch.float32, device=dev)
+    return _f32((2,), dev)
 
 
 def absmax_scale(x: Tensor, min_abs: float = 0.0) -> Tensor:
@@ -232,6 +239,9 @@
     return (scale, shift, mr, ascale) if want_ascale else (scale, shift, mr)
 
 
+WSCALE_STATS = {"carried": 0, "measured": 0}
+
+
 def pack_weight(w: Tensor, transposed: bool, wscale: Optional[Tensor] = None, terms: int = 0) -> Tensor:
     lib = _lib.load()
     Cout, Cin = w.shape[:2]
@@ -239,7 +249,11 @@
         terms = terms or _TERMS[CONV_MODE]
         out = torch.empty(int(lib.kmh_conv3d_pack_bf_bytes(Cout, Cin, int(transposed), terms)), dtype=torch.uint8,
                           device=w.device)
-        wscale = (wscale if wscale is not None else absmax_scale(w)) if terms == 2 else None
+        if terms == 2 and wscale is None:
+            wscale = peek(w, "wscale") if not _off("KEYMORPH_NO_FINAL_FOLD") else None
+            WSCALE_STATS["carried" if wscale is not None else "measured"] += 1
+            wscale = wscale if wscale is not None else absmax_scale(w)
+        wscale = wscale if terms == 2 else None
         attach(out, "packed", (terms, wscale))
         check(lib.kmh_conv3d_pack_weight_bf(_p(w), _p(out), Cout, Cin, int(transposed), terms, _p(wscale), _stream()),
               "kmh_conv3d_pack_weight_bf")
@@ -608,7 +622,7 @@
                             None, N, D, H, W, Cout, Cin, False, False,
                             mask=ymask, ascale=dscale, in_blocked=kind, stats_out=dstats,
                             winners=ctx.pool_arg if dy_sparse else None)
-            sc2 = torch.zeros(2, dtype=torch.float32, device=x.device) if (_needs_range_scales() and ctx.needs_input_grad[0]) else None
+            sc2 = _scale_slot(x.device) if (_needs_range_scales() and ctx.needs_input_grad[0]) else None
             c123, dgamma, dbeta = _gn_bwd_coeffs(lambda flag: channel_stats(dxn, x, N, V, Cin, only_if=flag), gamma, mr,
                                                  N, Cin, G, V, fold=(dstats, bhat, beta) if fold else None)
             if ctx.needs_input_grad[0] and dx_lazy:
@@ -738,8 +752,8 @@
         c123, dgamma, dbeta = _gn_bwd_coeffs(ab, gamma, mr, N, C, G, V, fold=(dstats, bhat, beta))
         c_s = c123[:, :Cs].contiguous()
         c_l = (c123[:, Cs:] * _const(dy.device, 1.0, 8.0, 8.0)).contiguous()
-        sc_s = torch.zeros(2, dtype=torch.float32, device=dy.device) if _needs_range_scales() else None
-        sc_l = torch.zeros(2, dtype=torch.float32, device=dy.device) if _needs_range_scales() else None
+        sc_s = _scale_slot(dy.device) if _needs_range_scales() else None
+        sc_l = _scale_slot(dy.device) if _needs_range_scales() else None
         dskip = dlow = None
         if ctx.needs_input_grad[0] and ctx.dskip_lazy:
             dskip = dxn_s
@@ -877,7 +891,7 @@
             c123, x = lazy
             N, D, H, W, C = ctx.xshape
             dxn = _prep(dskip)
-            sc2 = torch.zeros(2, dtype=torch.float32, device=dxn.device) if _needs_range_scales() else None
+            sc2 = _scale_slot(dxn.device) if _needs_range_scales() else None
             if dy is None:
                 return _gn_bwd_apply(dxn, x, c123, N, D * H * W, C, sc2)
             (arg,) = ctx.saved_tensors
@@ -1140,7 +1154,7 @@
                                _stream()), "kmh_in_bwd_stats")
     c123, _, _ = _gn_bwd_coeffs(ab, None, mr, N, C, C, Dp * Hp * Wp)
     out = g if in_place else torch.empty_like(zprev)
-    sc2 = torch.zeros(2, dtype=torch.float32, device=g.device) if _needs_range_scales() else None
+    sc2 = _scale_slot(g.device) if _needs_range_scales() else None
     if arg is not None:
         check(lib.kmh_in_bwd_apply_pool(_p(arg), _p(g), _p(zprev), _p(scale), _p(shift), _p(c123), N, Dp, Hp, Wp, C, _p(out),
                                         _p(sc2), _stream()), "kmh_in_bwd_apply_pool")
@@ -1297,8 +1311,7 @@
         if CONV_MODE != "f32" and Cin % 4 == 0:
             terms = _HEAD_TERMS[CONV_MODE]
             ws = workspace(int(lib.kmh_headcom_bwd_bf_ws_bytes(N, D * H * W, Cin, Cout, terms)), feat.device, "head")
-            dsc = (torch.zeros(2, dtype=torch.float32, device=feat.device)
-                   if (terms == 2 and dfeat is not None) else None)
+            dsc = _scale_slot(feat.device) if (terms == 2 and dfeat is not None) else None
             check(lib.kmh_headcom_bwd_bf(_p(dpts), _p(dpower), _p(feat), _p(w), _p(b), _p(sums), _p(dfeat), _p(dw), _p(db), N, D, H,
                                          W, Cin, Cout, _t(terms), ctx.mask_dfeat, _p(ctx.hsc), _p(dsc), _p(ctx.hmask), _p(ws), _stream()),
                   "kmh_headcom_bwd_bf")
diff --git a/keymorph_amd/csrc/absmax.h b/keymorph_amd/csrc/absmax.h
--- a/keymorph_amd/csrc/absmax.h
+++ b/keymorph_amd/csrc/absmax.h
@@ -1,41 +1,126 @@
 #pragma once
+#include <stdlib.h>
 #include "common.h"
 
+extern "C" unsigned* kmh_absmax_scratch(void* stream);
+
 namespace kmh_absmax {
+constexpr int kPairs = 128;
+static inline bool folded() {
+  const char* e = getenv("KEYMORPH_NO_FINAL_FOLD");
+  return !(e && *e);
+}
+template <bool PERFORMED = false>
 __device__ __forceinline__ void publish(float m, unsigned* acc) {
   m = wave_max(m);
   if ((threadIdx.x & 63) == 0) {
     const unsigned bits = __float_as_uint(m);
-    if (bits > __hip_atomic_load(acc, __ATOMIC_RELAXED, __HIP_MEMORY_SCOPE_AGENT)) atomicMax(acc, bits);
+    if (bits > __hip_atomic_load(acc, __ATOMIC_RELAXED, __HIP_MEMORY_SCOPE_AGENT)) {
+      atomicMax(acc, bits);
+      if (PERFORMED) asm volatile("s_waitcnt vmcnt(0)" ::: "memory");
+    }
   }
 }
-__global__ __launch_bounds__(256) static void partial_kernel(const float* __restrict__ x, long long n,
-                                                             unsigned* __restrict__ acc) {
+constexpr int kShards = 64;
+constexpr int kPairWord = 32 * (1 + kShards);
+constexpr size_t kScratchBytes = (size_t)(kPairWord + 32 * kPairs) * sizeof(unsigned);
+
+__device__ __forceinline__ void finish_if_last(unsigned* acc, unsigned* ticket, unsigned nblocks, float* out2, float min_abs) {
+  if (__hip_atomic_fetch_add(ticket, 1u, __ATOMIC_RELAXED, __HIP_MEMORY_SCOPE_AGENT) != nblocks - 1) return;
+  const unsigned bits = __hip_atomic_exchange(acc, 0u, __ATOMIC_RELAXED, __HIP_MEMORY_SCOPE_AGENT);
+  __hip_atomic_store(ticket, 0u, __ATOMIC_RELAXED, __HIP_MEMORY_SCOPE_AGENT);
+  range_scale(fmaxf(__uint_as_float(bits), min_abs), out2);
+}
+__device__ __forceinline__ void publish_tail(float m, unsigned* sc, float* out2, float min_abs) {
+  if (!out2) return publish(m, sc);
+  publish<true>(m, sc);
+  __syncthreads();
+  if (threadIdx.x == 0) {
+    const unsigned total = gridDim.x * gridDim.y * gridDim.z;
+    const unsigned id = blockIdx.x + gridDim.x * (blockIdx.y + gridDim.y * blockIdx.z);
+    const unsigned g = id % kShards;
+    const unsigned in_shard = (total - g + kShards - 1) / kShards;
+    unsigned* shard = sc + 32 * (1 + g);
+    if (__hip_atomic_fetch_add(shard, 1u, __ATOMIC_RELAXED, __HIP_MEMORY_SCOPE_AGENT) == in_shard - 1) {
+      __hip_atomic_store(shard, 0u, __ATOMIC_RELAXED, __HIP_MEMORY_SCOPE_AGENT);
+      finish_if_last(sc, sc + 1, total < kShards ? total : kShards, out2, min_abs);
+    }
+  }
+}
+__device__ __forceinline__ void publish_tail_pair(float m, unsigned* pair, unsigned nblocks, float* out2) {
+  publish<true>(m, pair);
+  __syncthreads();
+  if (threadIdx.x == 0) finish_if_last(pair, pair + 1, nblocks, out2, 0.f);
+}
+__device__ __forceinline__ float block_absmax(const float* __restrict__ x, long long n, unsigned bid, unsigned nblk) {
   float m = 0.f;
   long long head = (long long)(((16 - (reinterpret_cast<unsigned long long>(x) & 15)) & 15) >> 2);
   if (head > n) head = n;
   const float* xb = x + head;
   const long long nb = n - head, n4 = nb >> 2;
-  for (long long i = (long long)blockIdx.x * 256 + threadIdx.x; i < n4; i += (long long)gridDim.x * 256) {
+  for (long long i = (long long)bid * 256 + threadIdx.x; i < n4; i += (long long)nblk * 256) {
     const float4 v = reinterpret_cast<const float4*>(xb)[i];
     m = fmaxf(fmaxf(m, fmaxf(fabsf(v.x), fabsf(v.y))), fmaxf(fabsf(v.z), fabsf(v.w)));
   }
-  if (blockIdx.x == 0) {
+  if (bid == 0) {
     for (long long i = threadIdx.x; i < head; i += 256) m = fmaxf(m, fabsf(x[i]));
     for (long long i = (n4 << 2) + threadIdx.x; i < nb; i += 256) m = fmaxf(m, fabsf(xb[i]));
   }
-  publish(m, acc);
+  return m;
+}
+__global__ __launch_bounds__(256) static void partial_kernel(const float* __restrict__ x, long long n,
+                                                             unsigned* __restrict__ acc, float* __restrict__ out2,
+                                                             float min_abs) {
+  publish_tail(block_absmax(x, n, blockIdx.x, gridDim.x), acc, out2, min_abs);
+}
+__global__ __launch_bounds__(256) static void segments_kernel(const float* __restrict__ flat,
+                                                              const long long* __restrict__ table,
+                                                              unsigned* __restrict__ acc, float* __restrict__ out) {
+  const int i = blockIdx.y;
+  const long long n = table[2 * i + 1];
+  long long nb = (n / 4 + 256) / 256;
+  if (nb > gridDim.x) nb = gridDim.x;
+  if (blockIdx.x >= nb) return;
+  publish_tail_pair(block_absmax(flat + table[2 * i], n, blockIdx.x, (unsigned)nb), acc + kPairWord + 32 * i, (unsigned)nb,
+                    out + 2 * i);
 }
 __global__ static void final_kernel(float* __restrict__ out2, float min_abs) {
   const float m = fmaxf(__uint_as_float(reinterpret_cast<unsigned*>(out2)[0]), min_abs);
   range_scale(m, out2);
 }
+
+struct Tail {
+  unsigned* acc = nullptr;
+  float* out2 = nullptr;
+  float* legacy = nullptr;
+  int open(float* scale2, bool zeroed_by_caller, hipStream_t s) {
+    if (!scale2) return 0;
+    if (folded()) {
+      acc = kmh_absmax_scratch(s);
+      out2 = scale2;
+      return acc ? 0 : (int)hipErrorOutOfMemory;
+    }
+    acc = reinterpret_cast<unsigned*>(scale2);
+    legacy = scale2;
+    return zeroed_by_caller ? 0 : (int)hipMemsetAsync(scale2, 0, 2 * sizeof(float), s);
+  }
+  void close(hipStream_t s) const {
+    if (legacy) final_kernel<<<1, 1, 0, s>>>(legacy, 0.f);
+  }
+};
+
 static inline int launch(const float* x, long long n, float min_abs, float* out2, hipStream_t s) {
+  long long nb = (n / 4 + 256) / 256;
+  if (nb > 2048) nb = 2048;
+  if (folded()) {
+    unsigned* acc = kmh_absmax_scratch(s);
+    if (!acc) return (int)hipErrorOutOfMemory;
+    partial_kernel<<<(int)nb, 256, 0, s>>>(x, n, acc, out2, min_abs);
+    return (int)hipGetLastError();
+  }
   hipError_t e = hipMemsetAsync(out2, 0, 2 * sizeof(float), s);
   if (e != hipSuccess) return (int)e;
-  long long nb = (n / 4 + 256) / 256;
-  if (nb > 2048) nb = 2048;
-  partial_kernel<<<(int)nb, 256, 0, s>>>(x, n, reinterpret_cast<unsigned*>(out2));
+  partial_kernel<<<(int)nb, 256, 0, s>>>(x, n, reinterpret_cast<unsigned*>(out2), nullptr, 0.f);
   final_kernel<<<1, 1, 0, s>>>(out2, min_abs);
   return (int)hipGetLastError();
 }
diff --git a/keymorph_amd/csrc/headcom.hip b/keymorph_amd/csrc/headcom.hip
--- a/keymorph_amd/csrc/headcom.hip
+++ b/keymorph_amd/csrc/headcom.hip
@@ -765,6 +765,7 @@
                                                                         int Cin, int Cout, int CoutP, Dims d,
                                                                         const float* __restrict__ hs, int mask_dfeat,
                                                                         unsigned* __restrict__ amax ,
+                                                                        float* __restrict__ amax_out2 ,
                                                                         const int* __restrict__ gate, int want) {
   if (gate && *gate != want) return;
   extern __shared__ __attribute__((aligned(16))) unsigned char hsm[];
@@ -914,7 +915,7 @@
         }
       }
   }
-  if (amax) kmh_absmax::publish(mxo, amax);
+  if (amax) kmh_absmax::publish_tail(mxo, amax, amax_out2, 0.f);
 }
 
 template <int TERMS, int NWV, bool WIDE, bool AMP = false>
@@ -1041,7 +1042,8 @@
 __global__ __launch_bounds__(BF_TPB, 2) void headcom_bwd_feat_mask_kernel(
     const float* __restrict__ feat, const __bf16* __restrict__ wt, const unsigned* __restrict__ mask,
     const float* __restrict__ g, float* __restrict__ dfeat, long long V, int Cin, int Cout, int CoutP, Dims d,
-    const float* __restrict__ hs, int mask_dfeat, unsigned* __restrict__ amax, const int* __restrict__ gate, int want) {
+    const float* __restrict__ hs, int mask_dfeat, unsigned* __restrict__ amax, float* __restrict__ amax_out2,
+    const int* __restrict__ gate, int want) {
   if (gate && *gate != want) return;
   extern __shared__ __attribute__((aligned(16))) unsigned char hsm[];
   constexpr int IMG = TERMS * 64 * 128;
@@ -1165,7 +1167,7 @@
         }
       }
   }
-  if (amax) kmh_absmax::publish(mxo, amax);
+  if (amax) kmh_absmax::publish_tail(mxo, amax, amax_out2, 0.f);
 }
 
 
@@ -1387,6 +1389,8 @@
   headcom_coef_kernel<<<ceil_div(N * Cout, 64), 64, 0, s>>>(dpts, dpower, sums, N * Cout, g);
   if (TERMS == 2) head_dh_scale_kernel<<<1, 256, 0, s>>>(g, N * Cout, hs + 4, gate);
 
+  kmh_absmax::Tail tail;
+  if (int trc = tail.open(dfeat ? dfeat_scale2 : nullptr, true, s)) return trc;
   auto launch = [&](auto tag, const HeadBfPlan& pl, const void* img_, const float* hs_, int want, bool amp) -> int {
     constexpr int T = decltype(tag)::value;
     const __bf16* wk = (const __bf16*)img_;
@@ -1399,16 +1403,14 @@
       hipError_t e = hipFuncSetAttribute((const void*)kern, hipFuncAttributeMaxDynamicSharedMemorySize, (int)lds);
       if (e != hipSuccess) return (int)e;
       kern<<<dim3(ceil_div(V, 256), N), BF_TPB, lds, s>>>(
-          feat, wt, mask, g, dfeat, V, Cin, Cout, pl.CoutP, d, hs_, mask_dfeat, reinterpret_cast<unsigned*>(dfeat_scale2),
-          gate, want);
+          feat, wt, mask, g, dfeat, V, Cin, Cout, pl.CoutP, d, hs_, mask_dfeat, tail.acc, tail.out2, gate, want);
     } else if (dfeat) {
       const size_t lds = 2 * ((size_t)2 * T * 64 * 128 + WBLK * 32);
       hipError_t e = hipFuncSetAttribute((const void*)headcom_bwd_feat_bf_kernel<T>,
                                          hipFuncAttributeMaxDynamicSharedMemorySize, (int)lds);
       if (e != hipSuccess) return (int)e;
       headcom_bwd_feat_bf_kernel<T><<<dim3(ceil_div(V, 256), N), BF_TPB, lds, s>>>(
-          feat, wkp, wt, bias, g, dfeat, V, Cin, Cout, pl.CoutP, d, hs_, mask_dfeat,
-          reinterpret_cast<unsigned*>(dfeat_scale2), gate, want);
+          feat, wkp, wt, bias, g, dfeat, V, Cin, Cout, pl.CoutP, d, hs_, mask_dfeat, tail.acc, tail.out2, gate, want);
     }
     if (dw && mask) {
       const size_t lds = 2 * ((size_t)T * 64 * 128);
@@ -1441,7 +1443,7 @@
     rc = launch(std::integral_constant<int, 3>{}, p3, img3, hs3, 1, false);
     if (rc) return rc;
   }
-  if (dfeat && dfeat_scale2) kmh_absmax::final_kernel<<<1, 1, 0, s>>>(dfeat_scale2, 0.f);
+  tail.close(s);
   if (dw) {
     int nb = ceil_div((long long)Cout * Cin, 64);
     if (nb > 2048) nb = 2048;
diff --git a/keymorph_amd/csrc/norm.hip b/keymorph_amd/csrc/norm.hip
--- a/keymorph_amd/csrc/norm.hip
+++ b/keymorph_amd/csrc/norm.hip
@@ -1,3 +1,6 @@
+#include <map>
+#include <mutex>
+#include <utility>
 #include "common.h"
 #include "absmax.h"
 #include "stats_final.h"
@@ -200,6 +203,7 @@
                                                            const float* __restrict__ c123, long long V, int C,
                                                            int relu_mask, int accumulate, float* dx,
                                                            unsigned* __restrict__ amax ,
+                                                           float* __restrict__ amax_out2 ,
                                                            int out_blocked ) {
   const int n = blockIdx.y;
   const long long total = V * C;
@@ -237,7 +241,7 @@
     }
   }
   if (amax) {
-    kmh_absmax::publish(mx, amax);
+    kmh_absmax::publish_tail(mx, amax, amax_out2, 0.f);
   }
 }
 
@@ -341,7 +345,7 @@
 __global__ __launch_bounds__(TPB) void in_bwd_apply_kernel(const float* du, const float* __restrict__ z,
                                                            const float* __restrict__ scale, const float* __restrict__ shift,
                                                            const float* __restrict__ c123, long long V, int C, float* dz,
-                                                           unsigned* __restrict__ amax) {
+                                                           unsigned* __restrict__ amax, float* __restrict__ amax_out2) {
   const int n = blockIdx.y;
   const long long total = V * C, base = (long long)n * total;
   const float* cc = c123 + (long long)n * C * 3;
@@ -374,14 +378,15 @@
       mx = fmaxf(mx, fabsf(v));
     }
   }
-  if (amax) kmh_absmax::publish(mx, amax);
+  if (amax) kmh_absmax::publish_tail(mx, amax, amax_out2, 0.f);
 }
 
 __global__ __launch_bounds__(TPB) void in_bwd_apply_pool_kernel(const unsigned* __restrict__ argm, const float4* __restrict__ du,
                                                                 const float4* __restrict__ z, const float* __restrict__ scale,
                                                                 const float* __restrict__ shift, const float* __restrict__ c123,
                                                                 float4* __restrict__ dz, int D, int H, int W, int C4, int Do,
-                                                                int Ho, int Wo, unsigned* __restrict__ amax) {
+                                                                int Ho, int Wo, unsigned* __restrict__ amax,
+                                                                float* __restrict__ amax_out2) {
   const int n = blockIdx.y;
   const int total = Do * Ho * Wo * C4;
   const long long V = (long long)D * H * W;
@@ -420,7 +425,7 @@
       mx = fmaxf(fmaxf(mx, fmaxf(fabsf(t[0]), fabsf(t[1]))), fmaxf(fabsf(t[2]), fabsf(t[3])));
     }
   }
-  if (amax) kmh_absmax::publish(mx, amax);
+  if (amax) kmh_absmax::publish_tail(mx, amax, amax_out2, 0.f);
 }
 
 __global__ __launch_bounds__(TPB) void maxpool_fwd_kernel(const float* __restrict__ x, float* __restrict__ y,
@@ -614,7 +619,7 @@
                                                                 const float4* __restrict__ dxn, const float4* __restrict__ x,
                                                                 const float* __restrict__ c123, float4* __restrict__ dx,
                                                                 int D, int H, int W, int C4, int Do, int Ho, int Wo,
-                                                                unsigned* __restrict__ amax) {
+                                                                unsigned* __restrict__ amax, float* __restrict__ amax_out2) {
   const int n = blockIdx.y;
   const int total = Do * Ho * Wo * C4;
   const long long V = (long long)D * H * W;
@@ -651,7 +656,7 @@
       mx = fmaxf(fmaxf(mx, fmaxf(fabsf(val.x), fabsf(val.y))), fmaxf(fabsf(val.z), fabsf(val.w)));
     }
   }
-  if (amax) kmh_absmax::publish(mx, amax);
+  if (amax) kmh_absmax::publish_tail(mx, amax, amax_out2, 0.f);
 }
 
 __device__ __forceinline__ int nearest_src(int dst, int in_size, int out_size) {
@@ -852,6 +857,41 @@
   return kmh_absmax::launch(x, n, min_abs, out2, (hipStream_t)stream);
 }
 
+extern "C" unsigned* kmh_absmax_scratch(void* stream) {
+  static std::mutex mu;
+  static std::map<std::pair<int, void*>, unsigned*> table;
+  int dev = 0;
+  if (hipGetDevice(&dev) != hipSuccess) return nullptr;
+  std::lock_guard<std::mutex> lock(mu);
+  auto it = table.find({dev, stream});
+  if (it != table.end()) return it->second;
+  unsigned* p = nullptr;
+  const size_t bytes = kmh_absmax::kScratchBytes;
+  if (hipMalloc(&p, bytes) != hipSuccess) return nullptr;
+  if (hipMemsetAsync(p, 0, bytes, (hipStream_t)stream) != hipSuccess) {
+    (void)hipFree(p);
+    return nullptr;
+  }
+  table[{dev, stream}] = p;
+  return p;
+}
+
+KMH_API int kmh_absmax_segments(const float* flat, const long long* table, int nseg, long long max_len, float* out,
+                                void* stream) {
+  if (!flat || !table || !out || nseg < 0 || max_len < 0) return -22;
+  hipStream_t s = (hipStream_t)stream;
+  if (!kmh_absmax::folded()) return -22;
+  unsigned* acc = kmh_absmax_scratch(s);
+  if (!acc) return (int)hipErrorOutOfMemory;
+  long long nb = (max_len / 4 + 256) / 256;
+  if (nb > 256) nb = 256;
+  for (int i0 = 0; i0 < nseg; i0 += kmh_absmax::kPairs) {
+    const int cnt = nseg - i0 < kmh_absmax::kPairs ? nseg - i0 : kmh_absmax::kPairs;
+    kmh_absmax::segments_kernel<<<dim3((unsigned)nb, cnt), 256, 0, s>>>(flat, table + 2 * i0, acc, out + 2 * i0);
+  }
+  return KMH_LAUNCH_CHECK();
+}
+
 KMH_API int kmh_gn_bwd_coeffs(const double* ab, const float* gamma, const float* mean_rstd, int N, int C, int G,
                               double count, float* c123, float* dgamma, float* dbeta, const int* only_if, void* stream) {
   if (G <= 0 || C % G) return -22;
@@ -873,9 +913,11 @@
                              int relu_mask, int accumulate, float* dx, float* dx_scale2, int out_blocked, void* stream) {
   hipStream_t s = (hipStream_t)stream;
   if (out_blocked && ((C & 7) || dx == dxn || dx == x)) return -22;
+  kmh_absmax::Tail t;
+  if (int rc = t.open(dx_scale2, true, s)) return rc;
   gn_bwd_apply_kernel<<<dim3(stream_blocks(V * C / 4), N), TPB, 0, s>>>(dxn, x, c123, V, C, relu_mask, accumulate, dx,
-                                                                      reinterpret_cast<unsigned*>(dx_scale2), out_blocked);
-  if (dx_scale2) kmh_absmax::final_kernel<<<1, 1, 0, s>>>(dx_scale2, 0.f);
+                                                                      t.acc, t.out2, out_blocked);
+  t.close(s);
   return KMH_LAUNCH_CHECK();
 }
 
@@ -1032,13 +1074,10 @@
 KMH_API int kmh_in_bwd_apply(const float* du, const float* z, const float* scale, const float* shift, const float* c123,
                              int N, long long V, int C, float* dz, float* dz_scale2, void* stream) {
   hipStream_t s = (hipStream_t)stream;
-  if (dz_scale2) {
-    hipError_t e = hipMemsetAsync(dz_scale2, 0, 2 * sizeof(float), s);
-    if (e != hipSuccess) return (int)e;
-  }
-  in_bwd_apply_kernel<<<dim3(stream_blocks(V * C / 4), N), TPB, 0, s>>>(du, z, scale, shift, c123, V, C, dz,
-                                                                       reinterpret_cast<unsigned*>(dz_scale2));
-  if (dz_scale2) kmh_absmax::final_kernel<<<1, 1, 0, s>>>(dz_scale2, 0.f);
+  kmh_absmax::Tail t;
+  if (int rc = t.open(dz_scale2, false, s)) return rc;
+  in_bwd_apply_kernel<<<dim3(stream_blocks(V * C / 4), N), TPB, 0, s>>>(du, z, scale, shift, c123, V, C, dz, t.acc, t.out2);
+  t.close(s);
   return KMH_LAUNCH_CHECK();
 }
 
@@ -1051,14 +1090,12 @@
   if (pooled / 4 >= (1ll << 31) || (long long)D * H * W >= (1ll << 31)) return -22;
   if ((((uintptr_t)du | (uintptr_t)z | (uintptr_t)dz) & 15) || ((uintptr_t)argmax & 3)) return -22;
   hipStream_t s = (hipStream_t)stream;
-  if (dz_scale2) {
-    hipError_t e = hipMemsetAsync(dz_scale2, 0, 2 * sizeof(float), s);
-    if (e != hipSuccess) return (int)e;
-  }
+  kmh_absmax::Tail t;
+  if (int rc = t.open(dz_scale2, false, s)) return rc;
   in_bwd_apply_pool_kernel<<<dim3(stream_blocks(pooled), N), TPB, 0, s>>>(
       (const unsigned*)argmax, (const float4*)du, (const float4*)z, scale, shift, c123, (float4*)dz, D, H, W, C / 4, Do, Ho, Wo,
-      reinterpret_cast<unsigned*>(dz_scale2));
-  if (dz_scale2) kmh_absmax::final_kernel<<<1, 1, 0, s>>>(dz_scale2, 0.f);
+      t.acc, t.out2);
+  t.close(s);
   return KMH_LAUNCH_CHECK();
 }
 
@@ -1128,14 +1165,12 @@
   if (pooled / 4 >= (1ll << 31) || (long long)D * H * W >= (1ll << 31)) return -22;
   if ((((uintptr_t)dxn | (uintptr_t)x | (uintptr_t)dx | (uintptr_t)dy) & 15) || ((uintptr_t)argmax & 3)) return -22;
   hipStream_t s = (hipStream_t)stream;
-  if (dx_scale2) {
-    hipError_t e = hipMemsetAsync(dx_scale2, 0, 2 * sizeof(float), s);
-    if (e != hipSuccess) return (int)e;
-  }
+  kmh_absmax::Tail t;
+  if (int rc = t.open(dx_scale2, false, s)) return rc;
   maxpool_bwd4_lazy_kernel<<<dim3(stream_blocks(pooled), N), TPB, 0, s>>>(
       (const unsigned*)argmax, (const float4*)dy, (const float4*)dxn, (const float4*)x, c123, (float4*)dx, D, H, W, C / 4, Do,
-      Ho, Wo, reinterpret_cast<unsigned*>(dx_scale2));
-  if (dx_scale2) kmh_absmax::final_kernel<<<1, 1, 0, s>>>(dx_scale2, 0.f);
+      Ho, Wo, t.acc, t.out2);
+  t.close(s);
   return KMH_LAUNCH_CHECK();
 }
 
diff --git a/keymorph_amd/parallel.py b/keymorph_amd/parallel.py
--- a/keymorph_amd/parallel.py
+++ b/keymorph_amd/parallel.py
@@ -52,6 +52,7 @@
             self._views.append(v)
             o += k
         self.numel = n
+        self._wtable = None
 
     def zero_grad(self):
         for p in self.params:
@@ -81,6 +82,30 @@
     def broadcast(self, src: int = 0):
         if dist.is_initialized() and dist.get_world_size() > 1:
             dist.broadcast(self.flat, src)
+            self.measure_weight_scales()
+
+    def measure_weight_scales(self) -> int:
+        from . import backbone_ops as B
+        from ._handoff import attach
+        if not B._needs_range_scales() or B._off("KEYMORPH_NO_FINAL_FOLD") or not self.flat.is_cuda:
+            return 0
+        if self._wtable is None:
+            rows, o = [], 0
+            for i, p in enumerate(self.params):
+                if p.dim() == 5 and tuple(p.shape[2:]) == (3, 3, 3):
+                    rows.append((i, o, p.numel()))
+                o += p.numel()
+            self._wtable = (rows, torch.tensor([[o, k] for _, o, k in rows], dtype=torch.int64, device=self.flat.device)
+                            if rows else None)
+        rows, table = self._wtable
+        if not rows:
+            return 0
+        out = torch.empty((len(rows), 2), dtype=torch.float32, device=self.flat.device)
+        check(_lib.load().kmh_absmax_segments(_p(self.flat), _p(table), len(rows), max(k for _, _, k in rows), _p(out),
+                                              _stream()), "kmh_absmax_segments")
+        for j, (i, _, _) in enumerate(rows):
+            attach(self.params[i], "wscale", out[j])
+        return len(rows)
 
     def allreduce_grads(self) -> float:
         g = self.gather()
@@ -136,6 +161,7 @@
         check(lib.kmh_adam_step(_p(self.flat.flat), _p(self.flat.gather()), _p(self.m), _p(self.v), self.flat.numel,
                                 self.lr, self.betas[0], self.betas[1], self.eps, self.t, grad_scale, _stream()),
               "kmh_adam_step")
+        self.flat.measure_weight_scales()
 
 
 def gather_group_points(local_points: torch.Tensor, num_subjects: int) -> torch.Tensor:
```

Result: no change. 16.02 (median of 5 runs) (+0.1%).
